# zhaoweicai/mscnn

Hardware: AMD Instinct MI355X
Metric: images/sec mscnn-7s-576 KITTI-car inference (higher is better)
Workload: dtype f32

## Files before the change

### include/mscnn_hip.h

```cpp
#ifndef MSCNN_HIP_H_
#define MSCNN_HIP_H_

#include <stddef.h>
#include <stdint.h>

#if defined(__GNUC__)
#define MSCNN_API __attribute__((visibility("default")))
#else
#define MSCNN_API
#endif

#ifdef __cplusplus
extern "C" {
#endif

typedef enum {
  MSCNN_OK = 0,
  MSCNN_ERR_BAD_ARG = 1,
  MSCNN_ERR_HIP = 2,
  MSCNN_ERR_WORKSPACE = 3,
  MSCNN_ERR_UNSUPPORTED = 4
} mscnn_status;

MSCNN_API const char* mscnn_last_error(void);
MSCNN_API const char* mscnn_version(void);

typedef struct mscnn_conv_plan mscnn_conv_plan;

typedef enum {
  MSCNN_CONV_ALGO_AUTO = 0,
  MSCNN_CONV_ALGO_DIRECT = 1,
  MSCNN_CONV_ALGO_WINO_F2 = 2,
  MSCNN_CONV_ALGO_WINO_F3 = 3,
  MSCNN_CONV_ALGO_F16 = 4,
  MSCNN_CONV_ALGO_WINO_F3_X3 = 5,
  MSCNN_CONV_ALGO_WINO_F4 = 6
} mscnn_conv_algo;

typedef struct {
  int N, Cin, H, W;
  int Cout, Kh, Kw;
  int pad_h, pad_w, stride_h, stride_w, group;
  int relu;
  int algo;
  int tune_variant, tune_grid, tune_flags;
} mscnn_conv_desc;

MSCNN_API int mscnn_conv2d_plan_create(const mscnn_conv_desc* desc, mscnn_conv_plan** plan_out);
MSCNN_API void mscnn_conv2d_plan_destroy(mscnn_conv_plan* plan);
MSCNN_API size_t mscnn_conv2d_packed_weight_bytes(const mscnn_conv_plan* plan);
MSCNN_API size_t mscnn_conv2d_workspace_bytes(const mscnn_conv_plan* plan);
MSCNN_API const char* mscnn_conv2d_plan_kernel(const mscnn_conv_plan* plan);
MSCNN_API double mscnn_conv2d_plan_flops(const mscnn_conv_plan* plan);
MSCNN_API const char* mscnn_conv2d_plan_dtype(const mscnn_conv_plan* plan);
MSCNN_API double mscnn_conv2d_plan_executed_flops(const mscnn_conv_plan* plan);
MSCNN_API int mscnn_conv2d_plan_set_profiling(mscnn_conv_plan* plan, int on);
MSCNN_API int mscnn_conv2d_plan_stage_ms(const mscnn_conv_plan* plan, float ms_out[3]);
#define MSCNN_AMAX_SLOTS 1024
MSCNN_API int mscnn_conv2d_plan_publishes_amax(const mscnn_conv_plan* plan);
MSCNN_API int mscnn_conv2d_plan_set_amax_io(mscnn_conv_plan* plan, const uint32_t* in_bound, uint32_t* out_amax);
MSCNN_API int mscnn_conv2d_plan_set_batch(mscnn_conv_plan* plan, int N);
MSCNN_API unsigned long long mscnn_conv2d_plan_weight_layout(const mscnn_conv_plan* plan);
MSCNN_API int mscnn_conv2d_pack_weights(const mscnn_conv_plan* plan, const float* w, float* packed, void* stream);
MSCNN_API int mscnn_conv2d_fwd_f32(const mscnn_conv_plan* plan, const float* x, const float* w, const float* packed,
                         const float* bias, float* y, void* workspace, size_t workspace_bytes, void* stream);
MSCNN_API int mscnn_conv2d_plan_can_pool(const mscnn_conv_plan* plan);
MSCNN_API int mscnn_conv2d_fwd_pool_f32(const mscnn_conv_plan* plan, const float* x, const float* w, const float* packed,
                              const float* bias, float* y, float* y_pool, void* workspace, size_t workspace_bytes,
                              void* stream);

MSCNN_API int mscnn_relu_fwd_f32(const float* x, float* y, size_t count, float negative_slope, void* stream);

MSCNN_API int mscnn_pool_out_dim(int in, int kernel, int pad, int stride);
MSCNN_API int mscnn_pool2d_fwd_f32(const float* x, float* y, int N, int C, int H, int W, int kernel_h, int kernel_w,
                         int pad_h, int pad_w, int stride_h, int stride_w, int method, void* stream);

MSCNN_API int mscnn_inner_product_fwd_f32(const float* x, const float* w, const float* bias, float* y,
                                int M, int N, int K, int relu, void* stream);
MSCNN_API void mscnn_debug_inner_product_rows(int rows);

MSCNN_API int mscnn_inner_product_wg_supported(int M, int N, int K);
MSCNN_API size_t mscnn_inner_product_wg_packed_bytes(int N, int K);
MSCNN_API size_t mscnn_inner_product_wg_workspace_bytes(int M, int N, int K);
MSCNN_API int mscnn_inner_product_wg_pack(const float* w, float* wt, int N, int K, void* stream);
MSCNN_API int mscnn_inner_product_wg_fwd(const float* x, const float* wt, const float* bias, float* y, int M, int N, int K, int relu,
                                         void* workspace, size_t workspace_bytes, void* stream);
MSCNN_API unsigned long long mscnn_wgemm_handoff_event(void);
MSCNN_API void mscnn_wgemm_force_whole_tiles(int on);
MSCNN_API int mscnn_wgemm_whole_tiles_forced(void);
MSCNN_API void mscnn_debug_wgemm_handoff_fault(int drop_publish, unsigned spin_limit);
MSCNN_API int mscnn_inner_product_x3_supported(int N, int K);
MSCNN_API size_t mscnn_inner_product_x3_packed_bytes(int N, int K);
MSCNN_API size_t mscnn_inner_product_x3_workspace_bytes(int M, int N, int K);
MSCNN_API int mscnn_inner_product_x3_pack(const float* w, void* packed, int N, int K, void* stream);
MSCNN_API int mscnn_inner_product_x3_fwd(const float* x, const void* packed, const float* bias, float* y, int M, int N, int K, int relu,
                               const uint32_t* in_bound, void* workspace, size_t workspace_bytes, void* stream);
MSCNN_API int mscnn_inner_product_f16_supported(int N, int K);
MSCNN_API int mscnn_inner_product_pack_f16(const float* w, void* w16, int N, int K, void* stream);
MSCNN_API int mscnn_inner_product_fwd_f16(const float* x, const void* w16, const float* bias, float* y, int M, int N, int K, int relu,
                                          void* stream);

MSCNN_API int mscnn_concat_channels_f32(const float* x, float* y, int N, int C, int inner, int C_total, int c_offset, void* stream);

MSCNN_API int mscnn_deconv_depthwise_fwd_f32(const float* x, const float* w, const float* bias, float* y,
                                   int N, int C, int H, int W, int Kh, int Kw, int pad_h, int pad_w,
                                   int stride_h, int stride_w, void* stream);

MSCNN_API int mscnn_deconv2d_fwd_f32(const float* x, const float* w, const float* bias, float* y, int N, int Cin, int H, int W,
                                     int Cout, int Kh, int Kw, int pad_h, int pad_w, int stride_h, int stride_w, int group,
                                     void* stream);

MSCNN_API int mscnn_max_rel_diff_f32(const float* a, const float* ref, size_t count, float floor, float* out_dev, void* stream);
MSCNN_API int mscnn_max_rel_diff_strided_f32(const float* a, size_t a_stride, const float* ref, size_t ref_stride, size_t planes, size_t run,
                                             const double* sumsq_dev, double sumsq_count, float* out_dev, void* stream);
MSCNN_API int mscnn_store_words_i32(int* dst_dev, const int* values_host, int n, void* stream);
MSCNN_API int mscnn_sum_squares_f32(const float* x, size_t count, double* out_dev, void* stream);

MSCNN_API int mscnn_softmax_fwd_f32(const float* x, float* y, int outer, int C, int inner, void* stream);

MSCNN_API int mscnn_roipool_fwd_f32(const float* feat, const float* rois, float* out, int R, int N, int C, int H, int W,
                          int pooled_h, int pooled_w, float spatial_scale, float pad_ratio,
                          int C_total, int c_offset, void* stream);
MSCNN_API int mscnn_roipool_pair_fwd_f32(const float* feat, const float* rois, float* out, int R, int N, int C, int H, int W,
                                         int pooled_h, int pooled_w, float spatial_scale, float pad_ratio_a, int c_offset_a,
                                         float pad_ratio_b, int c_offset_b, int C_total, void* stream);

MSCNN_API int mscnn_conv2d_plan_can_chain(const mscnn_conv_plan* plan, const mscnn_conv_plan* next);
MSCNN_API int mscnn_conv2d_plan_can_pool_only(const mscnn_conv_plan* plan);
MSCNN_API int mscnn_conv2d_fwd_chain_f32(const mscnn_conv_plan* plan, const mscnn_conv_plan* next, const float* x, const float* packed,
                               const float* bias, float* y, float* y_pool, void* workspace, size_t workspace_bytes,
                               void* next_workspace, size_t next_workspace_bytes, void* stream);

MSCNN_API int mscnn_conv2d_plan_can_fuse_roipool(const mscnn_conv_plan* plan, int C, int pooled_h, int pooled_w);
MSCNN_API size_t mscnn_conv2d_roipool_workspace_bytes(const mscnn_conv_plan* plan, int N, int C, int H, int W);
MSCNN_API size_t mscnn_roipool_maps_bytes(int N, int C, int H, int W);
MSCNN_API int mscnn_roipool_maps_build_f32(const float* feat, float* maps, int N, int C, int H, int W, void* stream);
MSCNN_API int mscnn_conv2d_fwd_roipool_pair_f32(const mscnn_conv_plan* plan, const float* feat, const float* prepared_maps, int N, int C,
                                                int H, int W, const float* rois, float spatial_scale, float pad_ratio_a,
                                                float pad_ratio_b, const float* packed_w, const float* bias, float* y, void* workspace,
                                                size_t workspace_bytes, void* stream);

MSCNN_API int mscnn_roialign_fwd_f32(const float* feat, const float* rois, float* out, int R, int N, int C, int H, int W,
                                     int pooled_h, int pooled_w, float spatial_scale, float pad_ratio, void* stream);
// ... 129 lines not shown
```

### mscnn_amd/csrc/conv.hip

```cpp
#include "common.h"
#include "headconv.h"
#include "winograd.h"
#include "wino_x3.h"
#include "wgemm.h"
#include "roipool_wino.h"
#include "conv_c3.h"
#include "wconv.h"
#include "wf2conv.h"
#include "x3_device.h"
#include <new>
#include <type_traits>

namespace {

typedef float f32x16 __attribute__((ext_vector_type(16)));
typedef _Float16 f16x8 __attribute__((ext_vector_type(8)));

struct IgemmArgs {
  const float* x; const float* wp; const float* bias; float* y; float* ws;
  int N, Cin, H, W, Cout, Ho, Wo, pad_h, pad_w;
  int MT, NTH, NTW, NT, KI, G, relu;
  int xcd_map;
  int epi_prio;
  float* yp;
  int Hp, Wp;
  int nt_major;
  unsigned w_img_bytes;
  int full_q;
  long total_iters;
  const unsigned* amax_in; const float* w_inv;
  unsigned* amax_out;
#ifdef MSCNN_WG_TRACE
  unsigned long long* trace;
#endif
};
#ifdef MSCNN_WG_TRACE
static unsigned long long* g_wg_trace = nullptr;
extern "C" __attribute__((visibility("default"))) void mscnn_debug_set_wg_trace(void* p) { g_wg_trace = static_cast<unsigned long long*>(p); }
#define MSCNN_TRACE_STAMP(slot)                                                                                  \
  if (a.trace && tid == 0 && (slot) < 16) a.trace[(long)blockIdx.x * 16 + (slot)] = __builtin_amdgcn_s_memrealtime();
#else
#define MSCNN_TRACE_STAMP(slot)
#endif
constexpr int kSlabsPerWg = 2;

template <int BM_, int BN_, int WGM_, int WGN_, int KH_, int KW_, int CK_, int TW_, int RH_ = 0, int RW_ = 0, int RP_ = 0, int PF_ = 0, int VEC_ = 0, int NOPN_ = 0, int F16_ = 0>
struct Cfg {
  static constexpr bool F16 = F16_ != 0;
  static constexpr bool X3 = F16_ == 2;
  static constexpr int PARTS = X3 ? 2 : 1;
  static constexpr bool PUBLISH = VEC_ == 0 && F16_ != 1;
  static constexpr int MIN_WG_PER_CU = PF_ == 3 ? 4 : (PF_ == 4 || PF_ == 5) ? 3 : 2;
  static constexpr int KG = CK_ / 8;
  static constexpr int VEC = VEC_;
  static constexpr bool PREFETCH_NEXT = VEC_ != 0 && NOPN_ == 0;
  static constexpr int F4_PER_CH = BN_ / 4;
  static constexpr int CH_PER_PASS = 256 / F4_PER_CH;
  static constexpr int BV_PER_T = CK_ * F4_PER_CH / 256;
// ... 799 lines not shown
#define ROI_ENTRY16(RH, RW, RP)                                                                                              \
  {"igemm16_128x128_k3x3_roi" #RH "x" #RW "p" #RP, 128, 128, 3, 3, 16, 0, 0, RH, RW, RP,                                       \
   Cfg<128, 128, 2, 2, 3, 3, 16, 32, RH, RW, RP, 0, 0, 0, 1>::IPT, 4, 200, igemm_kernel<Cfg<128, 128, 2, 2, 3, 3, 16, 32, RH, RW, RP, 0, 0, 0, 1>>, \
   igemm_fixup_kernel<Cfg<128, 128, 2, 2, 3, 3, 16, 32, RH, RW, RP, 0, 0, 0, 1>>}
    ENTRY16(128, 128, 2, 2, 16),
    ENTRY16(128, 128, 2, 2, 32),
    ENTRY16(64, 256, 1, 4, 32),
#define ENTRY16_OCC3(BM, BN, WGM, WGN, TW)                                                                                   \
  {"igemm16_" #BM "x" #BN "_k3x3_tw" #TW "_occ3", BM, BN, 3, 3, 16, TW, BN / TW, 0, 0, 0, 1, (BM * BN) / 4096, 201,            \
   igemm_kernel<Cfg<BM, BN, WGM, WGN, 3, 3, 16, TW, 0, 0, 0, 4, 0, 0, 1>>, igemm_fixup_kernel<Cfg<BM, BN, WGM, WGN, 3, 3, 16, TW, 0, 0, 0, 4, 0, 0, 1>>, \
   Cfg<BM, BN, WGM, WGN, 3, 3, 16, TW, 0, 0, 0, 4, 0, 0, 1>::CAN_POOL ? igemm_fixup_pool_kernel<Cfg<BM, BN, WGM, WGN, 3, 3, 16, TW, 0, 0, 0, 4, 0, 0, 1>> : nullptr}
    {"igemm16_128x256_k3x3_tw32", 128, 256, 3, 3, 16, 32, 8, 0, 0, 0, 1, 8, 202, igemm_kernel<Cfg<128, 256, 2, 2, 3, 3, 16, 32, 0, 0, 0, 0, 0, 0, 1>>,
     igemm_fixup_kernel<Cfg<128, 256, 2, 2, 3, 3, 16, 32, 0, 0, 0, 0, 0, 0, 1>>, igemm_fixup_pool_kernel<Cfg<128, 256, 2, 2, 3, 3, 16, 32, 0, 0, 0, 0, 0, 0, 1>>},
    {"igemm16x3_64x256_k3x3_tw32", 64, 256, 3, 3, 16, 32, 8, 0, 0, 0, 1, 4, 210, igemm_kernel<Cfg<64, 256, 1, 4, 3, 3, 16, 32, 0, 0, 0, 0, 0, 0, 2>>,
     igemm_fixup_kernel<Cfg<64, 256, 1, 4, 3, 3, 16, 32, 0, 0, 0, 0, 0, 0, 2>>, igemm_fixup_pool_kernel<Cfg<64, 256, 1, 4, 3, 3, 16, 32, 0, 0, 0, 0, 0, 0, 2>>},
    ENTRY16_OCC3(128, 128, 2, 2, 16),
    ENTRY16_OCC3(128, 128, 2, 2, 32),
    ENTRY16_OCC3(64, 256, 1, 4, 32),
    ROI_ENTRY16(7, 7, 0),
    ROI_ENTRY16(7, 5, 0),
    ROI_ENTRY16(8, 4, 1),
    ENTRY(32, 128, 1, 4, 5, 5, 8, 16),
    ENTRY(32, 128, 1, 4, 7, 7, 8, 16),
    ENTRY(32, 128, 1, 4, 5, 3, 8, 16),
    ENTRY(32, 128, 1, 4, 7, 5, 8, 16),
    ENTRY(64, 256, 1, 4, 5, 1, 8, 32),
    ENTRY(64, 256, 1, 4, 7, 1, 8, 32),
    ROI_ENTRY(128, 128, 2, 2, 3, 3, 8, 7, 7, 0),
    ROI_ENTRY(128, 128, 2, 2, 3, 3, 8, 7, 5, 0),
    ROI_ENTRY(128, 128, 2, 2, 3, 3, 8, 8, 4, 1),
};
constexpr int kTableN = sizeof(kTable) / sizeof(kTable[0]);

}

struct mscnn_conv_plan {
  mscnn_conv_desc d;
  int Ho, Wo;
  int entry;
  int MT, NTH, NTW, NT, KI, G, full_q;
  long total_iters;
  size_t packed_bytes, ws_bytes;
  mscnn::HeadPlan head;
  mscnn_conv_plan* wino = nullptr;
  bool use_wg = false;
  mscnn::WgemmPlan wg;
  bool c3 = false;
  bool wc_use = false;
  mscnn::WconvPlan wc;
  bool wf_use = false;
  mscnn::Wf2Plan wf;
  int wino_m = 2;
  int tiles_h = 0, tiles_w = 0, T_pad = 0;
  mscnn::X3Plan x3;
  mscnn::X3HeadPlan x3h;
  mscnn_conv_plan* hg = nullptr;
  int hg_rows = 0;
  int hg_kw = 0;
  size_t hg_t_bytes = 0;
  size_t x3d_hdr_off = 0, x3d_slots_off = 0;
  const unsigned* amax_in = nullptr;
  unsigned* amax_out = nullptr;
  bool profiling = false;
  mutable hipEvent_t ev[4] = {nullptr, nullptr, nullptr, nullptr};
  mutable bool ev_valid = false;
  ~mscnn_conv_plan() {
    delete hg;
    delete wino;
    for (hipEvent_t e : ev) if (e) (void)hipEventDestroy(e);
  }
};

using namespace mscnn;

static void plan_shape(mscnn_conv_plan* p);

static bool head_gemm_plan(mscnn_conv_plan* p) {
  const mscnn_conv_desc& d = p->d;
  const int flags = tune_env("MSCNN_TUNE_FLAGS", d.tune_flags);
  const long HW = (long)d.H * d.W;
  if (tune_env("MSCNN_CONV_ALGO", d.algo) == MSCNN_CONV_ALGO_WINO_F3_X3 || (flags & 32) || (flags & 2)) return false;
  if (d.stride_h != 1 || d.stride_w != 1 || d.group != 1 || d.Cout > 12 || d.Kh * d.Kw < 2 || d.Kh * d.Kw > 64 || d.N < 1) return false;
  if (d.Cin % 32 != 0 || d.Cin < 32 || p->Ho < 1 || p->Wo < 1) return false;
  const bool kw_legal = d.Kw * d.Cout >= 40 && d.Kw * d.Cout <= 64 && d.pad_w * 2 + 1 == d.Kw && p->Ho == d.H && p->Wo == d.W &&
                        (d.Kh == 5 || d.Kh == 7) && HW >= 1024;
  if (!(flags & 16) && !(flags & 512) && kw_legal && ((flags & 1024) || (d.Kw * d.Cout >= 56 && HW >= 8192))) {
    mscnn_conv_plan* g = new (std::nothrow) mscnn_conv_plan();
    if (!g) return false;
    g->d = d;
    g->d.N = 1; g->d.Cout = d.Kw * d.Cout; g->d.Kw = 1; g->d.pad_w = 0; g->d.relu = 0;
    g->d.algo = MSCNN_CONV_ALGO_DIRECT;
    g->d.tune_variant = 0; g->d.tune_grid = 0; g->d.tune_flags = (flags & 1) | 32 | 2;
    plan_shape(g);
    if (g->entry >= 0 && !g->wino && !g->hg && g->head.entry < 0 && g->Ho == d.H && g->Wo == d.W && kTable[g->entry].KW == 1 &&
        kTable[g->entry].BM == 64) {
      p->hg = g;
      p->hg_kw = d.Kw;
      p->hg_rows = d.Kw * d.Cout;
      p->hg_t_bytes = ((size_t)p->hg_rows * HW * sizeof(float) + 255) / 256 * 256;
      p->packed_bytes = g->packed_bytes + (size_t)p->hg_rows * d.Cin * d.Kh * sizeof(float);
      p->ws_bytes = p->hg_t_bytes + g->ws_bytes;
      return true;
    }
    delete g;
  }
  if (!(flags & 16) && !kHeadGemmDefault) return false;
  if (!(flags & 16) && HW < kHeadGemmMinPixels) return false;
  const int rows = d.Kh * d.Kw * d.Cout;
  if ((double)rows * HW * 4.0 >= 2.0e9) return false;
  mscnn_conv_plan* g = new (std::nothrow) mscnn_conv_plan();
  if (!g) return false;
  g->d = d;
  g->d.N = 1; g->d.Cout = rows; g->d.Kh = g->d.Kw = 1; g->d.pad_h = g->d.pad_w = 0; g->d.relu = 0;
  g->d.algo = MSCNN_CONV_ALGO_DIRECT;
  g->d.tune_variant = 0; g->d.tune_grid = 0; g->d.tune_flags = flags & 1;
  if (HW % 128 == 0) { g->d.H = (int)(HW / 128); g->d.W = 128; }
  else { g->d.H = 1; g->d.W = (int)HW; }
  plan_shape(g);
  if (g->entry < 0 || g->wino || g->hg || g->head.entry >= 0 || g->Ho * (long)g->Wo != HW) { delete g; return false; }
  p->hg = g;
  p->hg_kw = 0;
  p->hg_rows = rows;
  p->hg_t_bytes = ((size_t)rows * HW * sizeof(float) + 255) / 256 * 256;
  p->packed_bytes = g->packed_bytes + (size_t)rows * d.Cin * sizeof(float);
  p->ws_bytes = p->hg_t_bytes + g->ws_bytes;
  return true;
}

static bool wino_plan(mscnn_conv_plan* p) {
  const mscnn_conv_desc& d = p->d;
  const int algo = tune_env("MSCNN_CONV_ALGO", d.algo);
  if (algo == MSCNN_CONV_ALGO_DIRECT || d.Kh != 3 || d.Kw != 3 || d.stride_h != 1 || d.stride_w != 1 || d.group != 1) return false;
  if (p->Ho < 2 || p->Wo < 2) return false;
  const bool want_x3 = algo == MSCNN_CONV_ALGO_WINO_F3_X3;
  if (want_x3 && (d.tune_flags & 8)) return false;
  const bool force = algo == MSCNN_CONV_ALGO_WINO_F2 || algo == MSCNN_CONV_ALGO_WINO_F3 || algo == MSCNN_CONV_ALGO_WINO_F4 ||
                     (want_x3 && (d.tune_flags & 4));
  const double intensity = (double)d.Cin * d.Cout / (d.Cin + d.Cout);
  const bool roi_map = d.H <= 8 && d.W <= 8;
  const long T4 = (long)d.N * cdiv(p->Ho, 4) * cdiv(p->Wo, 4);
  const bool auto_f4 = algo == MSCNN_CONV_ALGO_AUTO && !roi_map && T4 >= 1000 && !(d.tune_flags & 64);
  const int m = roi_map ? 3 : (algo == MSCNN_CONV_ALGO_WINO_F2 ? 2 : (algo == MSCNN_CONV_ALGO_WINO_F4 || auto_f4) ? 4 : 3);
  const int planes = (m + 2) * (m + 2);
  const double wino_min = want_x3 && d.Cin % 16 == 0 ? 80.0 : (m == 4 ? 40.0 : m == 3 ? 60.0 : 100.0);
  if (!force && (intensity < wino_min || (!roi_map && d.H * d.W < 256))) return false;
  if (roi_map && d.N < 8) return false;
  const int th = cdiv(p->Ho, m), tw = cdiv(p->Wo, m);
  const long T = (long)d.N * th * tw;
  const long T_pad = (T + 127) / 128 * 128;
  if ((double)T_pad * (d.Cin > d.Cout ? d.Cin : d.Cout) * 4.0 >= 2.0e9) return false;
  if (want_x3 && m == 3 && x3_plan(d.Cin, d.Cout, T_pad, d.tune_variant, &p->x3)) {
    p->wino_m = 3;
    p->tiles_h = th; p->tiles_w = tw; p->T_pad = (int)T_pad;
    p->packed_bytes = p->x3.packed_bytes;
    p->ws_bytes = p->x3.scal_bytes + p->x3.v_bytes + (size_t)25 * d.Cout * T_pad * sizeof(float);
    return true;
  }
  mscnn_conv_plan* g = new (std::nothrow) mscnn_conv_plan();
  if (!g) return false;
  g->d = d;
  if (g->d.tune_variant >= 300) g->d.tune_variant = 0;
  g->d.N = planes; g->d.H = (int)(T_pad / 128); g->d.W = 128; g->d.Kh = g->d.Kw = 1; g->d.pad_h = g->d.pad_w = 0; g->d.relu = 0;
  g->d.algo = MSCNN_CONV_ALGO_DIRECT;
  plan_shape(g);
  if (g->entry >= 0 && g->d.tune_variant == 0 && (long)g->MT * g->NT >= 3000 && ((long)g->MT * g->NT) % 1000 == 0) {
    g->d.tune_variant = 107;
    g->d.tune_grid = 1000;
    plan_shape(g);
  }
  if (g->entry < 0 || g->wino || g->head.entry >= 0) { delete g; return false; }
  p->wino_m = m;
  p->wino = g;
  p->tiles_h = th; p->tiles_w = tw; p->T_pad = (int)T_pad;
  p->packed_bytes = (size_t)planes * g->packed_bytes;
  p->ws_bytes = (size_t)planes * ((size_t)d.Cin + d.Cout) * T_pad * sizeof(float) + g->ws_bytes;
  p->use_wg = false;
  if (m >= 3 && !(d.tune_flags & 128) && mscnn::wgemm_plan(planes, d.Cout, d.Cin, (int)T, (d.tune_variant >= 300 && d.tune_variant < 1100) ? d.tune_variant - 300 : 0, &p->wg)) {
    p->use_wg = true;
    p->T_pad = p->wg.T_pad;
    p->packed_bytes = p->wg.packed_bytes;
    p->ws_bytes = (size_t)planes * ((size_t)d.Cin + d.Cout) * p->wg.T_pad * sizeof(float) + p->wg.ws_bytes;
  }
  return true;
}

static void plan_shape(mscnn_conv_plan* p) {
  const mscnn_conv_desc& d = p->d;
  p->Ho = (d.H + 2 * d.pad_h - d.Kh) / d.stride_h + 1;
  p->Wo = (d.W + 2 * d.pad_w - d.Kw) / d.stride_w + 1;
  p->entry = -1;
  p->c3 = false;
  p->wc_use = false;
  p->wf_use = false;
  p->packed_bytes = 0;
  p->ws_bytes = 0;
  p->head.entry = -1;
  p->x3h = mscnn::X3HeadPlan();
  delete p->hg;
  p->hg = nullptr;
  p->hg_rows = 0;
  p->hg_kw = 0;
  p->hg_t_bytes = 0;
  if (tune_env("MSCNN_CONV_ALGO", d.algo) == MSCNN_CONV_ALGO_WINO_F3_X3 && d.stride_h == 1 && d.stride_w == 1 && d.group == 1 &&
      d.Cout <= 12 && d.Kh * d.Kw > 1 && d.N > 0 && !(d.tune_flags & 2) &&
      x3_head_plan(d.Cin, d.Cout, d.Kh, d.Kw, (long)d.H * d.W, &p->x3h)) {
    p->packed_bytes = p->x3h.packed_bytes;
    p->ws_bytes = 4096 + p->x3h.t_bytes;
    return;
  }
  if (head_gemm_plan(p)) return;
  if (head_plan(d, p->Ho, p->Wo, &p->head)) {
    p->packed_bytes = p->head.packed_bytes;
    p->ws_bytes = p->head.ws_bytes;
    return;
  }
  delete p->wino;
  p->wino = nullptr;
  p->x3 = mscnn::X3Plan();
  {
    const int algo = tune_env("MSCNN_CONV_ALGO", d.algo);
    const bool named_wino = algo == MSCNN_CONV_ALGO_WINO_F2 || algo == MSCNN_CONV_ALGO_WINO_F3 || algo == MSCNN_CONV_ALGO_WINO_F4;
    if (!named_wino && !(d.tune_flags & 2048) && mscnn::c3_plan(d, p->Ho, p->Wo)) { p->c3 = true; return; }
  }
  if (d.stride_h != 1 || d.stride_w != 1 || d.group != 1 || d.N == 0 || d.Cin > 2048) return;
  const bool want16 = tune_env("MSCNN_CONV_ALGO", d.algo) == MSCNN_CONV_ALGO_F16 && d.Kh == 3 && d.Kw == 3;
  if (!want16 && wino_plan(p)) return;
  const bool wantx3 = tune_env("MSCNN_CONV_ALGO", d.algo) == MSCNN_CONV_ALGO_WINO_F3_X3 && d.Kh == 3 && d.Kw == 3 && d.Cin % 16 == 0 &&
                      (long)d.H * d.W >= 4096;
  const double win_x = (double)d.Cin * d.H * d.W * 4.0, win_y = (double)d.Cout * p->Ho * p->Wo * 4.0;
  double best = 1e300;
  const int tv0 = tune_env("MSCNN_TUNE_VARIANT", d.tune_variant);
  const int tv = tv0 >= 400 ? 0 : tv0;
  const bool venv = tv > 0 && d.Kh == 3 && d.Kw == 3;
  const int want = venv ? tv - 1 : (d.Cout >= 128 ? 1 : 0);
// ... 94 lines not shown
  MSCNN_REQUIRE(p, "conv plan: out of memory");
  p->d = d;
  plan_shape(p);
  *plan_out = p;
  return MSCNN_OK;
}

extern "C" void mscnn_conv2d_plan_destroy(mscnn_conv_plan* plan) { delete plan; }
extern "C" size_t mscnn_conv2d_packed_weight_bytes(const mscnn_conv_plan* p) { return p ? p->packed_bytes : 0; }
extern "C" size_t mscnn_conv2d_workspace_bytes(const mscnn_conv_plan* p) { return p ? p->ws_bytes : 0; }
extern "C" const char* mscnn_conv2d_plan_kernel(const mscnn_conv_plan* p) {
  if (!p) return "";
  if (p->x3h.rows) return "head_gemm_shiftadd_x3f16";
  if (p->hg) return p->hg_kw ? "head_kwfold_shiftadd_f32" : "head_gemm_shiftadd_f32";
  if (p->head.entry >= 0) return head_kernel_name(p->head);
  if (p->x3.BM) return p->x3.BM == 256 ? "winograd_f3x3_3x3_x3f16_256" : "winograd_f3x3_3x3_x3f16_128";
  if (p->wino) return p->wino_m == 4 ? "winograd_f4x4_3x3" : p->wino_m == 3 ? "winograd_f3x3_3x3" : "winograd_f2x2_3x3";
  if (p->c3) return mscnn::c3_kernel_name();
  if (p->wf_use) return mscnn::wf2_kernel_name();
  if (p->wc_use) return mscnn::wconv_kernel_name();
  return p->entry < 0 ? "direct_f32" : kTable[p->entry].name;
}
extern "C" unsigned long long mscnn_conv2d_plan_weight_layout(const mscnn_conv_plan* p) {
  if (!p) return 0;
  unsigned long long kind, e, mt, ki;
  if (p->x3h.rows) { kind = 7; e = (unsigned)p->x3h.rows_pad; mt = 0; ki = (unsigned)p->x3h.KG; }
  else if (p->hg) { kind = p->hg_kw ? 10 : 8; e = (unsigned)p->hg->entry; mt = (unsigned)p->hg->MT; ki = (unsigned)p->hg->KI; }
  else if (p->head.entry >= 0) { kind = 2; e = p->head.valu >= 0 ? 100u + (unsigned)p->head.valu : (unsigned)p->head.entry; mt = 0; ki = (unsigned)p->head.KI; }
  else if (p->x3.BM) { kind = 6; e = (unsigned)p->x3.BM; mt = (unsigned)p->x3.MT; ki = (unsigned)p->x3.KG; }
  else if (p->wino && p->use_wg) { kind = p->wino_m == 4 ? 9u : 2 + (unsigned)p->wino_m; e = 200u + (unsigned)(p->wg.BM / 128);       mt = (unsigned)p->wg.MT; ki = (unsigned)p->wg.KI; }
  else if (p->wino) { kind = p->wino_m == 4 ? 9u : 2 + (unsigned)p->wino_m; e = (unsigned)p->wino->entry; mt = (unsigned)p->wino->MT; ki = (unsigned)p->wino->KI; }
  else if (p->wf_use) { kind = 11; e = 0; mt = 1; ki = (unsigned)p->wf.KI; }
  else if (p->entry >= 0) { kind = 1; e = (unsigned)p->entry; mt = (unsigned)p->MT; ki = (unsigned)p->KI; }
  else return 0;
  return kind | (e << 8) | (mt << 24) | (ki << 44);
}
extern "C" double mscnn_conv2d_plan_flops(const mscnn_conv_plan* p) {
  if (!p) return 0;
  const mscnn_conv_desc& d = p->d;
  return 2.0 * d.N * d.Cout * p->Ho * p->Wo * (double)(d.Cin / d.group) * d.Kh * d.Kw;
}
extern "C" const char* mscnn_conv2d_plan_dtype(const mscnn_conv_plan* p) {
  if (p && p->x3h.rows) return "f16x3";
  if (p && (p->x3.BM || (!p->wino && p->head.entry < 0 && p->entry >= 0 && kTable[p->entry].variant == 210))) return "f16x3";
  return (p && !p->wino && p->head.entry < 0 && p->entry >= 0 && kTable[p->entry].variant >= 200 && kTable[p->entry].variant <= 202) ? "f16" : "f32";
}
extern "C" double mscnn_conv2d_plan_executed_flops(const mscnn_conv_plan* p) {
  if (!p) return 0;
  if (p->x3h.rows) return 3.0 * mscnn_conv2d_plan_flops(p);
  if (p->wf_use) return mscnn_conv2d_plan_flops(p) * (16.0 / 36.0);
  if (!p->wino && !p->x3.BM)
    return mscnn_conv2d_plan_flops(p) * ((p->head.entry < 0 && p->entry >= 0 && kTable[p->entry].variant == 210) ? 3.0 : 1.0);
  const mscnn_conv_desc& d = p->d;
  const double planes = (double)((p->wino_m + 2) * (p->wino_m + 2)) * (p->x3.BM ? 3.0 : 1.0);
  return 2.0 * planes * d.Cout * d.Cin * ((double)d.N * p->tiles_h * p->tiles_w);
}
extern "C" int mscnn_conv2d_plan_set_profiling(mscnn_conv_plan* p, int on) {
  MSCNN_REQUIRE(p, "conv plan: null");
  p->profiling = on != 0;
  p->ev_valid = false;
  if (p->profiling)
    for (hipEvent_t& e : p->ev)
      if (!e) MSCNN_HIP_TRY(hipEventCreate(&e));
  return MSCNN_OK;
}
extern "C" int mscnn_conv2d_plan_stage_ms(const mscnn_conv_plan* p, float ms_out[3]) {
  MSCNN_REQUIRE(p && ms_out, "conv plan: null");
  ms_out[0] = ms_out[1] = ms_out[2] = 0.f;
  MSCNN_REQUIRE(p->profiling && p->ev_valid, "conv plan: no profiled forward yet (mscnn_conv2d_plan_set_profiling)");
  MSCNN_HIP_TRY(hipEventSynchronize(p->ev[3]));
  for (int i = 0; i < 3; ++i) MSCNN_HIP_TRY(hipEventElapsedTime(&ms_out[i], p->ev[i], p->ev[i + 1]));
  return MSCNN_OK;
}
extern "C" int mscnn_conv2d_plan_publishes_amax(const mscnn_conv_plan* p) {
  return p && !p->x3h.rows && (p->x3.BM || (p->wino && p->wino_m >= 3) || p->c3 ||
               (!p->wino && p->head.entry < 0 && p->entry >= 0 && !p->wc_use && !p->wf_use && !(kTable[p->entry].variant >= 200 && kTable[p->entry].variant <= 202))) ? 1 : 0;
}
extern "C" int mscnn_conv2d_plan_set_amax_io(mscnn_conv_plan* p, const uint32_t* in_bound, uint32_t* out_amax) {
  MSCNN_REQUIRE(p, "conv plan: null");
  if (out_amax && !mscnn_conv2d_plan_publishes_amax(p)) {
    set_error("conv plan: kernel %s does not publish max |y|", mscnn_conv2d_plan_kernel(p));
    return MSCNN_ERR_UNSUPPORTED;
  }
  p->amax_in = in_bound;
  p->amax_out = out_amax;
  return MSCNN_OK;
}
extern "C" int mscnn_conv2d_plan_set_batch(mscnn_conv_plan* p, int N) {
  MSCNN_REQUIRE(p && N >= 0, "conv plan: bad batch");
  p->d.N = N;
  plan_shape(p);
  return MSCNN_OK;
}

extern "C" int mscnn_conv2d_pack_weights(const mscnn_conv_plan* p, const float* w, float* packed, void* stream) {
  MSCNN_REQUIRE(p, "conv pack: null plan");
  if (p->x3h.rows) {
    MSCNN_REQUIRE(w && packed, "conv pack: null pointer");
    return x3_head_pack(p->x3h, w, packed, as_stream(stream));
  }
  if (p->hg) {
    MSCNN_REQUIRE(w && packed, "conv pack: null pointer");
    float* wprime = reinterpret_cast<float*>(reinterpret_cast<unsigned char*>(packed) + p->hg->packed_bytes);
    if (p->hg_kw) {
      const long tot = (long)p->hg_rows * p->d.Cin * p->d.Kh;
      head_kw_weight_kernel<<<(int)((tot + 255) / 256 > 4096 ? 4096 : (tot + 255) / 256), 256, 0, as_stream(stream)>>>(
          w, wprime, p->d.Cout, p->d.Cin, p->d.Kh, p->d.Kw);
      MSCNN_POST_LAUNCH();
// ... 49 lines not shown
  const mscnn_conv_desc& d = p->d;
  const KernelEntry& k = kTable[p->entry];
  const long rem_tiles = (long)p->MT * p->NT - (long)p->full_q * p->G;
  const bool split = rem_tiles > 0;
  if (split) {
    if (!workspace || workspace_bytes < p->ws_bytes) {
      set_error("conv: workspace %zu < %zu", workspace_bytes, p->ws_bytes);
      return MSCNN_ERR_WORKSPACE;
    }
  }
  IgemmArgs a;
  a.x = x; a.wp = packed; a.bias = bias; a.y = y; a.ws = static_cast<float*>(workspace);
  a.N = d.N; a.Cin = d.Cin; a.H = d.H; a.W = d.W; a.Cout = d.Cout; a.Ho = p->Ho; a.Wo = p->Wo; a.pad_h = d.pad_h; a.pad_w = d.pad_w;
  a.MT = p->MT; a.NTH = p->NTH; a.NTW = p->NTW; a.NT = p->NT; a.KI = p->KI; a.G = p->G; a.relu = d.relu;
  a.total_iters = p->total_iters; a.full_q = p->full_q;
  a.w_img_bytes = w_img_bytes; a.nt_major = nt_major;
  a.yp = y_pool; a.Hp = (p->Ho + 1) / 2; a.Wp = (p->Wo + 1) / 2;
  if (y_pool && !k.fix_pool_fn) {
    set_error("conv: kernel %s has no fused pooling epilogue", k.name);
    return MSCNN_ERR_BAD_ARG;
  }
  a.xcd_map = (tune_env("MSCNN_TUNE_FLAGS", d.tune_flags) & 1) ? 0 : 1;
  a.epi_prio = ((k.BM == 64 && k.BN == 256 && k.KH == 3 && k.KW == 3) ? 1 : 0) ^ ((tune_env("MSCNN_TUNE_FLAGS", d.tune_flags) & 16384) ? 1 : 0);
#ifdef MSCNN_WG_TRACE
  a.trace = g_wg_trace;
#endif
  a.amax_in = nullptr; a.w_inv = nullptr;
  a.amax_out = nt_major ? nullptr : p->amax_out;
  if (k.variant == 210) {
    if (!workspace || workspace_bytes < p->ws_bytes) {
      set_error("conv(x3): workspace %zu < %zu", workspace_bytes, p->ws_bytes);
      return MSCNN_ERR_WORKSPACE;
    }
    a.w_inv = reinterpret_cast<const float*>(reinterpret_cast<const unsigned char*>(packed) + p->x3d_hdr_off);
    a.amax_in = p->amax_in;
    if (!a.amax_in) {
      unsigned* slots = reinterpret_cast<unsigned*>(static_cast<unsigned char*>(workspace) + p->x3d_slots_off);
      const int rc = x3_amax(x, (long)d.N * d.Cin * d.H * d.W, slots, st);
      if (rc != MSCNN_OK) return rc;
      a.amax_in = slots;
    }
  }
  k.main_fn<<<p->G, 256, 0, st>>>(a);
  MSCNN_POST_LAUNCH();
  if (split) {
    (y_pool ? k.fix_pool_fn : k.fix_fn)<<<(int)rem_tiles * k.fix_split, 256, 0, st>>>(a);
    MSCNN_POST_LAUNCH();
  }
  return MSCNN_OK;
}

extern "C" int mscnn_conv2d_plan_can_pool(const mscnn_conv_plan* p) {
  if (!p || p->head.entry >= 0 || p->x3h.rows || p->hg) return 0;
  if (p->wino || p->x3.BM) return p->wino_m == 2 || p->wino_m == 4 || (p->tiles_h % 2 == 0 && p->tiles_w % 2 == 0 && p->d.H > 8);
  return p->entry >= 0 && kTable[p->entry].fix_pool_fn != nullptr;
}

static int conv_forward_single(const mscnn_conv_plan* p, const float* x, const float* w, const float* packed, const float* bias,
                               float* y, float* y_pool, void* workspace, size_t workspace_bytes, hipStream_t st);

extern "C" int mscnn_conv2d_fwd_f32(const mscnn_conv_plan* p, const float* x, const float* w, const float* packed,
                                    const float* bias, float* y, void* workspace, size_t workspace_bytes, void* stream) {
  return mscnn_conv2d_fwd_pool_f32(p, x, w, packed, bias, y, nullptr, workspace, workspace_bytes, stream);
}

template <class InputStage, class OutputStage>
static int wino_forward_stages(const mscnn_conv_plan* p, const float* packed, void* workspace, size_t workspace_bytes, hipStream_t st,
                               InputStage&& input_stage, OutputStage&& output_stage) {
  const mscnn_conv_desc& d = p->d;
#define MSCNN_STAGE_EVENT(i) do { if (p->profiling) MSCNN_HIP_TRY(hipEventRecord(p->ev[i], st)); } while (0)
  MSCNN_REQUIRE(packed, "conv: Winograd path needs packed weights (mscnn_conv2d_pack_weights)");
  if (!workspace || workspace_bytes < p->ws_bytes) {
    set_error("conv(winograd): workspace %zu < %zu", workspace_bytes, p->ws_bytes);
    return MSCNN_ERR_WORKSPACE;
  }
  const mscnn_conv_plan* g = p->wino;
  const size_t planes = (size_t)(p->wino_m + 2) * (p->wino_m + 2);
  float* V = static_cast<float*>(workspace);
  float* M = V + planes * d.Cin * p->T_pad;
  float* gws = M + planes * d.Cout * p->T_pad;
  MSCNN_STAGE_EVENT(0);
  int rc = input_stage(V);
  if (rc != MSCNN_OK) return rc;
  MSCNN_STAGE_EVENT(1);
  if (p->use_wg) rc = mscnn::wgemm_launch(p->wg, packed, V, M, gws, st);
  else rc = launch_igemm(g, V, packed, nullptr, M, nullptr, gws, g->ws_bytes, st, (unsigned)g->packed_bytes, 1);
  if (rc != MSCNN_OK) return rc;
  MSCNN_STAGE_EVENT(2);
  rc = output_stage(M);
  if (rc != MSCNN_OK) return rc;
  MSCNN_STAGE_EVENT(3);
  p->ev_valid = p->profiling;
  return MSCNN_OK;
#undef MSCNN_STAGE_EVENT
}

template <class InputStage>
static int wino_forward(const mscnn_conv_plan* p, const float* packed, const float* bias, float* y, float* y_pool, void* workspace,
                        size_t workspace_bytes, hipStream_t st, InputStage&& input_stage) {
  const mscnn_conv_desc& d = p->d;
  return wino_forward_stages(p, packed, workspace, workspace_bytes, st, input_stage, [&](const float* M) {
    return wino_output_transform(p->wino_m, M, bias, y, y_pool, d.N, d.Cout, p->Ho, p->Wo, p->tiles_h, p->tiles_w, p->T_pad, d.relu, st,
                                 p->wino_m >= 3 ? p->amax_out : nullptr, (d.tune_flags & 256) != 0);
  });
}

extern "C" int mscnn_conv2d_fwd_pool_f32(const mscnn_conv_plan* p, const float* x, const float* w, const float* packed,
                                         const float* bias, float* y, float* y_pool, void* workspace, size_t workspace_bytes,
                                         void* stream) {
  MSCNN_REQUIRE(p, "conv: null plan");
  MSCNN_REQUIRE(!y_pool || mscnn_conv2d_plan_can_pool(p), "conv: this plan has no fused 2x2 max-pooling epilogue");
  const mscnn_conv_desc& d = p->d;
  if (d.N == 0) return MSCNN_OK;
  MSCNN_REQUIRE(x && (y || (y_pool && mscnn_conv2d_plan_can_pool_only(p))),
                "conv: null pointer (y may be NULL only with y_pool on a plan where mscnn_conv2d_plan_can_pool_only)");
  hipStream_t st = as_stream(stream);
#define MSCNN_STAGE_EVENT(i) do { if (p->profiling) MSCNN_HIP_TRY(hipEventRecord(p->ev[i], st)); } while (0)
  if (p->x3.BM) {
    MSCNN_REQUIRE(packed, "conv: Winograd path needs packed weights (mscnn_conv2d_pack_weights)");
    if (!workspace || workspace_bytes < p->ws_bytes) {
      set_error("conv(winograd x3): workspace %zu < %zu", workspace_bytes, p->ws_bytes);
      return MSCNN_ERR_WORKSPACE;
    }
    unsigned char* wsb = static_cast<unsigned char*>(workspace);
    const unsigned* scal = p->amax_in ? p->amax_in : reinterpret_cast<unsigned*>(wsb);
    void* V16 = wsb + p->x3.scal_bytes;
    float* M = reinterpret_cast<float*>(wsb + p->x3.scal_bytes + p->x3.v_bytes);
    MSCNN_STAGE_EVENT(0);
    int rc = p->amax_in ? MSCNN_OK : x3_amax(x, (long)d.N * d.Cin * d.H * d.W, reinterpret_cast<unsigned*>(wsb), st);
    if (rc != MSCNN_OK) return rc;
    rc = x3_input_transform(p->x3, x, V16, scal, d.N, d.H, d.W, d.pad_h, d.pad_w, p->tiles_h, p->tiles_w, st);
    if (rc != MSCNN_OK) return rc;
    MSCNN_STAGE_EVENT(1);
    rc = x3_gemm(p->x3, packed, V16, M, scal, (tune_env("MSCNN_TUNE_FLAGS", d.tune_flags) & 1) ? 0 : 1, st);
    if (rc != MSCNN_OK) return rc;
    MSCNN_STAGE_EVENT(2);
    rc = wino_output_transform(3, M, bias, y, y_pool, d.N, d.Cout, p->Ho, p->Wo, p->tiles_h, p->tiles_w, p->T_pad, d.relu, st,
                               p->amax_out);
    if (rc != MSCNN_OK) return rc;
    MSCNN_STAGE_EVENT(3);
    p->ev_valid = p->profiling;
    return MSCNN_OK;
  }
  if (!p->wino) {
    MSCNN_STAGE_EVENT(0); MSCNN_STAGE_EVENT(1);
    const int rc = conv_forward_single(p, x, w, packed, bias, y, y_pool, workspace, workspace_bytes, st);
    if (rc != MSCNN_OK) return rc;
    MSCNN_STAGE_EVENT(2); MSCNN_STAGE_EVENT(3);
    p->ev_valid = p->profiling;
    return MSCNN_OK;
  }
  return wino_forward(p, packed, bias, y, y_pool, workspace, workspace_bytes, st, [&](float* V) {
    return wino_input_transform(p->wino_m, x, V, d.N, d.Cin, d.H, d.W, d.pad_h, d.pad_w, p->tiles_h, p->tiles_w, p->T_pad, st,
                                (d.tune_flags & 256) != 0, (d.tune_flags & 4096) != 0);
  });
#undef MSCNN_STAGE_EVENT
}


static bool is_f4_plane_path(const mscnn_conv_plan* p) { return p && p->wino && p->wino_m == 4 && !p->x3.BM && p->d.N > 0; }
extern "C" int mscnn_conv2d_plan_can_chain(const mscnn_conv_plan* p, const mscnn_conv_plan* next) {
  if (!is_f4_plane_path(p) || !is_f4_plane_path(next)) return 0;
  const mscnn_conv_desc &a = p->d, &b = next->d;
  return a.N == b.N && a.Cout == b.Cin && p->Ho == b.H && p->Wo == b.W && b.Kh == 3 && b.Kw == 3 && b.pad_h == 1 && b.pad_w == 1 &&
                 b.stride_h == 1 && b.stride_w == 1 && p->tiles_h == next->tiles_h && p->tiles_w == next->tiles_w &&
                 !((a.tune_flags | b.tune_flags) & 256) && mscnn::wino44_outin_supported(p->Ho, p->Wo, p->tiles_h, p->tiles_w)
             ? 1 : 0;
}
extern "C" int mscnn_conv2d_plan_can_pool_only(const mscnn_conv_plan* p) {
  if (!p || !mscnn_conv2d_plan_can_pool(p)) return 0;
  if (is_f4_plane_path(p)) return p->Wo % 4 == 0 && p->tiles_w * 4 == p->Wo && !(p->d.tune_flags & 256) ? 1 : 0;
  return !p->wino && !p->x3.BM && !p->x3h.rows && !p->hg && p->head.entry < 0 && !p->c3 && p->entry >= 0 ? 1 : 0;
}
extern "C" int mscnn_conv2d_fwd_chain_f32(const mscnn_conv_plan* p, const mscnn_conv_plan* next, const float* x, const float* packed,
                                          const float* bias, float* y, float* y_pool, void* workspace, size_t workspace_bytes,
                                          void* next_workspace, size_t next_workspace_bytes, void* stream) {
  MSCNN_REQUIRE(p, "conv: null plan");
  MSCNN_REQUIRE(is_f4_plane_path(p), "conv(chain): the plan does not take the fp32 F(4x4,3x3) path");
  MSCNN_REQUIRE(!next || mscnn_conv2d_plan_can_chain(p, next), "conv(chain): these two plans do not chain (mscnn_conv2d_plan_can_chain)");
  MSCNN_REQUIRE(next ? !y_pool : (y != nullptr || (y_pool && mscnn_conv2d_plan_can_pool_only(p))),
                "conv(chain): y_pool only without a next plan; y may be NULL only with one, or with y_pool where mscnn_conv2d_plan_can_pool_only");
  MSCNN_REQUIRE(!y_pool || mscnn_conv2d_plan_can_pool(p), "conv: this plan has no fused 2x2 max-pooling epilogue");
  const mscnn_conv_desc& d = p->d;
  hipStream_t st = as_stream(stream);
  if (next) {
    const size_t vbytes = sizeof(float) * 36 * (size_t)next->d.Cin * next->T_pad;
    if (!next_workspace || next_workspace_bytes < next->ws_bytes) {
      set_error("conv(chain): next workspace %zu < %zu", next_workspace_bytes, next->ws_bytes);
      return MSCNN_ERR_WORKSPACE;
    }
    const unsigned char *a0 = static_cast<const unsigned char*>(workspace), *b0 = static_cast<const unsigned char*>(next_workspace);
    MSCNN_REQUIRE(b0 + vbytes <= a0 || a0 + p->ws_bytes <= b0, "conv(chain): the next plan's planes overlap this plan's workspace");
  }
  auto input_stage = [&](float* V) {
    if (!x) return (int)MSCNN_OK;
    return wino_input_transform(p->wino_m, x, V, d.N, d.Cin, d.H, d.W, d.pad_h, d.pad_w, p->tiles_h, p->tiles_w, p->T_pad, st,
                                (d.tune_flags & 256) != 0, (d.tune_flags & 4096) != 0);
  };
  if (!next) return wino_forward(p, packed, bias, y, y_pool, workspace, workspace_bytes, st, input_stage);
  return wino_forward_stages(p, packed, workspace, workspace_bytes, st, input_stage, [&](const float* M) {
    return mscnn::wino44_output_into_input(M, bias, y, static_cast<float*>(next_workspace), d.N, d.Cout, p->Ho, p->Wo, p->tiles_h, p->tiles_w,
                                           p->T_pad, next->T_pad, d.relu, st, p->amax_out);
  });
}

extern "C" int mscnn_conv2d_plan_can_fuse_roipool(const mscnn_conv_plan* p, int C, int pooled_h, int pooled_w) {
  return p && p->wino && p->wino_m == 3 && !p->x3.BM && p->d.N > 0 && p->d.Cin == 2 * C && p->d.H == pooled_h && p->d.W == pooled_w &&
                 p->tiles_h == 2 && p->tiles_w == 2 && p->d.Kh == 3 && p->d.Kw == 3 &&
                 mscnn::roipool_wino33_supported(C, pooled_h, pooled_w, p->d.pad_h, p->d.pad_w)
             ? 1 : 0;
}
static size_t roipool_scratch_offset(const mscnn_conv_plan* p) { return (p->ws_bytes + 255) / 256 * 256; }
extern "C" size_t mscnn_conv2d_roipool_workspace_bytes(const mscnn_conv_plan* p, int N, int C, int H, int W) {
  return p ? roipool_scratch_offset(p) + mscnn::roipool_wino33_scratch_bytes(N, C, H, W) : 0;
}
extern "C" size_t mscnn_roipool_maps_bytes(int N, int C, int H, int W) { return mscnn::roipool_wino33_scratch_bytes(N, C, H, W); }
extern "C" int mscnn_roipool_maps_build_f32(const float* feat, float* maps, int N, int C, int H, int W, void* stream) {
  return mscnn::roipool_wino33_build_maps(feat, maps, N, C, H, W, as_stream(stream));
}
extern "C" int mscnn_conv2d_fwd_roipool_pair_f32(const mscnn_conv_plan* p, const float* feat, const float* prepared_maps, int N, int C,
                                                 int H, int W, const float* rois, float spatial_scale, float pad_ratio_a, float pad_ratio_b,
                                                 const float* packed, const float* bias, float* y, void* workspace,
                                                 size_t workspace_bytes, void* stream) {
  MSCNN_REQUIRE(p, "conv: null plan");
  if (p->d.N == 0) return MSCNN_OK;
  MSCNN_REQUIRE((feat || prepared_maps) && rois && y && N > 0 && H > 0 && W > 0, "conv(roipool): bad argument");
  MSCNN_REQUIRE(mscnn_conv2d_plan_can_fuse_roipool(p, C, p->d.H, p->d.W), "conv(roipool): this plan does not take the fused ROI-pooling input stage");
  const size_t need = prepared_maps ? p->ws_bytes : mscnn_conv2d_roipool_workspace_bytes(p, N, C, H, W);
  if (!workspace || workspace_bytes < need) {
    set_error("conv(roipool): workspace %zu < %zu", workspace_bytes, need);
    return MSCNN_ERR_WORKSPACE;
  }
  hipStream_t st = as_stream(stream);
  float* own_maps = reinterpret_cast<float*>(static_cast<unsigned char*>(workspace) + roipool_scratch_offset(p));
  return wino_forward(p, packed, bias, y, nullptr, workspace, workspace_bytes, st, [&](float* V) {
    if (!prepared_maps) {
      const int rc = mscnn::roipool_wino33_build_maps(feat, own_maps, N, C, H, W, st);
      if (rc != MSCNN_OK) return rc;
    }
    return mscnn::roipool_wino33_forward(prepared_maps ? prepared_maps : own_maps, rois, V, p->d.N, N, C, H, W, p->T_pad, spatial_scale,
                                         pad_ratio_a, pad_ratio_b, st);
  });
}

static int conv_forward_single(const mscnn_conv_plan* p, const float* x, const float* w, const float* packed, const float* bias,
                               float* y, float* y_pool, void* workspace, size_t workspace_bytes, hipStream_t st) {
  const mscnn_conv_desc& d = p->d;
  if (p->x3h.rows) {
    MSCNN_REQUIRE(packed, "conv: head kernel needs packed weights (mscnn_conv2d_pack_weights)");
    if (!workspace || workspace_bytes < p->ws_bytes) {
      set_error("conv(head x3): workspace %zu < %zu", workspace_bytes, p->ws_bytes);
      return MSCNN_ERR_WORKSPACE;
    }
    for (int n = 0; n < d.N; ++n) {
      const int rc = x3_head_forward(p->x3h, x + (size_t)n * d.Cin * d.H * d.W, packed, bias, y + (size_t)n * d.Cout * p->Ho * p->Wo, d.H,
                                     d.W, p->Ho, p->Wo, d.pad_h, d.pad_w, d.relu, d.N == 1 ? p->amax_in : nullptr, workspace, st);
      if (rc != MSCNN_OK) return rc;
    }
    return MSCNN_OK;
  }
  if (p->hg) {
    MSCNN_REQUIRE(packed, "conv: head kernel needs packed weights (mscnn_conv2d_pack_weights)");
    if (!workspace || workspace_bytes < p->ws_bytes) {
      set_error("conv(head gemm): workspace %zu < %zu", workspace_bytes, p->ws_bytes);
      return MSCNN_ERR_WORKSPACE;
    }
    float* T = static_cast<float*>(workspace);
    void* nested_ws = static_cast<unsigned char*>(workspace) + p->hg_t_bytes;
    for (int n = 0; n < d.N; ++n) {
      int rc = launch_igemm(p->hg, x + (size_t)n * d.Cin * d.H * d.W, packed, nullptr, T, nullptr, nested_ws, p->hg->ws_bytes, st, 0u,
                            p->hg_kw ? 0 : 1);
      if (rc != MSCNN_OK) return rc;
      if (p->hg_kw)
        rc = head_shift_add(T, bias, y + (size_t)n * d.Cout * p->Ho * p->Wo, d.Cout, d.H, d.W, p->Ho, p->Wo, 1, d.Kw, 0, d.pad_w,
                            (unsigned)((long)d.H * d.W), d.relu, st);
      else
        rc = head_shift_add(T, bias, y + (size_t)n * d.Cout * p->Ho * p->Wo, d.Cout, d.H, d.W, p->Ho, p->Wo, d.Kh, d.Kw, d.pad_h, d.pad_w,
                            (unsigned)((long)d.H * d.W), d.relu, st);
      if (rc != MSCNN_OK) return rc;
    }
    return MSCNN_OK;
  }
  if (p->head.entry >= 0) {
    MSCNN_REQUIRE(packed, "conv: head kernel needs packed weights (mscnn_conv2d_pack_weights)");
    return head_forward(d, p->head, p->Ho, p->Wo, x, packed, bias, y, workspace, workspace_bytes, st);
  }
  if (p->c3) {
    MSCNN_REQUIRE(w, "conv: the Cin = 3 kernel needs the Caffe-layout weights");
    return mscnn::c3_forward(d, x, w, bias, y, p->amax_out, st);
  }
  if (p->entry < 0) {
    MSCNN_REQUIRE(w, "conv: direct kernel needs the Caffe-layout weights");
    const long total = (long)d.N * d.Cout * p->Ho * p->Wo;
    long blocks = (total + 255) / 256;
// ... 12 lines not shown
```

### mscnn_amd/csrc/roipool_wino.h

```cpp
#pragma once
#include "common.h"

namespace mscnn {

bool roipool_wino33_supported(int C, int pooled_h, int pooled_w, int conv_pad_h, int conv_pad_w);
size_t roipool_wino33_scratch_bytes(int N, int C, int H, int W);
int roipool_wino33_build_maps(const float* feat, float* maps, int N, int C, int H, int W, hipStream_t st);
int roipool_wino33_forward(const float* maps, const float* rois, float* V, int R, int N, int C, int H, int W, int T_pad,
                           float spatial_scale, float pad_a, float pad_b, hipStream_t st);

}
```

### mscnn_amd/csrc/roipool_wino.hip

```cpp
#include "roipool_wino.h"
#include "wino33_device.h"
#include <cfloat>

namespace {

typedef unsigned u32x4 __attribute__((ext_vector_type(4)));

constexpr int kNB = 4;
constexpr int kLevels = 4;

struct RpwArgs {
  const float* maps;
  const float* rois;
  float* V;
  int R, C, H, W, T_pad;
  unsigned level_bytes, maps_bytes, v_bytes;
  float spatial_scale, pad_a, pad_b;
};

__device__ __forceinline__ __amdgpu_buffer_rsrc_t make_rsrc(const void* p, unsigned bytes) {
  return __builtin_amdgcn_make_buffer_rsrc(const_cast<void*>(p), 0, (int)bytes, 0x00020000);
}
__device__ __forceinline__ int uni(int v) { return __builtin_amdgcn_readfirstlane(v); }
__device__ __forceinline__ float max3(float a, float b, float c) {
  float r;
  asm("v_max3_f32 %0, %1, %2, %3" : "=v"(r) : "v"(a), "v"(b), "v"(c));
  return r;
}
__device__ __forceinline__ void launder(float& v) { asm volatile("" : "+v"(v)); }

constexpr int kRois = 8;
constexpr int kLdsRow = kRois * 4 + 4;

template <int PH, int PW>
__global__ __launch_bounds__(kRois * 64) void roipool_wino33_kernel(RpwArgs a) {
  static_assert(PH == 7 && PW == 7, "tiles per ROI: 2 x 2 tiles of 3 x 3 outputs (a 16-byte unit of V per plane)");
  __shared__ __attribute__((aligned(16))) float s_out[5 * 64 * kLdsRow];
  const int tid = threadIdx.x, lane = tid & 63, wave = uni(tid >> 6);
  const int r0 = blockIdx.y * kRois;
  const int r = r0 + wave;
  const bool live = r < a.R;
  const int c0 = blockIdx.x * 64;
  const int c = c0 + lane;
  const __amdgpu_buffer_rsrc_t rF = make_rsrc(a.maps, a.maps_bytes), rV = make_rsrc(a.V, a.v_bytes);
  const unsigned lane_off = (unsigned)c * 4u;

  const float* roi = a.rois + 5 * (size_t)(live ? r : 0);
  const int b = (int)roi[0];
  const float x1 = roi[1], y1 = roi[2], x2 = roi[3], y2 = roi[4];
  const int H = a.H, W = a.W, C = a.C;
  const int row0 = b * H;
  const unsigned pxB = (unsigned)C * 4u, rowB = (unsigned)W * pxB;
  auto load_at = [&](unsigned off) {
#ifdef RPW_NO_POOL
    return (float)(off + lane);
#endif
    return __builtin_bit_cast(float, __builtin_amdgcn_raw_buffer_load_b32(rF, lane_off, off, 0));
  };

  {
    const int q = blockIdx.z;
    const float pad_ratio = q == 0 ? a.pad_a : a.pad_b;
    const float pad_w = (x2 - x1 + 1) * pad_ratio;
    const float pad_h = (y2 - y1 + 1) * pad_ratio;
    const int roi_start_w = (int)roundf((x1 - pad_w) * a.spatial_scale);
    const int roi_start_h = (int)roundf((y1 - pad_h) * a.spatial_scale);
    const int roi_end_w = (int)roundf((x2 + pad_w) * a.spatial_scale);
    const int roi_end_h = (int)roundf((y2 + pad_h) * a.spatial_scale);
    const int roi_width = max(roi_end_w - roi_start_w + 1, 1);
    const int roi_height = max(roi_end_h - roi_start_h + 1, 1);
    const float bin_size_h = (float)roi_height / (float)PH;
    const float bin_size_w = (float)roi_width / (float)PW;
    const bool wide = roi_width >= roi_height;
    int bw_[PW];
    unsigned wsB[PW], weB[PW];
#pragma unroll
    for (int pw = 0; pw < PW; ++pw) {
      const int ws = uni(min(max((int)floorf((float)pw * bin_size_w) + roi_start_w, 0), W));
      const int we = uni(min(max((int)ceilf((float)(pw + 1) * bin_size_w) + roi_start_w, 0), W));
      bw_[pw] = we - ws;
      wsB[pw] = (unsigned)min(ws, W - 1) * pxB;
      weB[pw] = (unsigned)max(we, min(ws, W - 1) + 1) * pxB;
    }

    float pooled[PH * PW];
#pragma unroll
    for (int ph = 0; ph < PH; ++ph) {
// ... 23 lines not shown
            v[bi][0] = load_at(ac0 + al0); v[bi][1] = load_at(ac0 + a1); v[bi][2] = load_at(ac0 + a2); v[bi][3] = load_at(ac0 + a3);
            v[bi][4] = load_at(ac1 + al0); v[bi][5] = load_at(ac1 + a1); v[bi][6] = load_at(ac1 + a2); v[bi][7] = load_at(ac1 + a3);
          }
        }
#pragma unroll
        for (int bi = 0; bi < NB; ++bi) {
          const int pw = half * NB + bi;
          if (pw < PW) {
            const int w = bw_[pw];
            float m = max3(v[bi][0], v[bi][1], v[bi][2]);
            m = max3(m, v[bi][3], v[bi][4]);
            m = max3(m, v[bi][5], v[bi][6]);
            m = max3(m, v[bi][7], -FLT_MAX);
            const int s_ = 1 << lev[bi];
            const int across_len = wide ? h : w, along_len = wide ? w : h;
            if (across_len > 2 * s_ || along_len > 4 * s_) {
              const unsigned stepx = pxB << lev[bi], stepy = rowB << lev[bi];
              const unsigned xlastB = weB[pw] - stepx, ylastB = heB - stepy, base = (unsigned)lev[bi] * a.level_bytes;
              for (unsigned yB = hsB; yB < heB; yB += stepy)
                for (unsigned xB = wsB[pw]; xB < weB[pw]; xB += 4 * stepx) {
                  const unsigned rb = base + min(yB, ylastB);
                  const float u0 = load_at(rb + min(xB, xlastB)), u1 = load_at(rb + min(xB + stepx, xlastB));
                  const float u2 = load_at(rb + min(xB + 2 * stepx, xlastB)), u3 = load_at(rb + min(xB + 3 * stepx, xlastB));
                  m = max3(m, u0, u1);
                  m = max3(m, u2, u3);
                }
            }
            pooled[ph * PW + pw] = (h <= 0 || w <= 0) ? 0.f : m;
          }
        }
      }
    }

#ifdef RPW_DBG_POOLED
    {
      const unsigned rb = ((unsigned)(q * C) * (unsigned)a.T_pad + (unsigned)r * 4u) * 4u, vl = (unsigned)c * (unsigned)a.T_pad * 4u;
      const unsigned pb = (unsigned)(2 * C) * (unsigned)a.T_pad * 4u;
      if (live)
#pragma unroll
        for (int k = 0; k < PH * PW; ++k)
          __builtin_amdgcn_raw_buffer_store_b32(__builtin_bit_cast(unsigned, pooled[k]), rV, vl, rb + (unsigned)(k % 25) * pb + (unsigned)(k / 25) * 4u, 0);
      return;
    }
#endif
    const unsigned plane_bytes = (unsigned)(2 * C) * (unsigned)a.T_pad * 4u;
#pragma unroll
    for (int i = 0; i < 5; ++i) {
#pragma unroll
      for (int k = 0; k < PH * PW; ++k) launder(pooled[k]);
      float out[5][4];
#pragma unroll
      for (int t = 0; t < 4; ++t) {
        const int ty = t >> 1, tx = t & 1;
        float rr[5];
#pragma unroll
        for (int j = 0; j < 5; ++j) {
          float d[5], o[5];
#pragma unroll
          for (int k = 0; k < 5; ++k) {
            const int h = 3 * ty + k, w = 3 * tx + j;
            d[k] = (h < PH && w < PW) ? pooled[h * PW + w] : 0.f;
          }
          mscnn::bt5(d, o);
          rr[j] = o[i];
        }
        float o2[5];
        mscnn::bt5(rr, o2);
#pragma unroll
        for (int j = 0; j < 5; ++j) out[j][t] = o2[j];
      }
      __syncthreads();
#pragma unroll
      for (int j = 0; j < 5; ++j)
        *reinterpret_cast<float4*>(&s_out[(j * 64 + lane) * kLdsRow + wave * 4]) = make_float4(out[j][0], out[j][1], out[j][2], out[j][3]);
      __syncthreads();
#pragma unroll
      for (int n = 0; n < 5 * 64 * kRois / (kRois * 64); ++n) {
        const int item = tid + n * (kRois * 64);
        const int rq = item % kRois, ch = (item / kRois) % 64, j = item / (kRois * 64);
        if (r0 + rq < a.R) {
          const float4 u = *reinterpret_cast<const float4*>(&s_out[(j * 64 + ch) * kLdsRow + rq * 4]);
          u32x4 pk;
          pk.x = __builtin_bit_cast(unsigned, u.x); pk.y = __builtin_bit_cast(unsigned, u.y);
          pk.z = __builtin_bit_cast(unsigned, u.z); pk.w = __builtin_bit_cast(unsigned, u.w);
          const unsigned off = (unsigned)(i * 5 + j) * plane_bytes + ((unsigned)(q * C + c0 + ch) * (unsigned)a.T_pad + (unsigned)(r0 + rq) * 4u) * 4u;
#ifndef RPW_NO_STORE
          __builtin_amdgcn_raw_buffer_store_b128(pk, rV, off, 0u, 0);
#else
          if (a.T_pad < 0) __builtin_amdgcn_raw_buffer_store_b128(pk, rV, off, 0u, 0);
#endif
        }
      }
    }
  }
}

__global__ __launch_bounds__(256) void nchw_to_nhwc_kernel(const float* __restrict__ x, float* __restrict__ y, int C, int HW) {
  __shared__ float t[64][65];
  const int n = blockIdx.z, c0 = blockIdx.y * 64, p0 = blockIdx.x * 64;
  const int tx = threadIdx.x & 63, ty = threadIdx.x >> 6;
  const float* src = x + (size_t)n * C * HW;
  float* dst = y + (size_t)n * C * HW;
#pragma unroll
  for (int i = 0; i < 16; ++i) {
    const int cc = c0 + ty + 4 * i, pp = p0 + tx;
    t[ty + 4 * i][tx] = (cc < C && pp < HW) ? src[(size_t)cc * HW + pp] : 0.f;
  }
  __syncthreads();
#pragma unroll
  for (int i = 0; i < 16; ++i) {
    const int pp = p0 + ty + 4 * i, cc = c0 + tx;
    if (pp < HW && cc < C) dst[(size_t)pp * C + cc] = t[tx][ty + 4 * i];
  }
}

__global__ __launch_bounds__(256) void sliding_max_kernel(const float* __restrict__ src, float* __restrict__ dst, int H, int W, int C4, int half,
                                                          long total) {
  const long i = blockIdx.x * 256L + threadIdx.x;
  if (i >= total) return;
  const int c4 = (int)(i % C4);
  long p = i / C4;
  const int x = (int)(p % W); p /= W;
  const int y = (int)(p % H);
  const long n = p / H;
  const int y2 = min(y + half, H - 1), x2 = min(x + half, W - 1);
  const float4* s4 = reinterpret_cast<const float4*>(src) + n * H * W * C4;
  const float4 a = s4[((long)y * W + x) * C4 + c4], b = s4[((long)y * W + x2) * C4 + c4];
  const float4 c = s4[((long)y2 * W + x) * C4 + c4], d = s4[((long)y2 * W + x2) * C4 + c4];
  float4 m = a;
  m.x = b.x > m.x ? b.x : m.x; m.y = b.y > m.y ? b.y : m.y; m.z = b.z > m.z ? b.z : m.z; m.w = b.w > m.w ? b.w : m.w;
  m.x = c.x > m.x ? c.x : m.x; m.y = c.y > m.y ? c.y : m.y; m.z = c.z > m.z ? c.z : m.z; m.w = c.w > m.w ? c.w : m.w;
  m.x = d.x > m.x ? d.x : m.x; m.y = d.y > m.y ? d.y : m.y; m.z = d.z > m.z ? d.z : m.z; m.w = d.w > m.w ? d.w : m.w;
  reinterpret_cast<float4*>(dst)[i] = m;
}

}

namespace mscnn {

bool roipool_wino33_supported(int C, int pooled_h, int pooled_w, int conv_pad_h, int conv_pad_w) {
  return pooled_h == 7 && pooled_w == 7 && conv_pad_h == 0 && conv_pad_w == 0 && C > 0 && C % 64 == 0;
}

size_t roipool_wino33_scratch_bytes(int N, int C, int H, int W) { return (size_t)kLevels * N * C * H * W * sizeof(float); }

int roipool_wino33_build_maps(const float* feat, float* maps, int N, int C, int H, int W, hipStream_t st) {
  MSCNN_REQUIRE(feat && maps, "roipool maps: null pointer");
  MSCNN_REQUIRE(N > 0 && C % 64 == 0 && H > 0 && W > 0, "roipool maps: bad shape");
  MSCNN_REQUIRE(kLevels * (double)N * C * H * W * 4.0 < 4.0e9, "roipool maps: beyond a 32-bit buffer window");
  MSCNN_REQUIRE(reinterpret_cast<uintptr_t>(maps) % 16 == 0, "roipool maps: the maps must be 16-byte aligned");
  const int HW = H * W;
  const long per_level = (long)N * C * HW;
  nchw_to_nhwc_kernel<<<dim3(cdiv(HW, 64), cdiv(C, 64), N), 256, 0, st>>>(feat, maps, C, HW);
  MSCNN_POST_LAUNCH();
  for (int k = 1; k < kLevels; ++k) {
    const long total = per_level / 4;
    sliding_max_kernel<<<(unsigned)((total + 255) / 256), 256, 0, st>>>(maps + (k - 1) * per_level, maps + k * per_level, H, W, C / 4, 1 << (k - 1), total);
    MSCNN_POST_LAUNCH();
  }
  return MSCNN_OK;
}

int roipool_wino33_forward(const float* maps, const float* rois, float* V, int R, int N, int C, int H, int W, int T_pad,
                           float spatial_scale, float pad_a, float pad_b, hipStream_t st) {
  MSCNN_REQUIRE(maps && rois && V, "roipool+transform: null pointer");
  MSCNN_REQUIRE(R > 0 && N > 0 && C % 64 == 0 && H > 0 && W > 0 && T_pad >= 4 * R && T_pad % 4 == 0, "roipool+transform: bad shape");
  const double lb = (double)N * C * H * W * 4.0, vb = 25.0 * 2.0 * C * (double)T_pad * 4.0;
  MSCNN_REQUIRE(kLevels * lb < 4.0e9 && vb < 4.0e9, "roipool+transform: feature maps or transform planes beyond a 32-bit buffer window");
  MSCNN_REQUIRE(reinterpret_cast<uintptr_t>(V) % 16 == 0, "roipool+transform: V must be 16-byte aligned");
  RpwArgs a;
  a.maps = maps; a.rois = rois; a.V = V;
  a.R = R; a.C = C; a.H = H; a.W = W; a.T_pad = T_pad;
  a.level_bytes = (unsigned)lb; a.maps_bytes = (unsigned)(kLevels * lb); a.v_bytes = (unsigned)vb;
  a.spatial_scale = spatial_scale; a.pad_a = pad_a; a.pad_b = pad_b;
  roipool_wino33_kernel<7, 7><<<dim3(C / 64, cdiv(R, kRois), 2), kRois * 64, 0, st>>>(a);
  MSCNN_POST_LAUNCH();
  return MSCNN_OK;
}

}
```

### mscnn_amd/csrc/wgemm.h

```cpp
#pragma once
#include <hip/hip_runtime.h>
#include <cstddef>

namespace mscnn {

struct WgemmPlan {
  int P, Cout, Cin, T, T_pad;
  int BM, BN, CK, MT, NT, KI;
  int G;
  int device;
  int full_q;
  int variant;
  double model_us;
  const char* name;
  size_t packed_bytes;
  size_t ws_bytes;
};

bool wgemm_plan(int P, int Cout, int Cin, int T, int variant, WgemmPlan* out);

int wgemm_launch(const WgemmPlan& p, const float* Up, const float* V, float* M, float* ws, hipStream_t st, int abl = 0,
                 unsigned long long* dbg = nullptr, const float* bias = nullptr, int relu = 0, size_t m_valid_bytes = 0);

unsigned long long wgemm_handoff_event();
void wgemm_force_whole_tiles(int on);
int wgemm_whole_tiles_forced();
void wgemm_debug_handoff_fault(int drop_publish, unsigned spin_limit);

}
```

### mscnn_amd/csrc/wgemm.hip

```cpp
#include "wgemm.h"
#include "common.h"
#include <atomic>
#include <chrono>

namespace {

typedef float f32x16 __attribute__((ext_vector_type(16)));

struct WgemmArgs {
  const float* Up; const float* V; float* M; float* ws;
  int P, MT, NT, KI, Cin, Cout, T_pad;
  int tiles, G, abl;
  int full_q;
  unsigned ws_bytes;
  unsigned epoch;
  unsigned long long* dbg;
  unsigned up_bytes, v_bytes, m_bytes;
  const float* bias; int relu;
  unsigned long long* status;
  unsigned spin_limit;
  int drop_publish;
};

template <int BM_, int BN_, int WGM_, int WGN_, int CK_, int ST_, int DPG_ = 1, int SK_ = 0>
struct WCfg {
  static constexpr int BM = BM_, BN = BN_, WGM = WGM_, WGN = WGN_, CK = CK_, ST = ST_;
  static constexpr int DPG = DPG_, SK = SK_;
  static constexpr int NW = WGM * WGN, THREADS = NW * 64;
  static constexpr int WM = BM / WGM, WN = BN / WGN, MI = WM / 32, NI = WN / 32;
  static constexpr int A_BYTES = CK * BM * 4, B_BYTES = CK * BN * 4, STAGE_BYTES = A_BYTES + B_BYTES;
  static constexpr int STAGE_FLOATS = STAGE_BYTES / 4;
  static constexpr int PA = A_BYTES / 1024, PB = B_BYTES / 1024;
  static constexpr int PA_W = PA / NW, PB_W = (PB + NW - 1) / NW;
  static constexpr int NP = PA_W + PB_W;
  static constexpr int F4_PER_ROW = BN / 4;
  static constexpr bool B_EVEN = (64 % F4_PER_ROW == 0) && (PB % NW == 0);
  static constexpr int ROWS_PER_PIECE = B_EVEN ? 64 / F4_PER_ROW : 0;
  static constexpr int LDS_FLOATS = ST * STAGE_FLOATS + (B_EVEN ? 0 : 256);
  static constexpr int STEPS = CK / 2;
  static_assert(PA % NW == 0 && B_BYTES % 1024 == 0, "pieces per wave");
  static_assert(LDS_FLOATS * 4 <= 160 * 1024, "LDS ring");
  static_assert(WM % 32 == 0 && WN % 32 == 0, "wave tile");
};

template <int I, int N, class F>
__device__ __forceinline__ void static_for(F&& f) {
  if constexpr (I < N) {
    f(std::integral_constant<int, I>{});
    static_for<I + 1, N>(f);
  }
}

__device__ __forceinline__ __amdgpu_buffer_rsrc_t make_rsrc(const void* p, unsigned bytes) {
  return __builtin_amdgcn_make_buffer_rsrc(const_cast<void*>(p), 0, (int)bytes, 0x00020000);
}

__device__ __forceinline__ void dma16(__amdgpu_buffer_rsrc_t rsrc, unsigned voff, unsigned soff, unsigned lds_addr) {
  soff = __builtin_amdgcn_readfirstlane(soff);
  lds_addr = __builtin_amdgcn_readfirstlane(lds_addr);
  asm volatile("s_nop 4\n\ts_mov_b32 m0, %3\n\ts_nop 0\n\tbuffer_load_dwordx4 %0, %1, %2 offen lds" ::"v"(voff), "s"(rsrc), "s"(soff), "s"(lds_addr) : "memory");
}

template <int N>
__device__ __forceinline__ void wait_vm_barrier() {
  if constexpr (N == 0) asm volatile("s_waitcnt vmcnt(0)\n\ts_barrier" ::: "memory");
  else asm volatile("s_waitcnt vmcnt(%0)\n\ts_barrier" ::"n"(N) : "memory");
}

template <int OFF>
__device__ __forceinline__ float lds_rd(unsigned addr) {
  float r;
  asm volatile("ds_read_b32 %0, %1 offset:%2" : "=v"(r) : "v"(addr), "n"(OFF) : "memory");
  return r;
}
template <int N>
__device__ __forceinline__ void lds_wait() { asm volatile("s_waitcnt lgkmcnt(%0)" ::"n"(N) : "memory"); }
__device__ __forceinline__ void lds_pin(float& v) { asm volatile("" : "+v"(v)); }

__device__ __host__ __forceinline__ void wg_range(int total, int G, int g, int& b, int& e) {
  b = (int)((unsigned)total * (unsigned)g / (unsigned)G);
  e = (int)((unsigned)total * (unsigned)(g + 1) / (unsigned)G);
}

struct SegCursor {
  int slot, G, KI, full_q, rem_tile0, r;
  int it, re;
  int nparts;
  __device__ __forceinline__ void init(const WgemmArgs& a, int slot_) {
    slot = slot_; G = a.G; KI = a.KI; rem_tile0 = a.full_q * a.G; r = 0; nparts = 0;
    full_q = slot_ < a.tiles ? min(a.full_q, (a.tiles - slot_ + a.G - 1) / a.G) : 0;
    if (a.tiles > rem_tile0) wg_range((a.tiles - rem_tile0) * a.KI, a.G, slot_, it, re);
    else it = re = 0;
  }
  __device__ __forceinline__ int units() const { return full_q * KI + (re - it); }
  __device__ __forceinline__ bool next(int& t, int& k0, int& k1, int& part) {
    if (r < full_q) { t = slot + r * G; k0 = 0; k1 = KI; part = -1; ++r; return true; }
    if (it >= re) return false;
    t = rem_tile0 + it / KI;
    k0 = it % KI;
    const int left = re - it;
    k1 = left < KI - k0 ? k0 + left : KI;
    it += k1 - k0;
    part = (k0 == 0 && k1 == KI) ? -1 : nparts++;
    return true;
  }
};

template <class C, int ABL, int EPI = 0>
__global__ __launch_bounds__(C::THREADS, C::NW / 4) void wgemm_kernel(WgemmArgs a) {
  __shared__ __attribute__((aligned(1024))) float lds[C::LDS_FLOATS];
  __shared__ unsigned s_handoff_timeout;
  static_assert(C::ST == 3, "the ring protocol below is written for three stages");
  const int tid = threadIdx.x;
  const int lane = tid & 63;
  const int wave = __builtin_amdgcn_readfirstlane(tid >> 6);
  const int l31 = lane & 31, khalf = lane >> 5;
  const int wm = wave / C::WGN, wn = wave % C::WGN;

  const int xcd = (int)(blockIdx.x % 8), gq = a.G / 8, gr = a.G % 8;
  const int slot = xcd * gq + min(xcd, gr) + (int)(blockIdx.x / 8);
  SegCursor pcur, ccur;
  pcur.init(a, slot); ccur.init(a, slot);
  const int nunits = pcur.units();
  if (nunits == 0) return;
  unsigned long long dbg_c = 0, dbg_r = 0;
  if (a.dbg && tid == 0) { dbg_c = __builtin_amdgcn_s_memtime(); dbg_r = __builtin_amdgcn_s_memrealtime(); }

  const __amdgpu_buffer_rsrc_t rA = make_rsrc(a.Up, a.up_bytes), rB = make_rsrc(a.V, a.v_bytes), rM = make_rsrc(a.M, a.m_bytes),
                               rW = make_rsrc(a.ws, a.ws_bytes);
  const unsigned row_bytes = (unsigned)a.T_pad * 4u;
  const unsigned vA = (unsigned)lane * 16u;
  const unsigned vB = (unsigned)(lane / C::F4_PER_ROW) * row_bytes + (unsigned)(lane % C::F4_PER_ROW) * 16u;
  unsigned vBj[C::PB_W];
#pragma unroll
  for (int i = 0; i < C::PB_W; ++i) {
    const int u = (wave * C::PB_W + i) * 64 + lane;
    vBj[i] = wave * C::PB_W + i < C::PB ? (unsigned)(u / C::F4_PER_ROW) * row_bytes + (unsigned)(u % C::F4_PER_ROW) * 16u : 0x80000000u;
  }
  const unsigned lds0 = (unsigned)(size_t)lds;
  const unsigned a_lane = (unsigned)(khalf * C::BM + wm * C::WM + l31) * 4u;
  const unsigned b_lane = (unsigned)C::A_BYTES + (unsigned)(khalf * C::BN + wn * C::WN + l31) * 4u;

  int pu = 0, p_kc = 0, p_k1 = 0, p_stage = 0;
  unsigned p_a = 0, p_b = 0;
  unsigned vA_eff = vA, vB_eff = vB;
  auto p_begin = [&]() {
    if (pu >= nunits) {
      vA_eff = 0x80000000u; vB_eff = 0x80000000u;
#pragma unroll
      for (int i = 0; i < C::PB_W; ++i) vBj[i] = 0x80000000u;
    }
    if (p_kc == p_k1 && pu < nunits) {
      int t, part;
      pcur.next(t, p_kc, p_k1, part);
      const int mt = t % a.MT, nt = (t / a.MT) % a.NT, p = t / (a.MT * a.NT);
      p_kc = __builtin_amdgcn_readfirstlane(p_kc); p_k1 = __builtin_amdgcn_readfirstlane(p_k1);
      p_a = __builtin_amdgcn_readfirstlane((unsigned)((p * a.MT + mt) * a.KI) * (unsigned)C::A_BYTES);
      p_b = __builtin_amdgcn_readfirstlane(((unsigned)(p * a.Cin) * (unsigned)a.T_pad + (unsigned)(nt * C::BN)) * 4u);
    }
  };
  auto p_piece = [&](auto ic) {
    constexpr int i = decltype(ic)::value;
    const unsigned ls = lds0 + (unsigned)p_stage * C::STAGE_BYTES;
    if constexpr (i < C::PA_W) {
      const unsigned sa = p_a + (unsigned)p_kc * C::A_BYTES + (unsigned)(wave * C::PA_W + i) * 1024u;
      dma16(rA, vA_eff, sa, ls + (unsigned)(wave * C::PA_W + i) * 1024u);
    } else if constexpr (C::B_EVEN) {
      const int j = wave * C::PB_W + (i - C::PA_W);
      const unsigned sb = p_b + (unsigned)(p_kc * C::CK + j * C::ROWS_PER_PIECE) * row_bytes;
      dma16(rB, vB_eff, sb, ls + C::A_BYTES + (unsigned)j * 1024u);
    } else {
      const int j = wave * C::PB_W + (i - C::PA_W);
      const unsigned sb = p_b + (unsigned)(p_kc * C::CK) * row_bytes;
      dma16(rB, vBj[i - C::PA_W], sb, j < C::PB ? ls + C::A_BYTES + (unsigned)j * 1024u : lds0 + (unsigned)(C::ST * C::STAGE_BYTES));
    }
  };
  auto p_end = [&]() {
    ++pu;
    ++p_kc;
    if (++p_stage == C::ST) p_stage = 0;
  };

#pragma unroll
  for (int i = 0; i < 2; ++i)
    if (pu < nunits) {
      p_begin();
      static_for<0, C::NP>([&](auto ic) { p_piece(ic); });
      p_end();
    }
  wait_vm_barrier<0>();

  f32x16 acc[2][C::MI][C::NI];
#pragma unroll
  for (int q = 0; q < 2; ++q)
#pragma unroll
    for (int mi = 0; mi < C::MI; ++mi)
#pragma unroll
      for (int ni = 0; ni < C::NI; ++ni)
#pragma unroll
        for (int r = 0; r < 16; ++r) acc[q][mi][ni][r] = 0.f;
  float old_bias[C::NI];
#pragma unroll
  for (int ni = 0; ni < C::NI; ++ni) old_bias[ni] = 0.f;
  unsigned old_voff[C::MI][C::NI];
#pragma unroll
  for (int mi = 0; mi < C::MI; ++mi)
#pragma unroll
    for (int ni = 0; ni < C::NI; ++ni) old_voff[mi][ni] = 0x80000000u;
// ... 56 lines not shown
        if constexpr (s + 1 < C::STEPS) WG_READ(nxt, c_addr, s + 1)
        else WG_READ(nxt, next_addr, 0)
        lds_wait<NR>();
      }
#pragma unroll
      for (int mi = 0; mi < C::MI; ++mi) lds_pin(av[cur][mi]);
#pragma unroll
      for (int ni = 0; ni < C::NI; ++ni) lds_pin(bv[cur][ni]);
      __builtin_amdgcn_sched_barrier(0);
      static_for<0, NMF>([&](auto jc) {
        constexpr int j = decltype(jc)::value, mi = j / C::NI, ni = j % C::NI;
        if constexpr (!(ABL & 4)) acc[PAR][mi][ni] = __builtin_amdgcn_mfma_f32_32x32x2f32(av[cur][mi], bv[cur][ni], acc[PAR][mi][ni], 0, 0, 0);
        __builtin_amdgcn_sched_barrier(0);
        if constexpr (FLUSH && s >= C::SK) {
          if constexpr (!(ABL & 2))
            static_for<0, SPM>([&](auto kc_) {
              constexpr int e = (s - C::SK) * SPG + j * SPM + decltype(kc_)::value;
              if constexpr (e < (s - C::SK + 1) * SPG && e < TOTAL) store_one(std::integral_constant<int, PAR ^ 1>{}, std::integral_constant<int, e>{});
            });
          __builtin_amdgcn_sched_barrier(0);
        }
        if constexpr (j < C::DPG && s * C::DPG + j < C::NP) {
          if constexpr (!(ABL & 1)) p_piece(std::integral_constant<int, s * C::DPG + j>{});
          __builtin_amdgcn_sched_barrier(0);
        }
      });
    });
    p_end();
    if constexpr (ABL & 16) asm volatile("s_waitcnt vmcnt(0)" ::: "memory");
    else if constexpr (FLUSH) wait_vm_barrier<(AFTER_DMA < 63 ? AFTER_DMA : 63)>();
    else wait_vm_barrier<0>();
    c_addr = next_addr;
  };

  int c_stage = 0;
  auto next_stage_addr = [&]() {
    if (++c_stage == C::ST) c_stage = 0;
    return lds0 + (unsigned)c_stage * C::STAGE_BYTES;
  };
  int t, k0, k1, part;
  int fin_tile = -1;
  typedef __attribute__((address_space(1))) unsigned long long gu64;
  gu64* flags = (gu64*)(a.ws + (size_t)a.G * (C::BM * C::BN));
  const unsigned long long want_flag = ((unsigned long long)a.epoch << 32) | (unsigned)~a.epoch;
  auto publish_flag = [&]() {
    asm volatile("s_waitcnt vmcnt(0)\n\ts_barrier" ::: "memory");
    if (tid == 0 && !a.drop_publish) __hip_atomic_store(flags + slot, want_flag, __ATOMIC_RELAXED, __HIP_MEMORY_SCOPE_AGENT);
  };
  auto segment = [&](auto par_c) {
    constexpr int PAR = decltype(par_c)::value;
    chunk(par_c, std::true_type{}, next_stage_addr());
    if (old_pub) { publish_flag(); old_pub = false; }
    for (int kc = k0 + 1; kc < k1; ++kc) chunk(par_c, std::false_type{}, next_stage_addr());
    const int mt = t % a.MT, nt = (t / a.MT) % a.NT, p = t / (a.MT * a.NT);
    const bool pub = part >= 0 && k0 > 0;
    if (part >= 0 && k0 == 0) fin_tile = t;
    old_pub = pub;
    if (pub) { old_rsrc = rW; old_rowb = (unsigned)C::BN * 4u; }
    else { old_rsrc = rM; old_rowb = row_bytes; }
    const unsigned slab = (unsigned)slot * (unsigned)(C::BM * C::BN * 4);
    if constexpr (EPI) {
#pragma unroll
      for (int ni = 0; ni < C::NI; ++ni) {
        const int col = nt * C::BN + wn * C::WN + ni * 32 + l31;
        old_bias[ni] = (a.bias && col < a.T_pad) ? a.bias[col] : 0.f;
      }
    }
#pragma unroll
    for (int mi = 0; mi < C::MI; ++mi)
#pragma unroll
      for (int ni = 0; ni < C::NI; ++ni) {
        const int row = wm * C::WM + mi * 32, col = wn * C::WN + ni * 32 + l31;
        const int co0 = mt * C::BM + row;
        const unsigned to_m = co0 + 32 <= a.Cout ? ((unsigned)(p * a.Cout + co0 + 4 * khalf) * (unsigned)a.T_pad + (unsigned)(nt * C::BN + col)) * 4u : 0x80000000u;
        const unsigned to_ws = slab + (unsigned)((row + 4 * khalf) * C::BN + col) * 4u;
        old_voff[mi][ni] = pub ? to_ws : to_m;
#pragma unroll
        for (int r = 0; r < 16; ++r) acc[PAR ^ 1][mi][ni][r] = 0.f;
      }
  };
  int par = 0;
  while (true) {
    if (!ccur.next(t, k0, k1, part)) break;
    segment(std::integral_constant<int, 0>{});
    par = 1;
    if (!ccur.next(t, k0, k1, part)) break;
    segment(std::integral_constant<int, 1>{});
    par = 0;
  }
  auto finish = [&](auto qc) {
    constexpr int Q = decltype(qc)::value;
    if (fin_tile >= 0) {
      const int rem_tile0 = a.full_q * a.G, RU = (a.tiles - rem_tile0) * a.KI;
      const int tile_end = (fin_tile - rem_tile0 + 1) * a.KI;
      for (int s2 = slot + 1; s2 < a.G; ++s2) {
        int b, e;
        wg_range(RU, a.G, s2, b, e);
        if (b >= tile_end) break;
        if (e <= b) continue;
        if (tid == 0) {
          unsigned spins = 0;
          while (__hip_atomic_load(flags + s2, __ATOMIC_RELAXED, __HIP_MEMORY_SCOPE_AGENT) != want_flag && ++spins < a.spin_limit) __builtin_amdgcn_s_sleep(4);
          const bool timed_out = spins >= a.spin_limit;
          s_handoff_timeout = timed_out ? 1u : 0u;
          if (timed_out) {
            __hip_atomic_store(flags + a.G, 1ull, __ATOMIC_RELAXED, __HIP_MEMORY_SCOPE_AGENT);
            if (a.status) __hip_atomic_store(a.status, (unsigned long long)a.epoch, __ATOMIC_RELAXED, __HIP_MEMORY_SCOPE_SYSTEM);
          }
          __builtin_amdgcn_fence(__ATOMIC_ACQUIRE, "agent");
        }
        __syncthreads();
        const bool poisoned = s_handoff_timeout != 0;
        const unsigned sl2 = (unsigned)s2 * (unsigned)(C::BM * C::BN * 4);
#pragma unroll
        for (int mi = 0; mi < C::MI; ++mi)
#pragma unroll
          for (int ni = 0; ni < C::NI; ++ni) {
            const unsigned vo = sl2 + (unsigned)((wm * C::WM + mi * 32 + 4 * khalf) * C::BN + wn * C::WN + ni * 32 + l31) * 4u;
#pragma unroll
            for (int r = 0; r < 16; ++r)
              acc[Q][mi][ni][r] += __builtin_bit_cast(float, __builtin_amdgcn_raw_buffer_load_b32(rW, vo, (unsigned)((r & 3) + 8 * (r >> 2)) * (unsigned)(C::BN * 4), 0));
            if (poisoned)
#pragma unroll
              for (int r = 0; r < 16; ++r) acc[Q][mi][ni][r] = __builtin_nanf("");
          }
        __syncthreads();
      }
    }
    if (!(ABL & 2) || a.tiles < 0) static_for<0, NMF * 16>([&](auto ec) { store_one(qc, ec); });
  };
  if (par == 1) finish(std::integral_constant<int, 0>{});
  else finish(std::integral_constant<int, 1>{});
  if (old_pub) publish_flag();
  if (a.dbg && tid == 0) {
    const unsigned long long end_r = __builtin_amdgcn_s_memrealtime();
    a.dbg[blockIdx.x * 2] = __builtin_amdgcn_s_memtime() - dbg_c;
    a.dbg[blockIdx.x * 2 + 1] = end_r - dbg_r;
    a.dbg[2 * a.G + blockIdx.x * 2] = dbg_r;
    a.dbg[2 * a.G + blockIdx.x * 2 + 1] = end_r;
  }
}

typedef void (*WgemmFn)(WgemmArgs);
struct WEntry { const char* name; int variant, abl, BM, BN, CK, threads; WgemmFn fn; };
#define WG_ENTRY(name, v, abl, BM, BN, WGM, WGN, CK) {name, v, abl, BM, BN, CK, WGM * WGN * 64, wgemm_kernel<WCfg<BM, BN, WGM, WGN, CK, 3>, abl>}
#define WG_ENTRY_EPI(name, v, BM, BN, WGM, WGN, CK) {name, v + 64, 0, BM, BN, CK, WGM * WGN * 64, wgemm_kernel<WCfg<BM, BN, WGM, WGN, CK, 3>, 0, 1>}
#define WG_ENTRY_S(name, v, BM, BN, WGM, WGN, CK, DPG, SK) {name, v, 0, BM, BN, CK, WGM * WGN * 64, wgemm_kernel<WCfg<BM, BN, WGM, WGN, CK, 3, DPG, SK>, 0>}
const WEntry kW[] = {
    WG_ENTRY("wgemm_256x128_ck32", 1, 0, 256, 128, 4, 2, 32),
    WG_ENTRY("wgemm_128x256_ck32", 2, 0, 128, 256, 2, 4, 32),
    WG_ENTRY("wgemm_128x128_ck32", 3, 0, 128, 128, 2, 4, 32),
    WG_ENTRY("wgemm_256x96_ck32", 4, 0, 256, 96, 8, 1, 32),
    WG_ENTRY("wgemm_256x160_ck32", 5, 0, 256, 160, 8, 1, 32),
    WG_ENTRY_EPI("wgemm_256x128_ck32_epi", 1, 256, 128, 4, 2, 32),
#ifdef MSCNN_WGEMM_DEV
    WG_ENTRY_S("wgemm_256x128_ck32_d2", 25, 256, 128, 4, 2, 32, 2, 0),
    WG_ENTRY_S("wgemm_256x128_ck32_d2_s3", 26, 256, 128, 4, 2, 32, 2, 3),
    WG_ENTRY_S("wgemm_256x128_ck32_d3_s2", 27, 256, 128, 4, 2, 32, 3, 2),
    WG_ENTRY_S("wgemm_256x128_ck32_d1_s6", 28, 256, 128, 4, 2, 32, 1, 6),
#endif
#ifdef MSCNN_WGEMM_DEV
    WG_ENTRY("wgemm_256x128_ck32", 1, 1, 256, 128, 4, 2, 32),
    WG_ENTRY("wgemm_256x128_ck32", 1, 2, 256, 128, 4, 2, 32),
    WG_ENTRY("wgemm_256x128_ck32", 1, 3, 256, 128, 4, 2, 32),
    WG_ENTRY("wgemm_256x128_ck32", 1, 4, 256, 128, 4, 2, 32),
    WG_ENTRY("wgemm_256x128_ck32", 1, 11, 256, 128, 4, 2, 32),
    WG_ENTRY("wgemm_256x128_ck32", 1, 19, 256, 128, 4, 2, 32),
    WG_ENTRY("wgemm_256x128_ck32", 1, 27, 256, 128, 4, 2, 32),
    WG_ENTRY("wgemm_128x256_ck32", 2, 1, 128, 256, 2, 4, 32),
    WG_ENTRY("wgemm_128x256_ck32", 2, 2, 128, 256, 2, 4, 32),
    WG_ENTRY("wgemm_128x256_ck32", 2, 3, 128, 256, 2, 4, 32),
#endif
};

}

namespace mscnn {

static int device_cus(int* dev_out) {
  int dev = 0, n = 0;
  *dev_out = -1;
  if (hipGetDevice(&dev) != hipSuccess || hipDeviceGetAttribute(&n, hipDeviceAttributeMultiprocessorCount, dev) != hipSuccess || n <= 0) {
    (void)hipGetLastError();
    return 256;
  }
  *dev_out = dev;
  return n;
}

namespace {
std::atomic<int> g_whole_tiles{0};
std::atomic<unsigned> g_spin_limit{1u << 22};
std::atomic<int> g_drop_publish{0};
std::atomic<unsigned long long*> g_status[64];
}

static unsigned long long* status_word(int dev) {
  if (dev < 0 || dev >= 64) return nullptr;
  unsigned long long* w = g_status[dev].load(std::memory_order_acquire);
  if (w) return w;
  void* p = nullptr;
  if (hipHostMalloc(&p, 64, hipHostMallocPortable | hipHostMallocMapped | hipHostMallocCoherent) != hipSuccess || !p) {
    (void)hipGetLastError();
    return nullptr;
  }
  *static_cast<volatile unsigned long long*>(p) = 0ull;
  unsigned long long* expected = nullptr;
  if (!g_status[dev].compare_exchange_strong(expected, static_cast<unsigned long long*>(p))) {
    (void)hipHostFree(p);
    return expected;
  }
  return static_cast<unsigned long long*>(p);
}

unsigned long long wgemm_handoff_event() {
  int dev = 0;
  if (hipGetDevice(&dev) != hipSuccess) { (void)hipGetLastError(); return 0; }
  if (dev < 0 || dev >= 64) return 0;
  const unsigned long long* w = g_status[dev].load(std::memory_order_acquire);
  return w ? *static_cast<const volatile unsigned long long*>(w) : 0ull;
}
void wgemm_force_whole_tiles(int on) { g_whole_tiles.store(on ? 1 : 0); }
int wgemm_whole_tiles_forced() { return g_whole_tiles.load(); }
void wgemm_debug_handoff_fault(int drop_publish, unsigned spin_limit) {
  g_drop_publish.store(drop_publish ? 1 : 0);
  g_spin_limit.store(spin_limit ? spin_limit : (1u << 22));
}

bool wgemm_plan(int P, int Cout, int Cin, int T, int variant, WgemmPlan* o) {
  const int variant_flags = variant >> 8;
  variant &= 255;
  if (variant == 0) {
    variant = Cout >= 256 ? 1 : 2;
    if (variant == 1 && !variant_flags) {
      WgemmPlan p1, pc;
      if (wgemm_plan(P, Cout, Cin, T, 1, &p1)) {
        double best = 0.95 * p1.model_us;
        for (int cand : {4, 5})
          if (wgemm_plan(P, Cout, Cin, T, cand, &pc) && pc.model_us < best) { best = pc.model_us; variant = cand; }
        if ((long)P * p1.MT * p1.NT * 2 < p1.G && wgemm_plan(P, Cout, Cin, T, 3, &pc) && pc.model_us < best) { best = pc.model_us; variant = 3; }
      }
    }
  }
  const WEntry* e = nullptr;
  for (const WEntry& w : kW) if (w.variant == variant && w.abl == 0) e = &w;
  if (!e || Cin % e->CK != 0 || Cout % 32 != 0) return false;
  o->P = P; o->Cout = Cout; o->Cin = Cin; o->T = T;
  o->BM = e->BM; o->BN = e->BN; o->CK = e->CK;
  o->T_pad = (T + e->BN - 1) / e->BN * e->BN;
  o->MT = (Cout + e->BM - 1) / e->BM; o->NT = o->T_pad / e->BN; o->KI = Cin / e->CK;
  o->G = device_cus(&o->device);
  const long tiles = (long)P * o->MT * o->NT;
  const long rem = tiles % o->G;
  const double chunk_us = (double)e->BM * e->BN * e->CK / 128.0 / 2214.0;
  const double whole = (double)((tiles + o->G - 1) / o->G) * (o->KI * chunk_us + 6.0);
  const double handoff_us = 18.0 * (double)(e->BM * e->BN) / (256.0 * 128.0);
  const double split = (double)tiles * o->KI / o->G * chunk_us + (double)tiles / o->G * 6.0 + handoff_us;
  o->full_q = (int)(tiles / o->G);
  if (rem > 0 && !(split < 0.97 * whole)) o->full_q += 1;
  o->model_us = rem > 0 ? (split < 0.97 * whole ? split : whole) : whole;
  if (variant_flags & 1) o->full_q = (int)(tiles / o->G);
  if (variant_flags & 2) o->full_q = (int)((tiles + o->G - 1) / o->G);
  o->variant = variant; o->name = e->name;
  o->packed_bytes = (size_t)P * o->MT * o->KI * e->CK * e->BM * 4;
  o->ws_bytes = tiles > (long)o->full_q * o->G ? (size_t)o->G * e->BM * e->BN * 4 + ((size_t)o->G + 1) * 8 : 0;
  const double lim = 2147483648.0 - 65536.0;
  if ((double)tiles * o->KI * o->G >= 2.0e9 || o->KI < 1) return false;
  if ((double)P * Cin * o->T_pad * 4 >= lim || (double)P * Cout * o->T_pad * 4 >= lim || (double)o->packed_bytes >= lim ||
      (double)o->ws_bytes >= lim) return false;
  return true;
}

int wgemm_launch(const WgemmPlan& p, const float* Up, const float* V, float* M, float* ws, hipStream_t st, int abl, unsigned long long* dbg,
                 const float* bias, int relu, size_t m_valid_bytes) {
  const WEntry* e = nullptr;
  for (const WEntry& w : kW) if (w.variant == p.variant && w.abl == abl) e = &w;
  if (!e) return MSCNN_ERR_BAD_ARG;
  int dev = -1;
  if (hipGetDevice(&dev) != hipSuccess) { (void)hipGetLastError(); dev = -1; }
  if (p.device >= 0 && dev != p.device) {
    set_error("wgemm: plan made on device %d launched on device %d (re-plan on the device that runs it)", p.device, dev);
    return MSCNN_ERR_BAD_ARG;
  }
  WgemmArgs a;
  a.Up = Up; a.V = V; a.M = M; a.ws = ws;
  a.P = p.P; a.MT = p.MT; a.NT = p.NT; a.KI = p.KI; a.Cin = p.Cin; a.Cout = p.Cout; a.T_pad = p.T_pad;
  a.tiles = p.P * p.MT * p.NT; a.G = p.G; a.abl = abl; a.dbg = dbg;
  a.full_q = p.full_q; a.ws_bytes = (unsigned)p.ws_bytes;
  if (g_whole_tiles.load(std::memory_order_relaxed)) a.full_q = (a.tiles + p.G - 1) / p.G;
  const int rem = a.tiles - a.full_q * p.G;
  if (rem > 0 && !ws) { set_error("wgemm: workspace missing"); return MSCNN_ERR_WORKSPACE; }
  a.status = rem > 0 ? status_word(dev) : nullptr;
  a.spin_limit = g_spin_limit.load(std::memory_order_relaxed);
  a.drop_publish = g_drop_publish.load(std::memory_order_relaxed);
  a.up_bytes = (unsigned)p.packed_bytes; a.v_bytes = (unsigned)((size_t)p.P * p.Cin * p.T_pad * 4); a.m_bytes = (unsigned)((size_t)p.P * p.Cout * p.T_pad * 4);
  if (m_valid_bytes) a.m_bytes = (unsigned)m_valid_bytes;
  a.bias = bias; a.relu = relu;
  static std::atomic<unsigned> g_epoch{(unsigned)std::chrono::steady_clock::now().time_since_epoch().count() * 2654435761u};
  unsigned ep = ++g_epoch;
  if (ep == 0) ep = ++g_epoch;
  a.epoch = ep;
  e->fn<<<p.G, e->threads, 0, st>>>(a);
  MSCNN_POST_LAUNCH();
  return MSCNN_OK;
}

}

extern "C" unsigned long long mscnn_wgemm_handoff_event(void) { return mscnn::wgemm_handoff_event(); }
extern "C" void mscnn_wgemm_force_whole_tiles(int on) { mscnn::wgemm_force_whole_tiles(on); }
extern "C" int mscnn_wgemm_whole_tiles_forced(void) { return mscnn::wgemm_whole_tiles_forced(); }
extern "C" void mscnn_debug_wgemm_handoff_fault(int drop_publish, unsigned spin_limit) { mscnn::wgemm_debug_handoff_fault(drop_publish, spin_limit); }
```

### mscnn_amd/csrc/wino33_device.h

```cpp
#pragma once
#include <hip/hip_runtime.h>

namespace mscnn {

__device__ __forceinline__ void bt5(const float d[5], float r[5]) {
  r[0] = 2.f * d[0] - d[1] - 2.f * d[2] + d[3];
  r[1] = -2.f * d[1] - d[2] + d[3];
  r[2] = 2.f * d[1] - 3.f * d[2] + d[3];
  r[3] = d[3] - d[1];
  r[4] = 2.f * d[1] - d[2] - 2.f * d[3] + d[4];
}

}
```

### mscnn_amd/csrc/winograd.h

```cpp
#pragma once
#include "common.h"

namespace mscnn {

int wino_pack_weights(int m, const float* w, float* packed, int Cout, int Cin, int BM, int CK, int MT, int KI, hipStream_t st);

int wino_input_transform(int m, const float* x, float* V, int N, int Cin, int H, int W, int pad_h, int pad_w, int tiles_h,
                         int tiles_w, int T_pad, hipStream_t st, bool scalar_f4 = false, bool one_tile_per_lane = false);

int wino_output_transform(int m, const float* M, const float* bias, float* y, float* y_pool, int N, int Cout, int Ho, int Wo,
                          int tiles_h, int tiles_w, int T_pad, int relu, hipStream_t st, unsigned* amax = nullptr, bool scalar_f4 = false);

bool wino44_outin_supported(int H, int W, int tiles_h, int tiles_w);
int wino44_output_into_input(const float* M, const float* bias, float* y, float* V, int N, int C, int H, int W, int tiles_h, int tiles_w,
                             int T_pad_m, int T_pad_v, int relu, hipStream_t st, unsigned* amax = nullptr, int strip_w = 0, int chunk_rows = 0);

}
```

### mscnn_amd/csrc/winograd.hip

```cpp
#include "winograd.h"
#include "x3_device.h"
#include "wino33_device.h"
#include "wino_f4_math.h"
#include <cstdint>

namespace {

#ifndef WINO_NT
#define WINO_NT 1
#endif
template <int BIT>
__device__ __forceinline__ float ld_stream(const float* p) {
  if constexpr ((WINO_NT & BIT) != 0) return __builtin_nontemporal_load(p);
  else return *p;
}
template <int BIT>
__device__ __forceinline__ void st_stream(float* p, float v) {
  if constexpr ((WINO_NT & BIT) != 0) __builtin_nontemporal_store(v, p);
  else *p = v;
}

__global__ __launch_bounds__(256) void wino_weight_kernel(const float* __restrict__ w, float* __restrict__ wp, int Cout, int Cin,
                                                          int BM, int CK, int MT, int KI) {
  const long img_stride = (long)MT * KI * CK * BM;
// ... 111 lines not shown
    if (ow + 1 < Wo && v1 > pooled) pooled = v1;
    if (ow + 1 < Wo && (Wo % 2 == 0)) {
      *reinterpret_cast<float2*>(dst + oh * Wo + ow) = make_float2(v0, v1);
    } else {
      if (ow < Wo) dst[oh * Wo + ow] = v0;
      if (ow + 1 < Wo) dst[oh * Wo + ow + 1] = v1;
    }
  }
  if (yp) yp[(((long)n * Cout + co) * tiles_h + ty) * tiles_w + tx] = pooled;
}


using mscnn::bt5;

__global__ __launch_bounds__(256) void wino33_weight_kernel(const float* __restrict__ w, float* __restrict__ wp, int Cout, int Cin,
                                                            int BM, int CK, int MT, int KI) {
  const long img_stride = (long)MT * KI * CK * BM;
  const long total = (long)MT * BM * KI * CK;
  for (long i = blockIdx.x * 256L + threadIdx.x; i < total; i += (long)gridDim.x * 256) {
    const int m = (int)(i % BM);
    long r = i / BM;
    const int ck = (int)(r % CK); r /= CK;
    const int kc = (int)(r % KI);
    const int mt = (int)(r / KI);
    const int co = mt * BM + m, ci = kc * CK + ck;
    const bool live = co < Cout && ci < Cin;
    float g[3][3];
#pragma unroll
    for (int a = 0; a < 3; ++a)
#pragma unroll
      for (int b = 0; b < 3; ++b) g[a][b] = live ? w[((long)co * Cin + ci) * 9 + a * 3 + b] : 0.f;
    float t[5][3];
#pragma unroll
    for (int b = 0; b < 3; ++b) {
      t[0][b] = 0.5f * g[0][b];
      t[1][b] = -0.5f * (g[0][b] + g[1][b] + g[2][b]);
      t[2][b] = (-g[0][b] + g[1][b] - g[2][b]) * (1.f / 6.f);
      t[3][b] = g[0][b] * (1.f / 6.f) + g[1][b] * (1.f / 3.f) + g[2][b] * (2.f / 3.f);
      t[4][b] = g[2][b];
    }
    float* dst = wp + (((long)mt * KI + kc) * CK + ck) * BM + m;
#pragma unroll
    for (int a = 0; a < 5; ++a) {
      const float x0 = t[a][0], x1 = t[a][1], x2 = t[a][2];
      dst[(a * 5 + 0) * img_stride] = 0.5f * x0;
      dst[(a * 5 + 1) * img_stride] = -0.5f * (x0 + x1 + x2);
      dst[(a * 5 + 2) * img_stride] = (-x0 + x1 - x2) * (1.f / 6.f);
      dst[(a * 5 + 3) * img_stride] = x0 * (1.f / 6.f) + x1 * (1.f / 3.f) + x2 * (2.f / 3.f);
      dst[(a * 5 + 4) * img_stride] = x2;
    }
  }
}

constexpr int kW33Rois = 8, kW33Ch = 16, kW33MaxHW = 64;

__global__ __launch_bounds__(256) void wino33_input_kernel(const float* __restrict__ x, float* __restrict__ V, int N, int Cin, int H,
                                                           int W, int pad_h, int pad_w, int tiles_h, int tiles_w, int T, int T_pad) {
  __shared__ __attribute__((aligned(16))) float sm[kW33Rois * kW33Ch * kW33MaxHW];
  const int tid = threadIdx.x;
  const int r0 = blockIdx.x * kW33Rois, c0 = blockIdx.y * kW33Ch;
  const int HW = H * W, tpr = tiles_h * tiles_w;
  const int nch = min(kW33Ch, Cin - c0);
  const int run = nch * HW;
  for (int rl = 0; rl < kW33Rois; ++rl) {
    const int r = r0 + rl;
    if (r >= N) break;
    const float* src = x + ((long)r * Cin + c0) * HW;
    float* dst = sm + rl * (kW33Ch * HW);
    if ((run & 3) == 0 && ((((long)r * Cin + c0) * HW) & 3) == 0) {
      for (int i = tid; i < run / 4; i += 256) reinterpret_cast<float4*>(dst)[i] = reinterpret_cast<const float4*>(src)[i];
    } else {
      for (int i = tid; i < run; i += 256) dst[i] = src[i];
    }
  }
  __syncthreads();
  const int per_ch = kW33Rois * tpr;
  const long plane_stride = (long)Cin * T_pad;
  for (int it = tid; it < nch * per_ch; it += 256) {
    const int c = it / per_ch, q = it % per_ch;
    const int rl = q / tpr, tl = q % tpr;
    const int r = r0 + rl;
    if (r >= N) continue;
    const int ty = tl / tiles_w, tx = tl % tiles_w;
    const float* map = sm + (rl * kW33Ch + c) * HW;
    const int h0 = 3 * ty - pad_h, w0 = 3 * tx - pad_w;
    float d[5][5];
#pragma unroll
    for (int i = 0; i < 5; ++i) {
      const int h = h0 + i;
      const bool hok = h >= 0 && h < H;
#pragma unroll
      for (int j = 0; j < 5; ++j) {
        const int wv = w0 + j;
        d[i][j] = (hok && wv >= 0 && wv < W) ? map[h * W + wv] : 0.f;
      }
    }
    float rr[5][5];
#pragma unroll
    for (int j = 0; j < 5; ++j) {
      const float col[5] = {d[0][j], d[1][j], d[2][j], d[3][j], d[4][j]};
      float o[5];
      bt5(col, o);
#pragma unroll
      for (int i = 0; i < 5; ++i) rr[i][j] = o[i];
    }
    float* dst = V + (long)(c0 + c) * T_pad + (long)r * tpr + tl;
#pragma unroll
    for (int i = 0; i < 5; ++i) {
      float o[5];
      bt5(rr[i], o);
#pragma unroll
      for (int j = 0; j < 5; ++j) dst[(i * 5 + j) * plane_stride] = o[j];
    }
  }
  if (blockIdx.x == gridDim.x - 1) {
    for (int i = tid; i < nch * (T_pad - T); i += 256) {
      const int c = i / (T_pad - T), t = T + i % (T_pad - T);
#pragma unroll 1
      for (int pl = 0; pl < 25; ++pl) V[pl * plane_stride + (long)(c0 + c) * T_pad + t] = 0.f;
    }
  }
}

__global__ __launch_bounds__(256) void wino33_input_plane_kernel(const float* __restrict__ x, float* __restrict__ V, int N, int Cin,
                                                                 int H, int W, int pad_h, int pad_w, int tiles_h, int tiles_w,
                                                                 int T, int T_pad) {
  const int t = blockIdx.x * 256 + threadIdx.x;
  const int ci = blockIdx.y;
  if (t >= T_pad) return;
  const long plane_stride = (long)Cin * T_pad;
  float* dst = V + (long)ci * T_pad + t;
  float d[5][5];
  if (t < T) {
    const int tx = t % tiles_w, ty = (t / tiles_w) % tiles_h, n = t / (tiles_w * tiles_h);
    const float* src = x + ((long)n * Cin + ci) * H * W;
    const int h0 = 3 * ty - pad_h, w0 = 3 * tx - pad_w;
#pragma unroll
    for (int i = 0; i < 5; ++i) {
      const int h = h0 + i;
      const bool hok = h >= 0 && h < H;
#pragma unroll
      for (int j = 0; j < 5; ++j) {
        const int wv = w0 + j;
        d[i][j] = (hok && wv >= 0 && wv < W) ? src[h * W + wv] : 0.f;
      }
    }
  } else {
#pragma unroll
    for (int i = 0; i < 5; ++i)
#pragma unroll
      for (int j = 0; j < 5; ++j) d[i][j] = 0.f;
  }
  float r[5][5];
#pragma unroll
  for (int j = 0; j < 5; ++j) {
    const float col[5] = {d[0][j], d[1][j], d[2][j], d[3][j], d[4][j]};
    float o[5];
    bt5(col, o);
#pragma unroll
    for (int i = 0; i < 5; ++i) r[i][j] = o[i];
  }
#pragma unroll
  for (int i = 0; i < 5; ++i) {
    float o[5];
    bt5(r[i], o);
#pragma unroll
    for (int j = 0; j < 5; ++j) dst[(i * 5 + j) * plane_stride] = o[j];
  }
}

__global__ __launch_bounds__(256) void wino33_output_kernel(const float* __restrict__ M, const float* __restrict__ bias,
                                                            float* __restrict__ y, int N, int Cout, int Ho, int Wo, int tiles_h,
                                                            int tiles_w, int T, int T_pad, int relu, unsigned* __restrict__ amax) {
  const int t = blockIdx.x * 256 + threadIdx.x;
  const int co = blockIdx.y;
  unsigned am = 0;
  if (t < T) {
  const long plane_stride = (long)Cout * T_pad;
  const float* src = M + (long)co * T_pad + t;
  float r[3][5];
#pragma unroll
  for (int j = 0; j < 5; ++j) {
    const float m0 = src[(0 * 5 + j) * plane_stride], m1 = src[(1 * 5 + j) * plane_stride], m2 = src[(2 * 5 + j) * plane_stride];
    const float m3 = src[(3 * 5 + j) * plane_stride], m4 = src[(4 * 5 + j) * plane_stride];
    r[0][j] = m0 + m1 + m2 + m3;
    r[1][j] = m1 - m2 + 2.f * m3;
    r[2][j] = m1 + m2 + 4.f * m3 + m4;
  }
  const float b = bias ? bias[co] : 0.f;
  const int tx = t % tiles_w, ty = (t / tiles_w) % tiles_h, n = t / (tiles_w * tiles_h);
  float* dst = y + ((long)n * Cout + co) * Ho * Wo;
#pragma unroll
  for (int i = 0; i < 3; ++i) {
    const int oh = 3 * ty + i;
    if (oh >= Ho) continue;
    float v[3];
    v[0] = r[i][0] + r[i][1] + r[i][2] + r[i][3] + b;
    v[1] = r[i][1] - r[i][2] + 2.f * r[i][3] + b;
    v[2] = r[i][1] + r[i][2] + 4.f * r[i][3] + r[i][4] + b;
#pragma unroll
    for (int j = 0; j < 3; ++j) {
      const int ow = 3 * tx + j;
      if (ow >= Wo) continue;
      float u = v[j];
      if (relu) u = u < 0.f ? 0.f : u;
      dst[oh * Wo + ow] = u;
      am = max(am, __float_as_uint(u) & 0x7fffffffu);
    }
  }
  }
  if (amax) mscnn::publish_amax(am, amax, blockIdx.y * gridDim.x + blockIdx.x);
}


constexpr int kW33ORois = 16, kW33OCh = 8;

__global__ __launch_bounds__(256) void wino33_output_roi_kernel(const float* __restrict__ M, const float* __restrict__ bias,
                                                                float* __restrict__ y, int N, int Cout, int Ho, int Wo, int tiles_h,
                                                                int tiles_w, int T_pad, int relu, unsigned* __restrict__ amax) {
  __shared__ __attribute__((aligned(16))) float sm[kW33ORois * kW33OCh * kW33MaxHW];
  const int tid = threadIdx.x;
  const int r0 = blockIdx.x * kW33ORois, c0 = blockIdx.y * kW33OCh;
  const int HW = Ho * Wo, tpr = tiles_h * tiles_w;
  const int nch = min(kW33OCh, Cout - c0), nroi = min(kW33ORois, N - r0);
  const long plane_stride = (long)Cout * T_pad;
  const int per_ch = nroi * tpr;
  unsigned am = 0;
  for (int it = tid; it < nch * per_ch; it += 256) {
    const int c = it / per_ch, q = it % per_ch;
    const int rl = q / tpr, tl = q % tpr;
    const int ty = tl / tiles_w, tx = tl % tiles_w;
    const float* src = M + (long)(c0 + c) * T_pad + (long)(r0 + rl) * tpr + tl;
    float r[3][5];
#pragma unroll
    for (int j = 0; j < 5; ++j) {
      const float m0 = src[(0 * 5 + j) * plane_stride], m1 = src[(1 * 5 + j) * plane_stride], m2 = src[(2 * 5 + j) * plane_stride];
      const float m3 = src[(3 * 5 + j) * plane_stride], m4 = src[(4 * 5 + j) * plane_stride];
      r[0][j] = m0 + m1 + m2 + m3;
      r[1][j] = m1 - m2 + 2.f * m3;
      r[2][j] = m1 + m2 + 4.f * m3 + m4;
    }
    const float b = bias ? bias[c0 + c] : 0.f;
    float* dst = sm + (rl * nch + c) * HW;
#pragma unroll
    for (int i = 0; i < 3; ++i) {
      const int oh = 3 * ty + i;
      if (oh >= Ho) continue;
      float v[3];
      v[0] = r[i][0] + r[i][1] + r[i][2] + r[i][3] + b;
      v[1] = r[i][1] - r[i][2] + 2.f * r[i][3] + b;
      v[2] = r[i][1] + r[i][2] + 4.f * r[i][3] + r[i][4] + b;
#pragma unroll
      for (int j = 0; j < 3; ++j) {
        const int ow = 3 * tx + j;
        if (ow >= Wo) continue;
        float u = v[j];
        if (relu) u = u < 0.f ? 0.f : u;
        dst[oh * Wo + ow] = u;
        am = max(am, __float_as_uint(u) & 0x7fffffffu);
      }
    }
  }
  __syncthreads();
  const int run = nch * HW;
  for (int rl = 0; rl < nroi; ++rl) {
    float* dst = y + ((long)(r0 + rl) * Cout + c0) * HW;
    const float* src = sm + rl * run;
    if ((run & 3) == 0 && ((((long)(r0 + rl) * Cout + c0) * HW) & 3) == 0 && (reinterpret_cast<uintptr_t>(y) & 15) == 0) {
      for (int i = tid; i < run / 4; i += 256) reinterpret_cast<float4*>(dst)[i] = reinterpret_cast<const float4*>(src)[i];
    } else {
      for (int i = tid; i < run; i += 256) dst[i] = src[i];
    }
  }
  if (amax) mscnn::publish_amax(am, amax, blockIdx.y * gridDim.x + blockIdx.x);
}


__device__ __forceinline__ void at5(const float m[5], float o[3]) {
  o[0] = m[0] + m[1] + m[2] + m[3];
  o[1] = m[1] - m[2] + 2.f * m[3];
  o[2] = m[1] + m[2] + 4.f * m[3] + m[4];
}

__global__ __launch_bounds__(256) void wino33_output_pool_kernel(const float* __restrict__ M, const float* __restrict__ bias,
                                                                 float* __restrict__ y, float* __restrict__ yp, int N, int Cout,
                                                                 int Ho, int Wo, int tiles_h, int tiles_w, int T_pad, int relu,
                                                                 unsigned* __restrict__ amax) {
  const int sw = tiles_w / 2, sh = tiles_h / 2;
  const int S = N * sh * sw;
  const int sidx = blockIdx.x * 256 + threadIdx.x;
// ... 339 lines not shown
    }
    if (r0 - 2 + RW * (k + 1) < r1) load_m(q + RW);
    __syncthreads();
    const int p = r0 - 2 + RW * k + w;
    if (p >= r0 && p < r1 && colp) {
      const float* base = reinterpret_cast<const float*>(&ring[0][0][0]);
      float d[6][6];
#pragma unroll
      for (int i = 0; i < 6; ++i) {
        const int yr = 4 * (p - r0 + 1) - 1 + i;
        const float* row = base + ((yr >> 2) & (RING - 1)) * (1024 * S) + (yr & 3) * (256 * S) + 256 * strip + 4 * lane;
        const float4 mid = *reinterpret_cast<const float4*>(row + 4);
        d[i][0] = row[3]; d[i][1] = mid.x; d[i][2] = mid.y; d[i][3] = mid.z; d[i][4] = mid.w; d[i][5] = row[8];
      }
      float* dst = V + (long)c * T_pad_v + ((long)n * tiles_h + p) * tiles_w + jp;
      float r[6][6];
#pragma unroll
      for (int j = 0; j < 6; ++j) {
        const float col[6] = {d[0][j], d[1][j], d[2][j], d[3][j], d[4][j], d[5][j]};
        float o[6];
        wino_f4::bt6(col, o);
#pragma unroll
        for (int i = 0; i < 6; ++i) r[i][j] = o[i];
      }
#pragma unroll
      for (int i = 0; i < 6; ++i) {
        float o[6];
        wino_f4::bt6(r[i], o);
#pragma unroll
        for (int j = 0; j < 6; ++j) st_stream<4>(dst + (i * 6 + j) * stride_v, o[j]);
      }
    }
    __syncthreads();
  }
  if (amax) mscnn::publish_amax(am, amax, blockIdx.y * gridDim.x + blockIdx.x);
}

}

namespace mscnn {

int wino_pack_weights(int m, const float* w, float* packed, int Cout, int Cin, int BM, int CK, int MT, int KI, hipStream_t st) {
  const long total = (long)MT * BM * KI * CK;
  long blocks = (total + 255) / 256;
  if (blocks > 4096) blocks = 4096;
  if (m == 4) wino44_weight_kernel<<<(int)blocks, 256, 0, st>>>(w, packed, Cout, Cin, BM, CK, MT, KI);
  else if (m == 3) wino33_weight_kernel<<<(int)blocks, 256, 0, st>>>(w, packed, Cout, Cin, BM, CK, MT, KI);
  else wino_weight_kernel<<<(int)blocks, 256, 0, st>>>(w, packed, Cout, Cin, BM, CK, MT, KI);
  MSCNN_POST_LAUNCH();
  return MSCNN_OK;
}

int wino_input_transform(int m, const float* x, float* V, int N, int Cin, int H, int W, int pad_h, int pad_w, int tiles_h,
                         int tiles_w, int T_pad, hipStream_t st, bool scalar_f4, bool one_tile_per_lane) {
  const int T = N * tiles_h * tiles_w;
  dim3 grid(cdiv(T_pad, 256), Cin);
  if (m == 4 && pad_w == 1 && W % 4 == 0 && tiles_w * 4 == W && reinterpret_cast<uintptr_t>(x) % 16 == 0 && !scalar_f4) {
    const double fill1 = (double)tiles_w / (64.0 * cdiv(tiles_w, 64)), fill2 = 0.5 * tiles_w / (64.0 * cdiv(tiles_w, 128));
    if (tiles_w % 2 == 0 && T_pad % 2 == 0 && reinterpret_cast<uintptr_t>(V) % 8 == 0 && !one_tile_per_lane && fill2 >= 0.85 * fill1) {
      const int segs = cdiv(tiles_w, 128);
      wino44_input_vec2_kernel<<<dim3(cdiv((long)N * tiles_h * segs, 4), Cin), 256, 0, st>>>(x, V, N, Cin, H, W, pad_h, tiles_h, tiles_w, segs, T_pad);
    } else {
      const int segs = cdiv(tiles_w, 64);
      wino44_input_vec_kernel<<<dim3(cdiv((long)N * tiles_h * segs, 4), Cin), 256, 0, st>>>(x, V, N, Cin, H, W, pad_h, tiles_h, tiles_w, segs, T_pad);
    }
  } else if (m == 4) {
    wino44_input_plane_kernel<<<grid, 256, 0, st>>>(x, V, N, Cin, H, W, pad_h, pad_w, tiles_h, tiles_w, T, T_pad);
  } else if (m == 3 && H * W <= kW33MaxHW) {
    dim3 g3(cdiv(N, kW33Rois), cdiv(Cin, kW33Ch));
    wino33_input_kernel<<<g3, 256, 0, st>>>(x, V, N, Cin, H, W, pad_h, pad_w, tiles_h, tiles_w, T, T_pad);
  } else if (m == 3) {
    wino33_input_plane_kernel<<<grid, 256, 0, st>>>(x, V, N, Cin, H, W, pad_h, pad_w, tiles_h, tiles_w, T, T_pad);
  } else wino_input_kernel<<<grid, 256, 0, st>>>(x, V, N, Cin, H, W, pad_h, pad_w, tiles_h, tiles_w, T, T_pad);
  MSCNN_POST_LAUNCH();
  return MSCNN_OK;
}

int wino_output_transform(int m, const float* M, const float* bias, float* y, float* y_pool, int N, int Cout, int Ho, int Wo,
                          int tiles_h, int tiles_w, int T_pad, int relu, hipStream_t st, unsigned* amax, bool scalar_f4) {
  MSCNN_REQUIRE(!amax || m >= 3, "winograd: max |y| is published by the F(3x3,3x3) / F(4x4,3x3) output transforms only");
  const bool use_vec44 = m == 4 && Wo % 4 == 0 && tiles_w * 4 == Wo && reinterpret_cast<uintptr_t>(y) % 16 == 0 &&
                         (!y_pool || reinterpret_cast<uintptr_t>(y_pool) % 8 == 0) && !scalar_f4;
  MSCNN_REQUIRE(y || (y_pool && use_vec44), "winograd: only the vector F(4x4,3x3) output transform with fused pooling (8-byte aligned pooled map) runs without y");
  const int T = N * tiles_h * tiles_w;
  dim3 grid(cdiv(T, 256), Cout);
  if (use_vec44) {
    wino44_output_vec_kernel<<<grid, 256, 0, st>>>(M, bias, y, y_pool, N, Cout, Ho, Wo, tiles_h, tiles_w, T, T_pad, relu, amax);
  } else if (m == 4) {
    wino44_output_kernel<<<grid, 256, 0, st>>>(M, bias, y, y_pool, N, Cout, Ho, Wo, tiles_h, tiles_w, T, T_pad, relu, amax);
  } else if (m == 3 && y_pool) {
    MSCNN_REQUIRE(tiles_h % 2 == 0 && tiles_w % 2 == 0, "winograd F(3x3,3x3): fused pooling needs even tile counts");
    dim3 gp(cdiv((long)N * (tiles_h / 2) * (tiles_w / 2), 256), Cout);
    wino33_output_pool_kernel<<<gp, 256, 0, st>>>(M, bias, y, y_pool, N, Cout, Ho, Wo, tiles_h, tiles_w, T_pad, relu, amax);
  } else if (m == 3 && Ho * Wo <= kW33MaxHW && !scalar_f4) {
    wino33_output_roi_kernel<<<dim3(cdiv(N, kW33ORois), cdiv(Cout, kW33OCh)), 256, 0, st>>>(M, bias, y, N, Cout, Ho, Wo, tiles_h, tiles_w, T_pad, relu, amax);
  } else if (m == 3) {
    wino33_output_kernel<<<grid, 256, 0, st>>>(M, bias, y, N, Cout, Ho, Wo, tiles_h, tiles_w, T, T_pad, relu, amax);
  } else {
    wino_output_kernel<<<grid, 256, 0, st>>>(M, bias, y, y_pool, N, Cout, Ho, Wo, tiles_h, tiles_w, T, T_pad, relu);
  }
  MSCNN_POST_LAUNCH();
  return MSCNN_OK;
}

bool wino44_outin_supported(int H, int W, int tiles_h, int tiles_w) {
  const int ns = cdiv(tiles_w, 62);
  return H % 4 == 0 && W % 4 == 0 && tiles_h * 4 == H && tiles_w * 4 == W && ns <= 8 && ns != 5 && ns != 7;
}

int wino44_output_into_input(const float* M, const float* bias, float* y, float* V, int N, int C, int H, int W, int tiles_h, int tiles_w,
                             int T_pad_m, int T_pad_v, int relu, hipStream_t st, unsigned* amax, int strip_w, int chunk_rows) {
  MSCNN_REQUIRE(wino44_outin_supported(H, W, tiles_h, tiles_w), "winograd F(4x4,3x3) chain: the map must be whole 4x4 tiles");
  MSCNN_REQUIRE(y == nullptr || reinterpret_cast<uintptr_t>(y) % 16 == 0, "winograd F(4x4,3x3) chain: y must be 16-byte aligned");
  const int ns = cdiv(tiles_w, 62);
  const int sgroups = ns > 4 ? 2 : 1, S = ns / sgroups;
  if (strip_w <= 0 || strip_w > 62 || cdiv(tiles_w, strip_w) != ns) strip_w = cdiv(tiles_w, ns);
  if (chunk_rows <= 0) {
    int chunks = 1;
    while ((long)N * C * chunks * sgroups < 512 && tiles_h / (chunks * 2) >= 9) chunks *= 2;
    chunk_rows = cdiv(tiles_h, chunks);
  }
  const int chunks = cdiv(tiles_h, chunk_rows);
  const dim3 grid(sgroups * chunks * N, C);
  const int nt_m = 36.0 * C * (double)T_pad_m * 4.0 > 200.0e6 ? 1 : 0;
#define MSCNN_OUTIN_(S_, RW_, RING_, NT_) wino44_outin_kernel<S_, RW_, RING_, NT_><<<grid, 64 * S_ * RW_, 0, st>>>(M, bias, y, V, N, C, H, W, tiles_h, tiles_w, T_pad_m, T_pad_v, relu, strip_w, sgroups, chunks, chunk_rows, amax)
#define MSCNN_OUTIN(S_, RW_, RING_) do { if (nt_m) MSCNN_OUTIN_(S_, RW_, RING_, 1); else MSCNN_OUTIN_(S_, RW_, RING_, 0); } while (0)
  if (S == 1) MSCNN_OUTIN(1, 4, 8);
  else if (S == 2) MSCNN_OUTIN(2, 2, 4);
  else if (S == 3) MSCNN_OUTIN(3, 2, 4);
  else MSCNN_OUTIN(4, 2, 4);
#undef MSCNN_OUTIN
#undef MSCNN_OUTIN_
  MSCNN_POST_LAUNCH();
  return MSCNN_OK;
}

}
```

### mscnn_amd/hipapi.py

```python
import ctypes as C
import os

import numpy as np
import torch

_HERE = os.path.dirname(os.path.abspath(__file__))
LIB_PATH = os.path.join(_HERE, "libmscnn_hip.so")
_lib = None


class MscnnError(RuntimeError):
    pass


class ConvDesc(C.Structure):
    _fields_ = [(n, C.c_int) for n in ("N", "Cin", "H", "W", "Cout", "Kh", "Kw", "pad_h", "pad_w",
                                       "stride_h", "stride_w", "group", "relu", "algo", "tune_variant", "tune_grid", "tune_flags")]


AMAX_SLOTS = 1024
ALGO_AUTO, ALGO_DIRECT, ALGO_WINO_F2, ALGO_WINO_F3, ALGO_F16, ALGO_WINO_F3_X3, ALGO_WINO_F4 = 0, 1, 2, 3, 4, 5, 6


MAX_HEADS = 16
# ... 39 lines not shown
        return None
    return C.byref(nms if isinstance(nms, NmsParams) else nms_params(**nms))


def lib():
    global _lib
    if _lib is None:
        if not os.path.exists(LIB_PATH):
            raise MscnnError(f"{LIB_PATH} not built: run `python -c 'import __graft_entry__ as g; g.build()'`")
        L = C.CDLL(LIB_PATH)
        L.mscnn_last_error.restype = C.c_char_p
        L.mscnn_version.restype = C.c_char_p
        L.mscnn_conv2d_plan_kernel.restype = C.c_char_p
        L.mscnn_conv2d_plan_kernel.argtypes = [C.c_void_p]
        L.mscnn_conv2d_plan_publishes_amax.argtypes = [C.c_void_p]
        L.mscnn_conv2d_plan_set_amax_io.argtypes = [C.c_void_p, C.c_void_p, C.c_void_p]
        L.mscnn_conv2d_plan_dtype.restype = C.c_char_p
        L.mscnn_conv2d_plan_dtype.argtypes = [C.c_void_p]
        L.mscnn_inner_product_f16_supported.argtypes = [C.c_int, C.c_int]
        L.mscnn_inner_product_x3_supported.argtypes = [C.c_int, C.c_int]
        L.mscnn_inner_product_x3_packed_bytes.restype = C.c_size_t
        L.mscnn_inner_product_x3_packed_bytes.argtypes = [C.c_int, C.c_int]
        L.mscnn_inner_product_x3_workspace_bytes.restype = C.c_size_t
        L.mscnn_inner_product_x3_workspace_bytes.argtypes = [C.c_int] * 3
        L.mscnn_inner_product_x3_pack.argtypes = [C.c_void_p, C.c_void_p, C.c_int, C.c_int, C.c_void_p]
        L.mscnn_inner_product_x3_fwd.argtypes = [C.c_void_p] * 4 + [C.c_int] * 4 + [C.c_void_p, C.c_void_p, C.c_size_t, C.c_void_p]
        L.mscnn_inner_product_wg_supported.argtypes = [C.c_int] * 3
        L.mscnn_inner_product_wg_packed_bytes.restype = C.c_size_t
        L.mscnn_inner_product_wg_packed_bytes.argtypes = [C.c_int, C.c_int]
        L.mscnn_inner_product_wg_workspace_bytes.restype = C.c_size_t
        L.mscnn_inner_product_wg_workspace_bytes.argtypes = [C.c_int] * 3
        L.mscnn_inner_product_wg_pack.argtypes = [C.c_void_p, C.c_void_p, C.c_int, C.c_int, C.c_void_p]
        L.mscnn_inner_product_wg_fwd.argtypes = [C.c_void_p] * 4 + [C.c_int] * 4 + [C.c_void_p, C.c_size_t, C.c_void_p]
        L.mscnn_max_rel_diff_f32.argtypes = [C.c_void_p, C.c_void_p, C.c_size_t, C.c_float, C.c_void_p, C.c_void_p]
        L.mscnn_sum_squares_f32.argtypes = [C.c_void_p, C.c_size_t, C.c_void_p, C.c_void_p]
        L.mscnn_max_rel_diff_strided_f32.argtypes = [C.c_void_p, C.c_size_t, C.c_void_p, C.c_size_t, C.c_size_t, C.c_size_t, C.c_void_p, C.c_double,
                                                     C.c_void_p, C.c_void_p]
        L.mscnn_store_words_i32.argtypes = [C.c_void_p, C.c_void_p, C.c_int, C.c_void_p]
        L.mscnn_wgemm_handoff_event.restype = C.c_ulonglong
        L.mscnn_wgemm_handoff_event.argtypes = []
        L.mscnn_wgemm_force_whole_tiles.restype = None
        L.mscnn_wgemm_force_whole_tiles.argtypes = [C.c_int]
        L.mscnn_wgemm_whole_tiles_forced.argtypes = []
        L.mscnn_debug_inner_product_rows.restype = None
        L.mscnn_debug_inner_product_rows.argtypes = [C.c_int]
        L.mscnn_debug_wgemm_handoff_fault.restype = None
        L.mscnn_debug_wgemm_handoff_fault.argtypes = [C.c_int, C.c_uint]
        L.mscnn_inner_product_pack_f16.argtypes = [C.c_void_p, C.c_void_p, C.c_int, C.c_int, C.c_void_p]
        L.mscnn_inner_product_fwd_f16.argtypes = [C.c_void_p] * 4 + [C.c_int] * 4 + [C.c_void_p]
        for f in ("mscnn_conv2d_plan_flops", "mscnn_conv2d_plan_executed_flops"):
            getattr(L, f).restype = C.c_double
            getattr(L, f).argtypes = [C.c_void_p]
        L.mscnn_conv2d_plan_set_profiling.argtypes = [C.c_void_p, C.c_int]
        L.mscnn_conv2d_plan_stage_ms.argtypes = [C.c_void_p, C.c_void_p]
        for f in ("mscnn_conv2d_packed_weight_bytes", "mscnn_conv2d_workspace_bytes"):
            getattr(L, f).restype = C.c_size_t
            getattr(L, f).argtypes = [C.c_void_p]
        L.mscnn_conv2d_plan_destroy.argtypes = [C.c_void_p]
        L.mscnn_conv2d_plan_destroy.restype = None
        L.mscnn_conv2d_plan_set_batch.argtypes = [C.c_void_p, C.c_int]
        L.mscnn_conv2d_pack_weights.argtypes = [C.c_void_p] * 4
        L.mscnn_conv2d_fwd_f32.argtypes = [C.c_void_p] * 7 + [C.c_size_t, C.c_void_p]
        L.mscnn_conv2d_fwd_pool_f32.argtypes = [C.c_void_p] * 8 + [C.c_size_t, C.c_void_p]
        L.mscnn_conv2d_plan_can_pool.argtypes = [C.c_void_p]
        L.mscnn_conv2d_plan_can_fuse_roipool.argtypes = [C.c_void_p, C.c_int, C.c_int, C.c_int]
        L.mscnn_conv2d_plan_can_chain.argtypes = [C.c_void_p, C.c_void_p]
        L.mscnn_conv2d_plan_can_pool_only.argtypes = [C.c_void_p]
        L.mscnn_conv2d_fwd_chain_f32.argtypes = [C.c_void_p] * 8 + [C.c_size_t, C.c_void_p, C.c_size_t, C.c_void_p]
        L.mscnn_conv2d_roipool_workspace_bytes.restype = C.c_size_t
        L.mscnn_conv2d_roipool_workspace_bytes.argtypes = [C.c_void_p] + [C.c_int] * 4
        L.mscnn_conv2d_fwd_roipool_pair_f32.argtypes = ([C.c_void_p, C.c_void_p, C.c_void_p] + [C.c_int] * 4 + [C.c_void_p, C.c_float, C.c_float, C.c_float]
                                                        + [C.c_void_p] * 4 + [C.c_size_t, C.c_void_p])
        L.mscnn_roipool_maps_bytes.restype = C.c_size_t
        L.mscnn_roipool_maps_bytes.argtypes = [C.c_int] * 4
        L.mscnn_roipool_maps_build_f32.argtypes = [C.c_void_p, C.c_void_p] + [C.c_int] * 4 + [C.c_void_p]
        L.mscnn_conv2d_plan_weight_layout.argtypes = [C.c_void_p]
        L.mscnn_conv2d_plan_weight_layout.restype = C.c_ulonglong
        L.mscnn_relu_fwd_f32.argtypes = [C.c_void_p, C.c_void_p, C.c_size_t, C.c_float, C.c_void_p]
        L.mscnn_pool2d_fwd_f32.argtypes = [C.c_void_p, C.c_void_p] + [C.c_int] * 11 + [C.c_void_p]
        L.mscnn_inner_product_fwd_f32.argtypes = [C.c_void_p] * 4 + [C.c_int] * 4 + [C.c_void_p]
        L.mscnn_concat_channels_f32.argtypes = [C.c_void_p, C.c_void_p] + [C.c_int] * 5 + [C.c_void_p]
        L.mscnn_deconv_depthwise_fwd_f32.argtypes = [C.c_void_p] * 4 + [C.c_int] * 10 + [C.c_void_p]
        L.mscnn_softmax_fwd_f32.argtypes = [C.c_void_p, C.c_void_p, C.c_int, C.c_int, C.c_int, C.c_void_p]
        L.mscnn_roipool_fwd_f32.argtypes = ([C.c_void_p] * 3 + [C.c_int] * 7 + [C.c_float, C.c_float] + [C.c_int] * 2
                                            + [C.c_void_p])
        L.mscnn_roipool_pair_fwd_f32.argtypes = ([C.c_void_p] * 3 + [C.c_int] * 7 + [C.c_float, C.c_float, C.c_int, C.c_float, C.c_int, C.c_int]
                                                 + [C.c_void_p])
        L.mscnn_roialign_fwd_f32.argtypes = [C.c_void_p] * 3 + [C.c_int] * 7 + [C.c_float, C.c_float, C.c_void_p]
        L.mscnn_eltwise_fwd_f32.argtypes = [C.c_void_p, C.c_int, C.c_void_p, C.c_void_p, C.c_size_t, C.c_int, C.c_void_p]
        L.mscnn_boxoutput_workspace_bytes.restype = C.c_size_t
        L.mscnn_boxoutput_workspace_bytes.argtypes = [C.c_void_p]
        L.mscnn_boxoutput_max_rows.argtypes = [C.c_void_p]
        L.mscnn_boxoutput_fwd_f32.argtypes = [C.c_void_p, C.c_void_p, C.c_void_p, C.c_void_p, C.c_void_p, C.c_int,
                                              C.c_void_p, C.c_void_p, C.c_size_t, C.c_void_p]
        L.mscnn_boxoutput_batch_workspace_bytes.restype = C.c_size_t
        L.mscnn_boxoutput_batch_workspace_bytes.argtypes = [C.c_void_p]
        L.mscnn_boxoutput_batch_fwd_f32.argtypes = L.mscnn_boxoutput_fwd_f32.argtypes
        L.mscnn_nms_workspace_bytes.restype = C.c_size_t
        L.mscnn_nms_workspace_bytes.argtypes = [C.c_int]
        L.mscnn_nms_greedy_f32.argtypes = [C.c_void_p, C.c_int, C.c_float, C.c_int, C.c_void_p, C.c_void_p, C.c_size_t,
                                           C.c_void_p]
        L.mscnn_decodebbox_fwd_f32.argtypes = [C.c_void_p] * 3 + [C.c_int, C.c_int, C.c_void_p, C.c_void_p, C.c_void_p]
        L.mscnn_detections_workspace_bytes.restype = C.c_size_t
        L.mscnn_detections_workspace_bytes.argtypes = [C.c_int]
        L.mscnn_detections_fwd.argtypes = [C.c_void_p] * 4 + [C.c_int] + [C.c_void_p] * 4 + [C.c_size_t, C.c_void_p]
        L.mscnn_detections_multi_pack_bytes.restype = C.c_size_t
# ... 26 lines not shown

def _dev(t):
    if t is None:
        return None
    if not t.is_cuda:
        raise MscnnError("libmscnn_hip has no CPU path: tensor must live on the GPU")
    if not t.is_contiguous():
        raise MscnnError("tensor must be contiguous")
    return C.c_void_p(t.data_ptr())


def _stream():
    return C.c_void_p(torch.cuda.current_stream().cuda_stream)


class ConvPlan:

    def __init__(self, N, Cin, H, W, Cout, Kh, Kw, pad=(0, 0), stride=(1, 1), group=1, relu=False, device="cuda",
                 algo=ALGO_AUTO, tune_variant=0, tune_grid=0, tune_flags=0):
        self.desc = ConvDesc(N, Cin, H, W, Cout, Kh, Kw, pad[0], pad[1], stride[0], stride[1], group, int(relu),
                             algo, tune_variant, tune_grid, tune_flags)
        self._p = C.c_void_p()
        _check(lib().mscnn_conv2d_plan_create(C.byref(self.desc), C.byref(self._p)))
        self.device = device
        self.packed = None
        self.ws = None
        self.w = None
        self._alloc()

    def _alloc(self):
        pb = lib().mscnn_conv2d_packed_weight_bytes(self._p)
        wb = lib().mscnn_conv2d_workspace_bytes(self._p)
        if pb and (self.packed is None or self.packed.numel() * 4 < pb):
            self.packed = torch.empty(pb // 4, dtype=torch.float32, device=self.device)
        if wb and (self.ws is None or self.ws.numel() * 4 < wb):
            self.ws = torch.empty(wb // 4, dtype=torch.float32, device=self.device)

    @property
    def kernel(self):
        return lib().mscnn_conv2d_plan_kernel(self._p).decode()

    @property
    def dtype(self):
        return lib().mscnn_conv2d_plan_dtype(self._p).decode()

    @property
    def flops(self):
        return lib().mscnn_conv2d_plan_flops(self._p)

    @property
    def executed_flops(self):
        return lib().mscnn_conv2d_plan_executed_flops(self._p)

    def set_profiling(self, on=True):
        _check(lib().mscnn_conv2d_plan_set_profiling(self._p, int(on)))

    def stage_ms(self):
        out = (C.c_float * 3)()
        _check(lib().mscnn_conv2d_plan_stage_ms(self._p, out))
        return tuple(out)

    def out_shape(self):
        d = self.desc
        return (d.N, d.Cout, (d.H + 2 * d.pad_h - d.Kh) // d.stride_h + 1, (d.W + 2 * d.pad_w - d.Kw) // d.stride_w + 1)

    def set_batch(self, N):
        before, had = lib().mscnn_conv2d_plan_weight_layout(self._p), self.packed
        _check(lib().mscnn_conv2d_plan_set_batch(self._p, N))
        self.desc.N = N
        self._alloc()
        if getattr(self, "w", None) is not None and self.packed is not None and \
                (lib().mscnn_conv2d_plan_weight_layout(self._p) != before or self.packed is not had):
            self.pack(self.w)

    def pack(self, w):
        self.w = w
        if self.packed is not None:
            _check(lib().mscnn_conv2d_pack_weights(self._p, _dev(w), _dev(self.packed), _stream()))

    @property
    def publishes_amax(self):
        return bool(lib().mscnn_conv2d_plan_publishes_amax(self._p))

    def set_amax_io(self, in_bound=None, out_amax=None):
        self._amax = (in_bound, out_amax)
        _check(lib().mscnn_conv2d_plan_set_amax_io(self._p, _dev(in_bound), _dev(out_amax)))

    @property
    def can_pool(self):
        return bool(lib().mscnn_conv2d_plan_can_pool(self._p))

    def forward(self, x, bias=None, out=None, pool_out=None):
        if out is None:
            out = torch.empty(self.out_shape(), dtype=torch.float32, device=x.device)
        wsb = self.ws.numel() * 4 if self.ws is not None else 0
        _check(lib().mscnn_conv2d_fwd_pool_f32(self._p, _dev(x), _dev(self.w), _dev(self.packed), _dev(bias), _dev(out),
                                               _dev(pool_out), _dev(self.ws), wsb, _stream()))
        return out

    @property
    def can_pool_only(self):
        return bool(lib().mscnn_conv2d_plan_can_pool_only(self._p))

    def can_chain(self, nxt):
        return bool(lib().mscnn_conv2d_plan_can_chain(self._p, nxt._p))

# ... 481 lines not shown
```

Baseline: 225.1.

## Use ragged per-plane column counts in F(3x3,3x3) Winograd GEMM for small maps

For small-map F(3x3,3x3) Winograd convolutions whose output size is not a multiple of 3 and which are not pooled, each transform plane now keeps only the tile columns that contribute to valid outputs. The wgemm plan takes per-plane column counts with offsets into a ragged tile schedule. The input, output and ROI-pool transforms are updated to write and read the compacted plane layout. This is meant to cut GEMM FLOPs and transform traffic on partial edge tiles, at the cost of extra tile decoding logic and narrower stores. Debug hooks for column counts and the schedule are also added.

```diff
diff --git a/include/mscnn_hip.h b/include/mscnn_hip.h
--- a/include/mscnn_hip.h
+++ b/include/mscnn_hip.h
@@ -54,6 +54,7 @@
 MSCNN_API double mscnn_conv2d_plan_flops(const mscnn_conv_plan* plan);
 MSCNN_API const char* mscnn_conv2d_plan_dtype(const mscnn_conv_plan* plan);
 MSCNN_API double mscnn_conv2d_plan_executed_flops(const mscnn_conv_plan* plan);
+MSCNN_API int mscnn_conv2d_plan_plane_columns(const mscnn_conv_plan* plan, int* cols, int n);
 MSCNN_API int mscnn_conv2d_plan_set_profiling(mscnn_conv_plan* plan, int on);
 MSCNN_API int mscnn_conv2d_plan_stage_ms(const mscnn_conv_plan* plan, float ms_out[3]);
 #define MSCNN_AMAX_SLOTS 1024
@@ -89,6 +90,7 @@
 MSCNN_API void mscnn_wgemm_force_whole_tiles(int on);
 MSCNN_API int mscnn_wgemm_whole_tiles_forced(void);
 MSCNN_API void mscnn_debug_wgemm_handoff_fault(int drop_publish, unsigned spin_limit);
+MSCNN_API long mscnn_debug_wgemm_schedule(const mscnn_conv_plan* plan, int whole_tiles, int* rows, long max_rows, int info[8]);
 MSCNN_API int mscnn_inner_product_x3_supported(int N, int K);
 MSCNN_API size_t mscnn_inner_product_x3_packed_bytes(int N, int K);
 MSCNN_API size_t mscnn_inner_product_x3_workspace_bytes(int M, int N, int K);
diff --git a/mscnn_amd/csrc/conv.hip b/mscnn_amd/csrc/conv.hip
--- a/mscnn_amd/csrc/conv.hip
+++ b/mscnn_amd/csrc/conv.hip
@@ -4,6 +4,7 @@
 #include "wino_x3.h"
 #include "wgemm.h"
 #include "roipool_wino.h"
+#include "wino33_device.h"
 #include "conv_c3.h"
 #include "wconv.h"
 #include "wf2conv.h"
@@ -909,6 +910,7 @@
   mscnn::Wf2Plan wf;
   int wino_m = 2;
   int tiles_h = 0, tiles_w = 0, T_pad = 0;
+  int ragged = 0;
   mscnn::X3Plan x3;
   mscnn::X3HeadPlan x3h;
   mscnn_conv_plan* hg = nullptr;
@@ -983,6 +985,8 @@
   p->ws_bytes = p->hg_t_bytes + g->ws_bytes;
   return true;
 }
+
+static bool wino_can_pool(int m, int tiles_h, int tiles_w, int H) { return m == 2 || m == 4 || (tiles_h % 2 == 0 && tiles_w % 2 == 0 && H > 8); }
 
 static bool wino_plan(mscnn_conv_plan* p) {
   const mscnn_conv_desc& d = p->d;
@@ -1032,11 +1036,30 @@
   p->packed_bytes = (size_t)planes * g->packed_bytes;
   p->ws_bytes = (size_t)planes * ((size_t)d.Cin + d.Cout) * T_pad * sizeof(float) + g->ws_bytes;
   p->use_wg = false;
-  if (m >= 3 && !(d.tune_flags & 128) && mscnn::wgemm_plan(planes, d.Cout, d.Cin, (int)T, (d.tune_variant >= 300 && d.tune_variant < 1100) ? d.tune_variant - 300 : 0, &p->wg)) {
+  p->ragged = 0;
+  const int wg_variant = (d.tune_variant >= 300 && d.tune_variant < 1100) ? d.tune_variant - 300 : 0;
+  if (m >= 3 && !(d.tune_flags & 128) && mscnn::wgemm_plan(planes, d.Cout, d.Cin, (int)T, wg_variant, &p->wg)) {
     p->use_wg = true;
     p->T_pad = p->wg.T_pad;
     p->packed_bytes = p->wg.packed_bytes;
     p->ws_bytes = (size_t)planes * ((size_t)d.Cin + d.Cout) * p->wg.T_pad * sizeof(float) + p->wg.ws_bytes;
+    const int mode = mscnn::wino33_ragged_mode(p->Ho, p->Wo);
+    if (m == 3 && d.H * d.W <= mscnn::kWino33SmallMapHW && !wino_can_pool(m, th, tw, d.H) && mode != 0) {
+      int cols[25];
+      for (int i = 0; i < 5; ++i)
+        for (int j = 0; j < 5; ++j) cols[i * 5 + j] = d.N * mscnn::wino33_plane_th(mode, i, th) * mscnn::wino33_plane_tw(mode, j, tw);
+      mscnn::WgemmPlan rg;
+      if (mscnn::wgemm_plan(planes, d.Cout, d.Cin, (int)T, wg_variant, &rg, cols)) {
+        const size_t ws_r = (size_t)planes * ((size_t)d.Cin + d.Cout) * rg.T_pad * sizeof(float) + rg.ws_bytes;
+        if (ws_r > p->ws_bytes) p->ws_bytes = ws_r;
+        if (rg.packed_bytes > p->packed_bytes) p->packed_bytes = rg.packed_bytes;
+        if (!(d.tune_flags & 131072)) {
+          p->wg = rg;
+          p->T_pad = rg.T_pad;
+          p->ragged = mode;
+        }
+      }
+    }
   }
   return true;
 }
@@ -1237,8 +1260,27 @@
   if (!p->wino && !p->x3.BM)
     return mscnn_conv2d_plan_flops(p) * ((p->head.entry < 0 && p->entry >= 0 && kTable[p->entry].variant == 210) ? 3.0 : 1.0);
   const mscnn_conv_desc& d = p->d;
+  if (p->ragged) {
+    double cols = 0;
+    for (int i = 0; i < p->wg.P; ++i) cols += p->wg.cols[i];
+    return 2.0 * d.Cout * d.Cin * cols;
+  }
   const double planes = (double)((p->wino_m + 2) * (p->wino_m + 2)) * (p->x3.BM ? 3.0 : 1.0);
   return 2.0 * planes * d.Cout * d.Cin * ((double)d.N * p->tiles_h * p->tiles_w);
+}
+extern "C" int mscnn_conv2d_plan_plane_columns(const mscnn_conv_plan* p, int* cols, int n) {
+  if (!p || (!p->wino && !p->x3.BM)) return 0;
+  const int planes = (p->wino_m + 2) * (p->wino_m + 2);
+  for (int i = 0; i < planes && i < n && cols; ++i) cols[i] = p->ragged ? p->wg.cols[i] : p->d.N * p->tiles_h * p->tiles_w;
+  return planes;
+}
+extern "C" long mscnn_debug_wgemm_schedule(const mscnn_conv_plan* p, int whole_tiles, int* rows, long max_rows, int info[8]) {
+  if (!p || !p->wino || !p->use_wg) return -1;
+  if (info) {
+    const int v[8] = {p->wg.tiles, p->wg.MT, p->wg.KI, p->wg.G, p->wg.full_q, p->wg.P, p->wg.BN, p->wg.ragged};
+    for (int i = 0; i < 8; ++i) info[i] = v[i];
+  }
+  return mscnn::wgemm_debug_schedule(p->wg, whole_tiles, rows, max_rows);
 }
 extern "C" int mscnn_conv2d_plan_set_profiling(mscnn_conv_plan* p, int on) {
   MSCNN_REQUIRE(p, "conv plan: null");
@@ -1394,7 +1436,7 @@
 
 extern "C" int mscnn_conv2d_plan_can_pool(const mscnn_conv_plan* p) {
   if (!p || p->head.entry >= 0 || p->x3h.rows || p->hg) return 0;
-  if (p->wino || p->x3.BM) return p->wino_m == 2 || p->wino_m == 4 || (p->tiles_h % 2 == 0 && p->tiles_w % 2 == 0 && p->d.H > 8);
+  if (p->wino || p->x3.BM) return wino_can_pool(p->wino_m, p->tiles_h, p->tiles_w, p->d.H);
   return p->entry >= 0 && kTable[p->entry].fix_pool_fn != nullptr;
 }
 
@@ -1443,7 +1485,7 @@
   const mscnn_conv_desc& d = p->d;
   return wino_forward_stages(p, packed, workspace, workspace_bytes, st, input_stage, [&](const float* M) {
     return wino_output_transform(p->wino_m, M, bias, y, y_pool, d.N, d.Cout, p->Ho, p->Wo, p->tiles_h, p->tiles_w, p->T_pad, d.relu, st,
-                                 p->wino_m >= 3 ? p->amax_out : nullptr, (d.tune_flags & 256) != 0);
+                                 p->wino_m >= 3 ? p->amax_out : nullptr, (d.tune_flags & 256) != 0, p->ragged);
   });
 }
 
@@ -1478,7 +1520,7 @@
     if (rc != MSCNN_OK) return rc;
     MSCNN_STAGE_EVENT(2);
     rc = wino_output_transform(3, M, bias, y, y_pool, d.N, d.Cout, p->Ho, p->Wo, p->tiles_h, p->tiles_w, p->T_pad, d.relu, st,
-                               p->amax_out);
+                               p->amax_out, false, 0);
     if (rc != MSCNN_OK) return rc;
     MSCNN_STAGE_EVENT(3);
     p->ev_valid = p->profiling;
@@ -1494,7 +1536,7 @@
   }
   return wino_forward(p, packed, bias, y, y_pool, workspace, workspace_bytes, st, [&](float* V) {
     return wino_input_transform(p->wino_m, x, V, d.N, d.Cin, d.H, d.W, d.pad_h, d.pad_w, p->tiles_h, p->tiles_w, p->T_pad, st,
-                                (d.tune_flags & 256) != 0, (d.tune_flags & 4096) != 0);
+                                (d.tune_flags & 256) != 0, (d.tune_flags & 4096) != 0, p->ragged);
   });
 #undef MSCNN_STAGE_EVENT
 }
@@ -1537,7 +1579,7 @@
   auto input_stage = [&](float* V) {
     if (!x) return (int)MSCNN_OK;
     return wino_input_transform(p->wino_m, x, V, d.N, d.Cin, d.H, d.W, d.pad_h, d.pad_w, p->tiles_h, p->tiles_w, p->T_pad, st,
-                                (d.tune_flags & 256) != 0, (d.tune_flags & 4096) != 0);
+                                (d.tune_flags & 256) != 0, (d.tune_flags & 4096) != 0, p->ragged);
   };
   if (!next) return wino_forward(p, packed, bias, y, y_pool, workspace, workspace_bytes, st, input_stage);
   return wino_forward_stages(p, packed, workspace, workspace_bytes, st, input_stage, [&](const float* M) {
@@ -1581,7 +1623,7 @@
       if (rc != MSCNN_OK) return rc;
     }
     return mscnn::roipool_wino33_forward(prepared_maps ? prepared_maps : own_maps, rois, V, p->d.N, N, C, H, W, p->T_pad, spatial_scale,
-                                         pad_ratio_a, pad_ratio_b, st);
+                                         pad_ratio_a, pad_ratio_b, st, p->ragged);
   });
 }
 
diff --git a/mscnn_amd/csrc/roipool_wino.h b/mscnn_amd/csrc/roipool_wino.h
--- a/mscnn_amd/csrc/roipool_wino.h
+++ b/mscnn_amd/csrc/roipool_wino.h
@@ -7,6 +7,6 @@
 size_t roipool_wino33_scratch_bytes(int N, int C, int H, int W);
 int roipool_wino33_build_maps(const float* feat, float* maps, int N, int C, int H, int W, hipStream_t st);
 int roipool_wino33_forward(const float* maps, const float* rois, float* V, int R, int N, int C, int H, int W, int T_pad,
-                           float spatial_scale, float pad_a, float pad_b, hipStream_t st);
+                           float spatial_scale, float pad_a, float pad_b, hipStream_t st, int ragged);
 
 }
diff --git a/mscnn_amd/csrc/roipool_wino.hip b/mscnn_amd/csrc/roipool_wino.hip
--- a/mscnn_amd/csrc/roipool_wino.hip
+++ b/mscnn_amd/csrc/roipool_wino.hip
@@ -5,6 +5,7 @@
 namespace {
 
 typedef unsigned u32x4 __attribute__((ext_vector_type(4)));
+typedef unsigned u32x2 __attribute__((ext_vector_type(2)));
 
 constexpr int kNB = 4;
 constexpr int kLevels = 4;
@@ -32,7 +33,7 @@
 constexpr int kRois = 8;
 constexpr int kLdsRow = kRois * 4 + 4;
 
-template <int PH, int PW>
+template <int PH, int PW, bool RAG>
 __global__ __launch_bounds__(kRois * 64) void roipool_wino33_kernel(RpwArgs a) {
   static_assert(PH == 7 && PW == 7, "tiles per ROI: 2 x 2 tiles of 3 x 3 outputs (a 16-byte unit of V per plane)");
   __shared__ __attribute__((aligned(16))) float s_out[5 * 64 * kLdsRow];
@@ -162,6 +163,7 @@
 #pragma unroll
       for (int t = 0; t < 4; ++t) {
         const int ty = t >> 1, tx = t & 1;
+        if (RAG && i == 4 && ty == 1) continue;
         float rr[5];
 #pragma unroll
         for (int j = 0; j < 5; ++j) {
@@ -181,24 +183,41 @@
       }
       __syncthreads();
 #pragma unroll
-      for (int j = 0; j < 5; ++j)
-        *reinterpret_cast<float4*>(&s_out[(j * 64 + lane) * kLdsRow + wave * 4]) = make_float4(out[j][0], out[j][1], out[j][2], out[j][3]);
+      for (int j = 0; j < 5; ++j) {
+        float* slot_ = &s_out[(j * 64 + lane) * kLdsRow + wave * 4];
+        if (!RAG || (i < 4 && j < 4)) *reinterpret_cast<float4*>(slot_) = make_float4(out[j][0], out[j][1], out[j][2], out[j][3]);
+        else if (i < 4) *reinterpret_cast<float2*>(slot_) = make_float2(out[j][0], out[j][2]);
+        else if (j < 4) *reinterpret_cast<float2*>(slot_) = make_float2(out[j][0], out[j][1]);
+        else *slot_ = out[j][0];
+      }
       __syncthreads();
-#pragma unroll
-      for (int n = 0; n < 5 * 64 * kRois / (kRois * 64); ++n) {
-        const int item = tid + n * (kRois * 64);
-        const int rq = item % kRois, ch = (item / kRois) % 64, j = item / (kRois * 64);
+      static_assert(kRois == 8, "thread = (channel, roi) of a pass");
+#pragma unroll
+      for (int j = 0; j < 5; ++j) {
+        const int rq = tid % kRois, ch = tid / kRois;
         if (r0 + rq < a.R) {
-          const float4 u = *reinterpret_cast<const float4*>(&s_out[(j * 64 + ch) * kLdsRow + rq * 4]);
-          u32x4 pk;
-          pk.x = __builtin_bit_cast(unsigned, u.x); pk.y = __builtin_bit_cast(unsigned, u.y);
-          pk.z = __builtin_bit_cast(unsigned, u.z); pk.w = __builtin_bit_cast(unsigned, u.w);
-          const unsigned off = (unsigned)(i * 5 + j) * plane_bytes + ((unsigned)(q * C + c0 + ch) * (unsigned)a.T_pad + (unsigned)(r0 + rq) * 4u) * 4u;
-#ifndef RPW_NO_STORE
-          __builtin_amdgcn_raw_buffer_store_b128(pk, rV, off, 0u, 0);
-#else
-          if (a.T_pad < 0) __builtin_amdgcn_raw_buffer_store_b128(pk, rV, off, 0u, 0);
+          const float* unit = &s_out[(j * 64 + ch) * kLdsRow + rq * 4];
+          const int uw = RAG ? (i < 4 ? 2 : 1) * (j < 4 ? 2 : 1) : 4;
+          const unsigned off = (unsigned)(i * 5 + j) * plane_bytes + ((unsigned)(q * C + c0 + ch) * (unsigned)a.T_pad + (unsigned)(r0 + rq) * (unsigned)uw) * 4u;
+#ifdef RPW_NO_STORE
+          if (a.T_pad < 0)
 #endif
+          {
+            if (uw == 4) {
+              const float4 u = *reinterpret_cast<const float4*>(unit);
+              u32x4 pk;
+              pk.x = __builtin_bit_cast(unsigned, u.x); pk.y = __builtin_bit_cast(unsigned, u.y);
+              pk.z = __builtin_bit_cast(unsigned, u.z); pk.w = __builtin_bit_cast(unsigned, u.w);
+              __builtin_amdgcn_raw_buffer_store_b128(pk, rV, off, 0u, 0);
+            } else if (uw == 2) {
+              const float2 u = *reinterpret_cast<const float2*>(unit);
+              u32x2 pk;
+              pk.x = __builtin_bit_cast(unsigned, u.x); pk.y = __builtin_bit_cast(unsigned, u.y);
+              __builtin_amdgcn_raw_buffer_store_b64(pk, rV, off, 0u, 0);
+            } else {
+              __builtin_amdgcn_raw_buffer_store_b32(__builtin_bit_cast(unsigned, unit[0]), rV, off, 0u, 0);
+            }
+          }
         }
       }
     }
@@ -272,8 +291,9 @@
 }
 
 int roipool_wino33_forward(const float* maps, const float* rois, float* V, int R, int N, int C, int H, int W, int T_pad,
-                           float spatial_scale, float pad_a, float pad_b, hipStream_t st) {
+                           float spatial_scale, float pad_a, float pad_b, hipStream_t st, int ragged) {
   MSCNN_REQUIRE(maps && rois && V, "roipool+transform: null pointer");
+  MSCNN_REQUIRE(ragged == 0 || ragged == wino33_ragged_mode(5, 5), "roipool+transform: the planes are uniform or ragged on both axes (5 x 5 outputs)");
   MSCNN_REQUIRE(R > 0 && N > 0 && C % 64 == 0 && H > 0 && W > 0 && T_pad >= 4 * R && T_pad % 4 == 0, "roipool+transform: bad shape");
   const double lb = (double)N * C * H * W * 4.0, vb = 25.0 * 2.0 * C * (double)T_pad * 4.0;
   MSCNN_REQUIRE(kLevels * lb < 4.0e9 && vb < 4.0e9, "roipool+transform: feature maps or transform planes beyond a 32-bit buffer window");
@@ -283,7 +303,8 @@
   a.R = R; a.C = C; a.H = H; a.W = W; a.T_pad = T_pad;
   a.level_bytes = (unsigned)lb; a.maps_bytes = (unsigned)(kLevels * lb); a.v_bytes = (unsigned)vb;
   a.spatial_scale = spatial_scale; a.pad_a = pad_a; a.pad_b = pad_b;
-  roipool_wino33_kernel<7, 7><<<dim3(C / 64, cdiv(R, kRois), 2), kRois * 64, 0, st>>>(a);
+  if (ragged) roipool_wino33_kernel<7, 7, true><<<dim3(C / 64, cdiv(R, kRois), 2), kRois * 64, 0, st>>>(a);
+  else roipool_wino33_kernel<7, 7, false><<<dim3(C / 64, cdiv(R, kRois), 2), kRois * 64, 0, st>>>(a);
   MSCNN_POST_LAUNCH();
   return MSCNN_OK;
 }
diff --git a/mscnn_amd/csrc/wgemm.h b/mscnn_amd/csrc/wgemm.h
--- a/mscnn_amd/csrc/wgemm.h
+++ b/mscnn_amd/csrc/wgemm.h
@@ -4,10 +4,34 @@
 
 namespace mscnn {
 
+constexpr int kWgemmMaxPlanes = 36;
+
+__host__ __device__ __forceinline__ void wgemm_tile_decode(int t, int MT, int NT, int P, const int* nt_off, int& p, int& nt, int& mt) {
+  mt = t % MT;
+  if (!nt_off) {
+    nt = (t / MT) % NT;
+    p = t / (MT * NT);
+    return;
+  }
+#if defined(__HIP_DEVICE_COMPILE__)
+  const int q = __builtin_amdgcn_readfirstlane(t / MT);
+#else
+  const int q = t / MT;
+#endif
+  int pp = 0;
+  while (pp + 1 < P && nt_off[pp + 1] <= q) ++pp;
+  p = pp;
+  nt = q - nt_off[pp];
+}
+
 struct WgemmPlan {
   int P, Cout, Cin, T, T_pad;
   int BM, BN, CK, MT, NT, KI;
   int G;
+  int tiles;
+  int ragged;
+  int cols[kWgemmMaxPlanes];
+  int nt_off[kWgemmMaxPlanes + 1];
   int device;
   int full_q;
   int variant;
@@ -17,7 +41,7 @@
   size_t ws_bytes;
 };
 
-bool wgemm_plan(int P, int Cout, int Cin, int T, int variant, WgemmPlan* out);
+bool wgemm_plan(int P, int Cout, int Cin, int T, int variant, WgemmPlan* out, const int* plane_cols = nullptr);
 
 int wgemm_launch(const WgemmPlan& p, const float* Up, const float* V, float* M, float* ws, hipStream_t st, int abl = 0,
                  unsigned long long* dbg = nullptr, const float* bias = nullptr, int relu = 0, size_t m_valid_bytes = 0);
@@ -26,5 +50,6 @@
 void wgemm_force_whole_tiles(int on);
 int wgemm_whole_tiles_forced();
 void wgemm_debug_handoff_fault(int drop_publish, unsigned spin_limit);
+long wgemm_debug_schedule(const WgemmPlan& p, int whole_tiles, int* out, long max_rows);
 
 }
diff --git a/mscnn_amd/csrc/wgemm.hip b/mscnn_amd/csrc/wgemm.hip
--- a/mscnn_amd/csrc/wgemm.hip
+++ b/mscnn_amd/csrc/wgemm.hip
@@ -20,6 +20,7 @@
   unsigned long long* status;
   unsigned spin_limit;
   int drop_publish;
+  int nt_off[mscnn::kWgemmMaxPlanes + 1];
 };
 
 template <int BM_, int BN_, int WGM_, int WGN_, int CK_, int ST_, int DPG_ = 1, int SK_ = 0>
@@ -86,14 +87,16 @@
   int slot, G, KI, full_q, rem_tile0, r;
   int it, re;
   int nparts;
-  __device__ __forceinline__ void init(const WgemmArgs& a, int slot_) {
-    slot = slot_; G = a.G; KI = a.KI; rem_tile0 = a.full_q * a.G; r = 0; nparts = 0;
-    full_q = slot_ < a.tiles ? min(a.full_q, (a.tiles - slot_ + a.G - 1) / a.G) : 0;
-    if (a.tiles > rem_tile0) wg_range((a.tiles - rem_tile0) * a.KI, a.G, slot_, it, re);
+  __device__ __forceinline__ void init(const WgemmArgs& a, int slot_) { init(a.tiles, a.G, a.KI, a.full_q, slot_); }
+  __device__ __host__ __forceinline__ void init(int tiles, int G_, int KI_, int a_full_q, int slot_) {
+    slot = slot_; G = G_; KI = KI_; rem_tile0 = a_full_q * G_; r = 0; nparts = 0;
+    const int rounds = slot_ < tiles ? (tiles - slot_ + G_ - 1) / G_ : 0;
+    full_q = a_full_q < rounds ? a_full_q : rounds;
+    if (tiles > rem_tile0) wg_range((tiles - rem_tile0) * KI_, G_, slot_, it, re);
     else it = re = 0;
   }
   __device__ __forceinline__ int units() const { return full_q * KI + (re - it); }
-  __device__ __forceinline__ bool next(int& t, int& k0, int& k1, int& part) {
+  __device__ __host__ __forceinline__ bool next(int& t, int& k0, int& k1, int& part) {
     if (r < full_q) { t = slot + r * G; k0 = 0; k1 = KI; part = -1; ++r; return true; }
     if (it >= re) return false;
     t = rem_tile0 + it / KI;
@@ -106,7 +109,7 @@
   }
 };
 
-template <class C, int ABL, int EPI = 0>
+template <class C, int ABL, int EPI = 0, bool RAG = false>
 __global__ __launch_bounds__(C::THREADS, C::NW / 4) void wgemm_kernel(WgemmArgs a) {
   __shared__ __attribute__((aligned(1024))) float lds[C::LDS_FLOATS];
   __shared__ unsigned s_handoff_timeout;
@@ -153,7 +156,8 @@
     if (p_kc == p_k1 && pu < nunits) {
       int t, part;
       pcur.next(t, p_kc, p_k1, part);
-      const int mt = t % a.MT, nt = (t / a.MT) % a.NT, p = t / (a.MT * a.NT);
+      int mt, nt, p;
+      mscnn::wgemm_tile_decode(t, a.MT, a.NT, a.P, RAG ? a.nt_off : nullptr, p, nt, mt);
       p_kc = __builtin_amdgcn_readfirstlane(p_kc); p_k1 = __builtin_amdgcn_readfirstlane(p_k1);
       p_a = __builtin_amdgcn_readfirstlane((unsigned)((p * a.MT + mt) * a.KI) * (unsigned)C::A_BYTES);
       p_b = __builtin_amdgcn_readfirstlane(((unsigned)(p * a.Cin) * (unsigned)a.T_pad + (unsigned)(nt * C::BN)) * 4u);
@@ -316,7 +320,8 @@
     chunk(par_c, std::true_type{}, next_stage_addr());
     if (old_pub) { publish_flag(); old_pub = false; }
     for (int kc = k0 + 1; kc < k1; ++kc) chunk(par_c, std::false_type{}, next_stage_addr());
-    const int mt = t % a.MT, nt = (t / a.MT) % a.NT, p = t / (a.MT * a.NT);
+    int mt, nt, p;
+    mscnn::wgemm_tile_decode(t, a.MT, a.NT, a.P, RAG ? a.nt_off : nullptr, p, nt, mt);
     const bool pub = part >= 0 && k0 > 0;
     if (part >= 0 && k0 == 0) fin_tile = t;
     old_pub = pub;
@@ -406,16 +411,17 @@
 }
 
 typedef void (*WgemmFn)(WgemmArgs);
-struct WEntry { const char* name; int variant, abl, BM, BN, CK, threads; WgemmFn fn; };
+struct WEntry { const char* name; int variant, abl, BM, BN, CK, threads; WgemmFn fn; WgemmFn fn_ragged = nullptr; };
 #define WG_ENTRY(name, v, abl, BM, BN, WGM, WGN, CK) {name, v, abl, BM, BN, CK, WGM * WGN * 64, wgemm_kernel<WCfg<BM, BN, WGM, WGN, CK, 3>, abl>}
+#define WG_ENTRY_R(name, v, BM, BN, WGM, WGN, CK) {name, v, 0, BM, BN, CK, WGM * WGN * 64, wgemm_kernel<WCfg<BM, BN, WGM, WGN, CK, 3>, 0>, wgemm_kernel<WCfg<BM, BN, WGM, WGN, CK, 3>, 0, 0, true>}
 #define WG_ENTRY_EPI(name, v, BM, BN, WGM, WGN, CK) {name, v + 64, 0, BM, BN, CK, WGM * WGN * 64, wgemm_kernel<WCfg<BM, BN, WGM, WGN, CK, 3>, 0, 1>}
 #define WG_ENTRY_S(name, v, BM, BN, WGM, WGN, CK, DPG, SK) {name, v, 0, BM, BN, CK, WGM * WGN * 64, wgemm_kernel<WCfg<BM, BN, WGM, WGN, CK, 3, DPG, SK>, 0>}
 const WEntry kW[] = {
-    WG_ENTRY("wgemm_256x128_ck32", 1, 0, 256, 128, 4, 2, 32),
-    WG_ENTRY("wgemm_128x256_ck32", 2, 0, 128, 256, 2, 4, 32),
-    WG_ENTRY("wgemm_128x128_ck32", 3, 0, 128, 128, 2, 4, 32),
-    WG_ENTRY("wgemm_256x96_ck32", 4, 0, 256, 96, 8, 1, 32),
-    WG_ENTRY("wgemm_256x160_ck32", 5, 0, 256, 160, 8, 1, 32),
+    WG_ENTRY_R("wgemm_256x128_ck32", 1, 256, 128, 4, 2, 32),
+    WG_ENTRY_R("wgemm_128x256_ck32", 2, 128, 256, 2, 4, 32),
+    WG_ENTRY_R("wgemm_128x128_ck32", 3, 128, 128, 2, 4, 32),
+    WG_ENTRY_R("wgemm_256x96_ck32", 4, 256, 96, 8, 1, 32),
+    WG_ENTRY_R("wgemm_256x160_ck32", 5, 256, 160, 8, 1, 32),
     WG_ENTRY_EPI("wgemm_256x128_ck32_epi", 1, 256, 128, 4, 2, 32),
 #ifdef MSCNN_WGEMM_DEV
     WG_ENTRY_S("wgemm_256x128_ck32_d2", 25, 256, 128, 4, 2, 32, 2, 0),
@@ -491,18 +497,22 @@
   g_spin_limit.store(spin_limit ? spin_limit : (1u << 22));
 }
 
-bool wgemm_plan(int P, int Cout, int Cin, int T, int variant, WgemmPlan* o) {
+bool wgemm_plan(int P, int Cout, int Cin, int T, int variant, WgemmPlan* o, const int* plane_cols) {
+  if (P < 1 || P > kWgemmMaxPlanes) return false;
+  if (plane_cols)
+    for (int p = 0; p < P; ++p)
+      if (plane_cols[p] < 0 || plane_cols[p] > T) return false;
   const int variant_flags = variant >> 8;
   variant &= 255;
   if (variant == 0) {
     variant = Cout >= 256 ? 1 : 2;
     if (variant == 1 && !variant_flags) {
       WgemmPlan p1, pc;
-      if (wgemm_plan(P, Cout, Cin, T, 1, &p1)) {
+      if (wgemm_plan(P, Cout, Cin, T, 1, &p1, plane_cols)) {
         double best = 0.95 * p1.model_us;
         for (int cand : {4, 5})
-          if (wgemm_plan(P, Cout, Cin, T, cand, &pc) && pc.model_us < best) { best = pc.model_us; variant = cand; }
-        if ((long)P * p1.MT * p1.NT * 2 < p1.G && wgemm_plan(P, Cout, Cin, T, 3, &pc) && pc.model_us < best) { best = pc.model_us; variant = 3; }
+          if (wgemm_plan(P, Cout, Cin, T, cand, &pc, plane_cols) && pc.model_us < best) { best = pc.model_us; variant = cand; }
+        if ((long)p1.tiles * 2 < p1.G && wgemm_plan(P, Cout, Cin, T, 3, &pc, plane_cols) && pc.model_us < best) { best = pc.model_us; variant = 3; }
       }
     }
   }
@@ -514,7 +524,14 @@
   o->T_pad = (T + e->BN - 1) / e->BN * e->BN;
   o->MT = (Cout + e->BM - 1) / e->BM; o->NT = o->T_pad / e->BN; o->KI = Cin / e->CK;
   o->G = device_cus(&o->device);
-  const long tiles = (long)P * o->MT * o->NT;
+  o->ragged = plane_cols ? 1 : 0;
+  o->nt_off[0] = 0;
+  for (int p = 0; p < kWgemmMaxPlanes; ++p) {
+    o->cols[p] = p < P ? (plane_cols ? plane_cols[p] : T) : 0;
+    o->nt_off[p + 1] = o->nt_off[p] + (p < P ? (plane_cols ? (plane_cols[p] + e->BN - 1) / e->BN : o->NT) : 0);
+  }
+  const long tiles = (long)o->MT * o->nt_off[P];
+  o->tiles = (int)tiles;
   const long rem = tiles % o->G;
   const double chunk_us = (double)e->BM * e->BN * e->CK / 128.0 / 2214.0;
   const double whole = (double)((tiles + o->G - 1) / o->G) * (o->KI * chunk_us + 6.0);
@@ -539,7 +556,7 @@
                  const float* bias, int relu, size_t m_valid_bytes) {
   const WEntry* e = nullptr;
   for (const WEntry& w : kW) if (w.variant == p.variant && w.abl == abl) e = &w;
-  if (!e) return MSCNN_ERR_BAD_ARG;
+  if (!e || (p.ragged && !e->fn_ragged)) return MSCNN_ERR_BAD_ARG;
   int dev = -1;
   if (hipGetDevice(&dev) != hipSuccess) { (void)hipGetLastError(); dev = -1; }
   if (p.device >= 0 && dev != p.device) {
@@ -549,7 +566,9 @@
   WgemmArgs a;
   a.Up = Up; a.V = V; a.M = M; a.ws = ws;
   a.P = p.P; a.MT = p.MT; a.NT = p.NT; a.KI = p.KI; a.Cin = p.Cin; a.Cout = p.Cout; a.T_pad = p.T_pad;
-  a.tiles = p.P * p.MT * p.NT; a.G = p.G; a.abl = abl; a.dbg = dbg;
+  a.tiles = p.tiles; a.G = p.G;
+  a.abl = abl; a.dbg = dbg;
+  for (int i = 0; i <= kWgemmMaxPlanes; ++i) a.nt_off[i] = p.nt_off[i];
   a.full_q = p.full_q; a.ws_bytes = (unsigned)p.ws_bytes;
   if (g_whole_tiles.load(std::memory_order_relaxed)) a.full_q = (a.tiles + p.G - 1) / p.G;
   const int rem = a.tiles - a.full_q * p.G;
@@ -564,9 +583,30 @@
   unsigned ep = ++g_epoch;
   if (ep == 0) ep = ++g_epoch;
   a.epoch = ep;
-  e->fn<<<p.G, e->threads, 0, st>>>(a);
+  (p.ragged ? e->fn_ragged : e->fn)<<<p.G, e->threads, 0, st>>>(a);
   MSCNN_POST_LAUNCH();
   return MSCNN_OK;
+}
+
+long wgemm_debug_schedule(const WgemmPlan& p, int whole_tiles, int* out, long max_rows) {
+  const int full_q = whole_tiles ? (p.tiles + p.G - 1) / p.G : p.full_q;
+  long n = 0;
+  for (int slot = 0; slot < p.G; ++slot) {
+    SegCursor c;
+    c.init(p.tiles, p.G, p.KI, full_q, slot);
+    int t, k0, k1, part;
+    while (c.next(t, k0, k1, part)) {
+      if (out) {
+        if (n >= max_rows) return -1;
+        int pl, nt, mt;
+        wgemm_tile_decode(t, p.MT, p.NT, p.P, p.ragged ? p.nt_off : nullptr, pl, nt, mt);
+        const int row[7] = {slot, pl, nt, mt, k0, k1, part};
+        for (int i = 0; i < 7; ++i) out[n * 7 + i] = row[i];
+      }
+      ++n;
+    }
+  }
+  return n;
 }
 
 }
diff --git a/mscnn_amd/csrc/wino33_device.h b/mscnn_amd/csrc/wino33_device.h
--- a/mscnn_amd/csrc/wino33_device.h
+++ b/mscnn_amd/csrc/wino33_device.h
@@ -11,4 +11,15 @@
   r[4] = 2.f * d[1] - d[2] - 2.f * d[3] + d[4];
 }
 
+constexpr int kWino33RaggedRows = 1, kWino33RaggedCols = 2;
+__host__ __device__ __forceinline__ int wino33_ragged_mode(int Ho, int Wo) {
+  return (Ho % 3 != 0 ? kWino33RaggedRows : 0) | (Wo % 3 != 0 ? kWino33RaggedCols : 0);
 }
+__host__ __device__ __forceinline__ int wino33_plane_th(int ragged, int i, int tiles_h) {
+  return tiles_h - ((i == 4 && (ragged & kWino33RaggedRows)) ? 1 : 0);
+}
+__host__ __device__ __forceinline__ int wino33_plane_tw(int ragged, int j, int tiles_w) {
+  return tiles_w - ((j == 4 && (ragged & kWino33RaggedCols)) ? 1 : 0);
+}
+
+}
diff --git a/mscnn_amd/csrc/winograd.h b/mscnn_amd/csrc/winograd.h
--- a/mscnn_amd/csrc/winograd.h
+++ b/mscnn_amd/csrc/winograd.h
@@ -3,13 +3,16 @@
 
 namespace mscnn {
 
+constexpr int kWino33SmallMapHW = 64;
+
 int wino_pack_weights(int m, const float* w, float* packed, int Cout, int Cin, int BM, int CK, int MT, int KI, hipStream_t st);
 
 int wino_input_transform(int m, const float* x, float* V, int N, int Cin, int H, int W, int pad_h, int pad_w, int tiles_h,
-                         int tiles_w, int T_pad, hipStream_t st, bool scalar_f4 = false, bool one_tile_per_lane = false);
+                         int tiles_w, int T_pad, hipStream_t st, bool scalar_f4 = false, bool one_tile_per_lane = false, int ragged = 0);
 
 int wino_output_transform(int m, const float* M, const float* bias, float* y, float* y_pool, int N, int Cout, int Ho, int Wo,
-                          int tiles_h, int tiles_w, int T_pad, int relu, hipStream_t st, unsigned* amax = nullptr, bool scalar_f4 = false);
+                          int tiles_h, int tiles_w, int T_pad, int relu, hipStream_t st, unsigned* amax = nullptr, bool scalar_f4 = false,
+                          int ragged = 0);
 
 bool wino44_outin_supported(int H, int W, int tiles_h, int tiles_w);
 int wino44_output_into_input(const float* M, const float* bias, float* y, float* V, int N, int C, int H, int W, int tiles_h, int tiles_w,
diff --git a/mscnn_amd/csrc/winograd.hip b/mscnn_amd/csrc/winograd.hip
--- a/mscnn_amd/csrc/winograd.hip
+++ b/mscnn_amd/csrc/winograd.hip
@@ -187,10 +187,11 @@
   }
 }
 
-constexpr int kW33Rois = 8, kW33Ch = 16, kW33MaxHW = 64;
+constexpr int kW33Rois = 8, kW33Ch = 16, kW33MaxHW = mscnn::kWino33SmallMapHW;
 
 __global__ __launch_bounds__(256) void wino33_input_kernel(const float* __restrict__ x, float* __restrict__ V, int N, int Cin, int H,
-                                                           int W, int pad_h, int pad_w, int tiles_h, int tiles_w, int T, int T_pad) {
+                                                           int W, int pad_h, int pad_w, int tiles_h, int tiles_w, int T, int T_pad,
+                                                           int ragged) {
   __shared__ __attribute__((aligned(16))) float sm[kW33Rois * kW33Ch * kW33MaxHW];
   const int tid = threadIdx.x;
   const int r0 = blockIdx.x * kW33Rois, c0 = blockIdx.y * kW33Ch;
@@ -244,11 +245,20 @@
     for (int i = 0; i < 5; ++i) {
       float o[5];
       bt5(rr[i], o);
-#pragma unroll
-      for (int j = 0; j < 5; ++j) dst[(i * 5 + j) * plane_stride] = o[j];
-    }
-  }
-  if (blockIdx.x == gridDim.x - 1) {
+      if (!ragged) {
+#pragma unroll
+        for (int j = 0; j < 5; ++j) dst[(i * 5 + j) * plane_stride] = o[j];
+      } else {
+        const int th = mscnn::wino33_plane_th(ragged, i, tiles_h);
+#pragma unroll
+        for (int j = 0; j < 5; ++j) {
+          const int tw = mscnn::wino33_plane_tw(ragged, j, tiles_w);
+          if (ty < th && tx < tw) V[(i * 5 + j) * plane_stride + (long)(c0 + c) * T_pad + ((long)r * th + ty) * tw + tx] = o[j];
+        }
+      }
+    }
+  }
+  if (blockIdx.x == gridDim.x - 1 && !ragged) {
     for (int i = tid; i < nch * (T_pad - T); i += 256) {
       const int c = i / (T_pad - T), t = T + i % (T_pad - T);
 #pragma unroll 1
@@ -304,26 +314,46 @@
   }
 }
 
+__device__ __forceinline__ void wino33_load_ragged_column(const float* __restrict__ row, long plane_stride, int ragged, int j, int n, int ty,
+                                                          int tx, int tiles_h, int tiles_w, float& m0, float& m1, float& m2, float& m3,
+                                                          float& m4) {
+  const int tw = mscnn::wino33_plane_tw(ragged, j, tiles_w);
+  const int th4 = mscnn::wino33_plane_th(ragged, 4, tiles_h);
+  m0 = m1 = m2 = m3 = m4 = 0.f;
+  if (tx < tw) {
+    const long col = ((long)n * tiles_h + ty) * tw + tx;
+    m0 = row[(0 * 5 + j) * plane_stride + col]; m1 = row[(1 * 5 + j) * plane_stride + col]; m2 = row[(2 * 5 + j) * plane_stride + col];
+    m3 = row[(3 * 5 + j) * plane_stride + col];
+    if (ty < th4) m4 = row[(4 * 5 + j) * plane_stride + ((long)n * th4 + ty) * tw + tx];
+  }
+}
+
 __global__ __launch_bounds__(256) void wino33_output_kernel(const float* __restrict__ M, const float* __restrict__ bias,
                                                             float* __restrict__ y, int N, int Cout, int Ho, int Wo, int tiles_h,
-                                                            int tiles_w, int T, int T_pad, int relu, unsigned* __restrict__ amax) {
+                                                            int tiles_w, int T, int T_pad, int relu, unsigned* __restrict__ amax,
+                                                            int ragged) {
   const int t = blockIdx.x * 256 + threadIdx.x;
   const int co = blockIdx.y;
   unsigned am = 0;
   if (t < T) {
   const long plane_stride = (long)Cout * T_pad;
   const float* src = M + (long)co * T_pad + t;
+  const int tx = t % tiles_w, ty = (t / tiles_w) % tiles_h, n = t / (tiles_w * tiles_h);
   float r[3][5];
 #pragma unroll
   for (int j = 0; j < 5; ++j) {
-    const float m0 = src[(0 * 5 + j) * plane_stride], m1 = src[(1 * 5 + j) * plane_stride], m2 = src[(2 * 5 + j) * plane_stride];
-    const float m3 = src[(3 * 5 + j) * plane_stride], m4 = src[(4 * 5 + j) * plane_stride];
+    float m0, m1, m2, m3, m4;
+    if (!ragged) {
+      m0 = src[(0 * 5 + j) * plane_stride]; m1 = src[(1 * 5 + j) * plane_stride]; m2 = src[(2 * 5 + j) * plane_stride];
+      m3 = src[(3 * 5 + j) * plane_stride]; m4 = src[(4 * 5 + j) * plane_stride];
+    } else {
+      wino33_load_ragged_column(M + (long)co * T_pad, plane_stride, ragged, j, n, ty, tx, tiles_h, tiles_w, m0, m1, m2, m3, m4);
+    }
     r[0][j] = m0 + m1 + m2 + m3;
     r[1][j] = m1 - m2 + 2.f * m3;
     r[2][j] = m1 + m2 + 4.f * m3 + m4;
   }
   const float b = bias ? bias[co] : 0.f;
-  const int tx = t % tiles_w, ty = (t / tiles_w) % tiles_h, n = t / (tiles_w * tiles_h);
   float* dst = y + ((long)n * Cout + co) * Ho * Wo;
 #pragma unroll
   for (int i = 0; i < 3; ++i) {
@@ -352,7 +382,8 @@
 
 __global__ __launch_bounds__(256) void wino33_output_roi_kernel(const float* __restrict__ M, const float* __restrict__ bias,
                                                                 float* __restrict__ y, int N, int Cout, int Ho, int Wo, int tiles_h,
-                                                                int tiles_w, int T_pad, int relu, unsigned* __restrict__ amax) {
+                                                                int tiles_w, int T_pad, int relu, unsigned* __restrict__ amax,
+                                                                int ragged) {
   __shared__ __attribute__((aligned(16))) float sm[kW33ORois * kW33OCh * kW33MaxHW];
   const int tid = threadIdx.x;
   const int r0 = blockIdx.x * kW33ORois, c0 = blockIdx.y * kW33OCh;
@@ -369,8 +400,13 @@
     float r[3][5];
 #pragma unroll
     for (int j = 0; j < 5; ++j) {
-      const float m0 = src[(0 * 5 + j) * plane_stride], m1 = src[(1 * 5 + j) * plane_stride], m2 = src[(2 * 5 + j) * plane_stride];
-      const float m3 = src[(3 * 5 + j) * plane_stride], m4 = src[(4 * 5 + j) * plane_stride];
+      float m0, m1, m2, m3, m4;
+      if (!ragged) {
+        m0 = src[(0 * 5 + j) * plane_stride]; m1 = src[(1 * 5 + j) * plane_stride]; m2 = src[(2 * 5 + j) * plane_stride];
+        m3 = src[(3 * 5 + j) * plane_stride]; m4 = src[(4 * 5 + j) * plane_stride];
+      } else {
+        wino33_load_ragged_column(M + (long)(c0 + c) * T_pad, plane_stride, ragged, j, r0 + rl, ty, tx, tiles_h, tiles_w, m0, m1, m2, m3, m4);
+      }
       r[0][j] = m0 + m1 + m2 + m3;
       r[1][j] = m1 - m2 + 2.f * m3;
       r[2][j] = m1 + m2 + 4.f * m3 + m4;
@@ -816,7 +852,8 @@
 }
 
 int wino_input_transform(int m, const float* x, float* V, int N, int Cin, int H, int W, int pad_h, int pad_w, int tiles_h,
-                         int tiles_w, int T_pad, hipStream_t st, bool scalar_f4, bool one_tile_per_lane) {
+                         int tiles_w, int T_pad, hipStream_t st, bool scalar_f4, bool one_tile_per_lane, int ragged) {
+  MSCNN_REQUIRE(!ragged || (m == 3 && H * W <= kW33MaxHW), "winograd: ragged planes exist for the small-map F(3x3,3x3) kernels only");
   const int T = N * tiles_h * tiles_w;
   dim3 grid(cdiv(T_pad, 256), Cin);
   if (m == 4 && pad_w == 1 && W % 4 == 0 && tiles_w * 4 == W && reinterpret_cast<uintptr_t>(x) % 16 == 0 && !scalar_f4) {
@@ -832,7 +869,7 @@
     wino44_input_plane_kernel<<<grid, 256, 0, st>>>(x, V, N, Cin, H, W, pad_h, pad_w, tiles_h, tiles_w, T, T_pad);
   } else if (m == 3 && H * W <= kW33MaxHW) {
     dim3 g3(cdiv(N, kW33Rois), cdiv(Cin, kW33Ch));
-    wino33_input_kernel<<<g3, 256, 0, st>>>(x, V, N, Cin, H, W, pad_h, pad_w, tiles_h, tiles_w, T, T_pad);
+    wino33_input_kernel<<<g3, 256, 0, st>>>(x, V, N, Cin, H, W, pad_h, pad_w, tiles_h, tiles_w, T, T_pad, ragged);
   } else if (m == 3) {
     wino33_input_plane_kernel<<<grid, 256, 0, st>>>(x, V, N, Cin, H, W, pad_h, pad_w, tiles_h, tiles_w, T, T_pad);
   } else wino_input_kernel<<<grid, 256, 0, st>>>(x, V, N, Cin, H, W, pad_h, pad_w, tiles_h, tiles_w, T, T_pad);
@@ -841,7 +878,9 @@
 }
 
 int wino_output_transform(int m, const float* M, const float* bias, float* y, float* y_pool, int N, int Cout, int Ho, int Wo,
-                          int tiles_h, int tiles_w, int T_pad, int relu, hipStream_t st, unsigned* amax, bool scalar_f4) {
+                          int tiles_h, int tiles_w, int T_pad, int relu, hipStream_t st, unsigned* amax, bool scalar_f4, int ragged) {
+  MSCNN_REQUIRE(!ragged || (m == 3 && !y_pool && ragged == mscnn::wino33_ragged_mode(Ho, Wo)),
+                "winograd: ragged planes exist for the F(3x3,3x3) output transforms without pooling only, with the mode of the output shape");
   MSCNN_REQUIRE(!amax || m >= 3, "winograd: max |y| is published by the F(3x3,3x3) / F(4x4,3x3) output transforms only");
   const bool use_vec44 = m == 4 && Wo % 4 == 0 && tiles_w * 4 == Wo && reinterpret_cast<uintptr_t>(y) % 16 == 0 &&
                          (!y_pool || reinterpret_cast<uintptr_t>(y_pool) % 8 == 0) && !scalar_f4;
@@ -857,9 +896,9 @@
     dim3 gp(cdiv((long)N * (tiles_h / 2) * (tiles_w / 2), 256), Cout);
     wino33_output_pool_kernel<<<gp, 256, 0, st>>>(M, bias, y, y_pool, N, Cout, Ho, Wo, tiles_h, tiles_w, T_pad, relu, amax);
   } else if (m == 3 && Ho * Wo <= kW33MaxHW && !scalar_f4) {
-    wino33_output_roi_kernel<<<dim3(cdiv(N, kW33ORois), cdiv(Cout, kW33OCh)), 256, 0, st>>>(M, bias, y, N, Cout, Ho, Wo, tiles_h, tiles_w, T_pad, relu, amax);
+    wino33_output_roi_kernel<<<dim3(cdiv(N, kW33ORois), cdiv(Cout, kW33OCh)), 256, 0, st>>>(M, bias, y, N, Cout, Ho, Wo, tiles_h, tiles_w, T_pad, relu, amax, ragged);
   } else if (m == 3) {
-    wino33_output_kernel<<<grid, 256, 0, st>>>(M, bias, y, N, Cout, Ho, Wo, tiles_h, tiles_w, T, T_pad, relu, amax);
+    wino33_output_kernel<<<grid, 256, 0, st>>>(M, bias, y, N, Cout, Ho, Wo, tiles_h, tiles_w, T, T_pad, relu, amax, ragged);
   } else {
     wino_output_kernel<<<grid, 256, 0, st>>>(M, bias, y, y_pool, N, Cout, Ho, Wo, tiles_h, tiles_w, T, T_pad, relu);
   }
diff --git a/mscnn_amd/hipapi.py b/mscnn_amd/hipapi.py
--- a/mscnn_amd/hipapi.py
+++ b/mscnn_amd/hipapi.py
@@ -115,6 +115,9 @@
             getattr(L, f).restype = C.c_double
             getattr(L, f).argtypes = [C.c_void_p]
         L.mscnn_conv2d_plan_set_profiling.argtypes = [C.c_void_p, C.c_int]
+        L.mscnn_conv2d_plan_plane_columns.argtypes = [C.c_void_p, C.c_void_p, C.c_int]
+        L.mscnn_debug_wgemm_schedule.restype = C.c_long
+        L.mscnn_debug_wgemm_schedule.argtypes = [C.c_void_p, C.c_int, C.c_void_p, C.c_long, C.c_void_p]
         L.mscnn_conv2d_plan_stage_ms.argtypes = [C.c_void_p, C.c_void_p]
         for f in ("mscnn_conv2d_packed_weight_bytes", "mscnn_conv2d_workspace_bytes"):
             getattr(L, f).restype = C.c_size_t
@@ -247,6 +250,23 @@
     def executed_flops(self):
         return lib().mscnn_conv2d_plan_executed_flops(self._p)
 
+    def plane_columns(self):
+        out = (C.c_int * 36)()
+        n = lib().mscnn_conv2d_plan_plane_columns(self._p, out, 36)
+        return [int(out[i]) for i in range(n)]
+
+    def debug_wgemm_schedule(self, whole_tiles=False):
+        import numpy as np
+        info = (C.c_int * 8)()
+        n = lib().mscnn_debug_wgemm_schedule(self._p, int(bool(whole_tiles)), None, 0, info)
+        if n < 0:
+            return None
+        rows = np.zeros((max(n, 1), 7), dtype=np.int32)
+        got = lib().mscnn_debug_wgemm_schedule(self._p, int(bool(whole_tiles)), rows.ctypes.data_as(C.c_void_p), n, info)
+        assert got == n
+        keys = ("tiles", "MT", "KI", "G", "full_q", "planes", "BN", "ragged")
+        return {k: int(info[i]) for i, k in enumerate(keys)}, rows[:n]
+
     def set_profiling(self, on=True):
         _check(lib().mscnn_conv2d_plan_set_profiling(self._p, int(on)))
 
```

Measured after the change: 229.9, median of 6. 2.1% higher.
